# honglianghe/CDNet

Measured on AMD Instinct MI355X. Metric: tiles/sec (train fwd+bwd+Adam), 256x256, higher is better.
Workload: dtype fp32

## Files before the change

### cdnet_amd/csrc/conv.hip

```cpp
#include <type_traits>
#include <vector>
#include "common.h"
#include "conv_args.h"
#include "launch.h"
#include "xform.h"
#include "stage16.h"
#include <stdlib.h>

using namespace cdnet;

typedef __attribute__((ext_vector_type(16))) float f32x16;
typedef __attribute__((ext_vector_type(4))) float f32x4;

namespace {

__device__ int g_dbg_dummy;

struct PackDesc {
    const float *w;
    unsigned short *out;
    int Cout, Cin, KH, KW, CK, BN, nchunk, ntile, TAPS, mode, parity;
    unsigned block0, nblocks;
    int split;
    const float *scale;
};

__device__ __forceinline__ void pack_range(const PackDesc &d, size_t first, size_t stride) {
    const float *__restrict__ w = d.w;
    unsigned short *__restrict__ out = d.out;
    const int Cout = d.Cout, Cin = d.Cin, KH = d.KH, KW = d.KW, CK = d.CK, BN = d.BN, nchunk = d.nchunk, TAPS = d.TAPS, mode = d.mode,
              parity = d.parity;
    const size_t total = (size_t)d.ntile * nchunk * TAPS * (CK / 16) * 2 * BN * (d.split ? 2 : 1);
    for (size_t i = first; i < total; i += stride) {
        size_t r = i;
        int tap = r % TAPS; r /= TAPS;
        int col = r % BN; r /= BN;
        int half = r % 2; r /= 2;
        int kc = r % (CK / 16); r /= (CK / 16);
        int hl = 0;
        if (d.split) { hl = r % 2; r /= 2; }
        int chunk = r % nchunk; r /= nchunk;
        int tile = (int)r;
        int co = tile * BN + col;
        const size_t ovec = ((((((size_t)tile * nchunk + chunk) * (d.split ? 2 : 1) + hl) * TAPS + tap) * (CK / 16) + kc) * 2 + half) * BN + col;
        unsigned short o8[8];
#pragma unroll
        for (int j = 0; j < 8; ++j) {
        int ci = chunk * CK + kc * 16 + half * 8 + j;
        float v = 0.f;
        if (co < Cout && ci < Cin) {
            if (mode == 0) {
                v = w[(((size_t)co * Cin + ci) * KH + tap / KW) * KW + tap % KW];
            } else if (mode == 1) {
                int kh = KH - 1 - tap / KW, kw = KW - 1 - tap % KW;
                v = w[(((size_t)ci * Cout + co) * KH + kh) * KW + kw];
            } else if (mode == 2) {
                int a = parity >> 1, b = parity & 1, ty = tap >> 1, tx = tap & 1;
                int kh = a == 0 ? (ty == 0 ? 1 : 3) : (ty == 0 ? 0 : 2);
                int kw = b == 0 ? (tx == 0 ? 1 : 3) : (tx == 0 ? 0 : 2);
                v = w[(((size_t)ci * Cout + co) * 4 + kh) * 4 + kw];
            } else if (mode == 3) {
                int a = parity >> 1, b = parity & 1;
                v = w[(((size_t)ci * Cout + co) * 2 + a) * 2 + b];
            } else if (mode == 7) {
                const int Ct = Cout / 4;
                const int a = co / (2 * Ct), b = (co / Ct) & 1, c = co % Ct;
                const int tf = 8 - tap;
                const int kh = 2 * (tf / 3 - 1) + a + 1, kw = 2 * (tf % 3 - 1) + b + 1;
                if (kh >= 0 && kh < 3 && kw >= 0 && kw < 3) v = w[(((size_t)ci * Ct + c) * 3 + kh) * 3 + kw];
            } else {
                const int Ct = Cin / 4;
                const int a = ci / (2 * Ct), b = (ci / Ct) & 1, c = ci % Ct;
                if (mode == 4) {
                    const int kh = 2 * (tap / 3) + a - 1, kw = 2 * (tap % 3) + b - 1;
                    if (kh >= 0 && kh < 4 && kw >= 0 && kw < 4) v = w[(((size_t)co * Ct + c) * 4 + kh) * 4 + kw];
                } else if (mode == 5) {
                    v = w[(((size_t)co * Ct + c) * 2 + a) * 2 + b];
                } else {
                    const int kh = 2 * (tap / 3 - 1) + a + 1, kw = 2 * (tap % 3 - 1) + b + 1;
                    if (kh >= 0 && kh < 3 && kw >= 0 && kw < 3) v = w[(((size_t)co * Ct + c) * 3 + kh) * 3 + kw];
                }
            }
        }
        if (d.scale && co < Cout) v *= d.scale[co];
        const unsigned short hi = f2bf(v);
        o8[j] = hl ? f2bf(v - bf2f(hi)) : hi;
        }
        uint4 ov;
        ov.x = o8[0] | ((unsigned)o8[1] << 16); ov.y = o8[2] | ((unsigned)o8[3] << 16);
        ov.z = o8[4] | ((unsigned)o8[5] << 16); ov.w = o8[6] | ((unsigned)o8[7] << 16);
        reinterpret_cast<uint4 *>(out)[ovec] = ov;
    }
}

__global__ void pack_weights_kernel(PackDesc d) {
    pack_range(d, (size_t)blockIdx.x * blockDim.x + threadIdx.x, (size_t)gridDim.x * blockDim.x);
}

__global__ void pack_weights_batch_kernel(const PackDesc *__restrict__ table, int n) {
    int lo = 0, hi = n - 1;
    while (lo < hi) {
        const int mid = (lo + hi + 1) >> 1;
        if (table[mid].block0 <= blockIdx.x) lo = mid; else hi = mid - 1;
    }
    const PackDesc d = table[lo];
    pack_range(d, (size_t)(blockIdx.x - d.block0) * blockDim.x + threadIdx.x, (size_t)d.nblocks * blockDim.x);
}

__device__ __forceinline__ V16 max8(V16 a, V16 b, bool nonneg) {
    V16 o;
    if (nonneg) {
        o.u = __builtin_bit_cast(uint4, xf_max_nonneg_bf8(__builtin_bit_cast(xf_u32x4, a.u), __builtin_bit_cast(xf_u32x4, b.u)));
        return o;
    }
#pragma unroll
    for (int j = 0; j < 8; ++j) o.h[j] = bf2f(a.h[j]) >= bf2f(b.h[j]) ? a.h[j] : b.h[j];
    return o;
}

constexpr int XF_MAX = 2048;

__device__ __forceinline__ void load_chan_xf(ChanXf &t, const ConvSrc &s, const float *xf, int xfs, int c) {
    t.on = s.scale != nullptr;
    if (!t.on) return;
    const float4 *ps = reinterpret_cast<const float4 *>(xf ? xf + c : s.scale + c);
    const float4 *ph = reinterpret_cast<const float4 *>(xf ? xf + xfs + c : s.shift + c);
    float4 a = ps[0], b = ps[1], cc = ph[0], d = ph[1];
    t.sc[0] = a.x; t.sc[1] = a.y; t.sc[2] = a.z; t.sc[3] = a.w; t.sc[4] = b.x; t.sc[5] = b.y; t.sc[6] = b.z; t.sc[7] = b.w;
    t.sh[0] = cc.x; t.sh[1] = cc.y; t.sh[2] = cc.z; t.sh[3] = cc.w; t.sh[4] = d.x; t.sh[5] = d.y; t.sh[6] = d.z; t.sh[7] = d.w;
}

template <int TH, int CK>
struct HaloImg {
    static constexpr bool SWZ = (TH == 16 && CK == 16);
    static constexpr int PSTR = SWZ ? CK * 2 : CK * 2 + 16;
    __device__ __forceinline__ static int off(int pix, int hy, int slot) { return pix * PSTR + (SWZ ? ((slot ^ (hy & 1)) * 16) : slot * 16); }
};

template <int TH, int TW, int CK>
__device__ __forceinline__ void stage_input(const ConvSrc &s, int cc0, int n, int y0, int x0, int H, int W,
                                            unsigned char *lds_a, int tid, const float *xf = nullptr, int xfs = 0) {
    constexpr int VPP = CK / 8;
    constexpr int HW_ = TW + 2, NPIX = (TH + 2) * (TW + 2);
    const int slot = tid % VPP;
    ChanXf t;
    load_chan_xf(t, s, xf, xfs, cc0 + slot * 8);
    const bool relu = s.relu != 0;
    const bool f16 = s.f16 != 0;
    const bool plain = !t.on && !relu && s.res == nullptr && !f16;
    const int Hl = s.pool ? (s.Hs + (s.pool == 2)) / 2 : s.Hs, Wl = s.pool ? (s.Ws + (s.pool == 2)) / 2 : s.Ws;
    const size_t rs = s.row_stride ? (size_t)s.row_stride : (size_t)s.Ws * s.C;
    const size_t img = (size_t)n * s.Hs * rs;
    for (int v = tid; v < NPIX * VPP; v += 256) {
        const int pix = v / VPP;
        const int hy = pix / HW_, hx = pix - hy * HW_;
        const int y = y0 - 1 + hy, x = x0 - 1 + hx;
        V16 val;
        val.u = make_uint4(0, 0, 0, 0);
        const int ys = y - s.off_y, xs = x - s.off_x;
        if (y >= 0 && y < H && x >= 0 && x < W && ys >= 0 && ys < Hl && xs >= 0 && xs < Wl) {
            if (!s.pool) {
                const size_t e = img + (size_t)ys * rs + (size_t)xs * s.C + cc0 + slot * 8;
                V16 raw;
                raw.u = *reinterpret_cast<const uint4 *>(s.x + e);
                if (plain) val = raw;
                else if (s.res) { V16 r; r.u = *reinterpret_cast<const uint4 *>(s.res + e); val = xform8(raw, &r, t, relu, f16); }
                else val = xform8(raw, nullptr, t, relu, f16);
            } else {
#pragma unroll
                for (int q = 0; q < 4; ++q) {
                    const int yy = 2 * ys + (q >> 1), xx = 2 * xs + (q & 1);
                    if (q != 0 && (yy >= s.Hs || xx >= s.Ws)) continue;
                    const size_t e = img + (size_t)yy * rs + (size_t)xx * s.C + cc0 + slot * 8;
                    V16 raw;
                    raw.u = *reinterpret_cast<const uint4 *>(s.x + e);
                    V16 tv = plain ? raw : xform8(raw, nullptr, t, relu, f16);
                    val = q == 0 ? tv : max8(val, tv, relu);
                }
            }
        }
        *reinterpret_cast<uint4 *>(lds_a + HaloImg<TH, CK>::off(pix, hy, slot)) = val.u;
    }
}

#ifndef CDNET_CONV_XCD
#define CDNET_CONV_XCD 1
#endif
#ifndef CDNET_CONV_GLDS
#define CDNET_CONV_GLDS 1
#endif
#ifndef CDNET_CONV_ADEPTH
#define CDNET_CONV_ADEPTH 1
#endif
template <int TH, int TW, int CK, int BN, int TAPS>
struct ConvLds {
    static constexpr bool DEEP = (CK == 16 && TH == 16);
    static constexpr bool GLDS = CDNET_CONV_GLDS && DEEP;
    static constexpr int ADEPTH = DEEP ? CDNET_CONV_ADEPTH : 1;
    static constexpr int PSTR = HaloImg<TH, CK>::PSTR;
    static constexpr int A_BYTES = (TH + 2) * (TW + 2) * PSTR;
    static constexpr int B_BYTES = TAPS * CK * BN * 2;
    static constexpr int STAGE = A_BYTES + (GLDS ? 2 : 1) * B_BYTES;
    static constexpr int OUT_BYTES = TH * TW * (BN * 2 + 8);
    static constexpr int STATS_BYTES = 4 * 2 * BN * 4;
    static constexpr int MAIN = ((STAGE > OUT_BYTES + STATS_BYTES ? STAGE : OUT_BYTES + STATS_BYTES) + 15) / 16 * 16;
    static int bytes(int ctot) { return MAIN + 2 * ((ctot + 7) / 8 * 8) * 4; }
};

template <int TH, int TW, int CK, int BN, int TAPS>
struct Prefetch {
    static constexpr int VPP = CK / 8;
    static constexpr int NPIX = (TH + 2) * (TW + 2);
    static constexpr int NA = (NPIX * VPP + 255) / 256;
    static constexpr bool GLDS = ConvLds<TH, TW, CK, BN, TAPS>::GLDS;
    static constexpr int NB = (TAPS * CK * BN * 2 / 16 + 255) / 256;
    static constexpr int ADEPTH = ConvLds<TH, TW, CK, BN, TAPS>::ADEPTH;
    struct ASlot {
        uint4 a[NA];
        unsigned valid;
        bool pooled;
    };
    ASlot s[ADEPTH];
    uint4 b[GLDS ? 1 : NB];
    int eoff[2][NA];
    unsigned tvalid[2];
};

template <int SI, int TH, int TW, int CK, int BN, int TAPS>
__device__ __forceinline__ void prep_source(Prefetch<TH, TW, CK, BN, TAPS> &P, const ConvSrc &s, int y0, int x0, int H, int W, int tid) {
    using PF = Prefetch<TH, TW, CK, BN, TAPS>;
    constexpr int HW_ = TW + 2;
    const int slot = tid % PF::VPP;
    const int rs = s.row_stride ? s.row_stride : s.Ws * s.C;
    P.tvalid[SI] = 0;
#pragma unroll
    for (int i = 0; i < PF::NA; ++i) {
        const int v = tid + i * 256;
        const int pix = v / PF::VPP;
        const int hy = pix / HW_, hx = pix - hy * HW_;
        const int y = y0 - 1 + hy, x = x0 - 1 + hx;
        const int ys = y - s.off_y, xs = x - s.off_x;
        const bool inr = v < PF::NPIX * PF::VPP;
        const bool ok = inr && (unsigned)y < (unsigned)H && (unsigned)x < (unsigned)W && (unsigned)ys < (unsigned)s.Hs && (unsigned)xs < (unsigned)s.Ws;
        P.eoff[SI][i] = ok ? ys * rs + xs * s.C + slot * 8 : -1;
        P.tvalid[SI] |= (ok ? 1u : 0u) << i;
    }
}

template <int TH, int TW, int CK, int BN, int TAPS>
__device__ __forceinline__ void issue_b(Prefetch<TH, TW, CK, BN, TAPS> &P, const unsigned short *wchunk, int tid, unsigned char *lds_b_next) {
    using PF = Prefetch<TH, TW, CK, BN, TAPS>;
    if (PF::GLDS) {
        constexpr int NVEC = TAPS * CK * BN * 2 / 16;
        static_assert(NVEC % 64 == 0, "whole wave-instructions");
        const int wave = tid >> 6, lane = tid & 63;
#pragma unroll
        for (int i = 0; i < PF::NB; ++i) {
            const int v0 = (i * 4 + wave) * 64;
            if (v0 < NVEC)
                __builtin_amdgcn_global_load_lds((const __attribute__((address_space(1))) void *)(wchunk + (size_t)(v0 + lane) * 8),
                                                 (__attribute__((address_space(3))) void *)(lds_b_next + v0 * 16), 16, 0, 0);
        }
    } else {
        const uint4 *src = reinterpret_cast<const uint4 *>(wchunk);
#pragma unroll
        for (int i = 0; i < PF::NB; ++i) {
            const int v = tid + i * 256;
            if (v < TAPS * CK * BN * 2 / 16) P.b[i] = src[v];
        }
    }
}

template <typename PF>
__device__ __forceinline__ void issue_a(PF &P, typename PF::ASlot &S, const ConvSrc &s, int si, int cc0, int n) {
    S.pooled = s.pool != 0;
    S.valid = 0;
    if (S.pooled) return;
    const size_t rs = s.row_stride ? (size_t)s.row_stride : (size_t)s.Ws * s.C;
    const unsigned short *base = s.x + (size_t)n * s.Hs * rs + cc0;
    S.valid = si ? P.tvalid[1] : P.tvalid[0];
#pragma unroll
    for (int i = 0; i < PF::NA; ++i) {
        const int e = si ? P.eoff[1][i] : P.eoff[0][i];
        if (e >= 0) S.a[i] = *reinterpret_cast<const uint4 *>(base + e);
    }
}

template <int TH, int TW, int CK, int BN, int TAPS>
__device__ __forceinline__ void commit_chunk(const Prefetch<TH, TW, CK, BN, TAPS> &P, const typename Prefetch<TH, TW, CK, BN, TAPS>::ASlot &S,
                                             const ConvSrc &s, int si, int cc0, int n, int y0,
                                             int x0, int H, int W, unsigned char *lds_a, unsigned char *lds_b, int tid,
                                             const float *xf, int xfs) {
    using PF = Prefetch<TH, TW, CK, BN, TAPS>;
    if (!PF::GLDS) {
        uint4 *dst = reinterpret_cast<uint4 *>(lds_b);
#pragma unroll
        for (int i = 0; i < PF::NB; ++i) {
            const int v = tid + i * 256;
            if (v < TAPS * CK * BN * 2 / 16) dst[v] = P.b[i];
        }
    }
    if (S.pooled) { stage_input<TH, TW, CK>(s, cc0, n, y0, x0, H, W, lds_a, tid, xf, xfs); return; }
    const int slot = tid % PF::VPP;
    ChanXf t;
    load_chan_xf(t, s, xf, xfs, cc0 + slot * 8);
    const bool relu = s.relu != 0, f16 = s.f16 != 0;
    const bool plain = !t.on && !relu && s.res == nullptr && !f16;
    const size_t rs = s.row_stride ? (size_t)s.row_stride : (size_t)s.Ws * s.C;
    V16 rr[PF::NA];
    if (s.res) {
        const unsigned short *rbase = s.res + (size_t)n * s.Hs * rs + cc0;
#pragma unroll
        for (int i = 0; i < PF::NA; ++i) rr[i].u = *reinterpret_cast<const uint4 *>(rbase + ((S.valid & (1u << i)) ? (si ? P.eoff[1][i] : P.eoff[0][i]) : 0));
    }
#pragma unroll
    for (int i = 0; i < PF::NA; ++i) {
        if (tid + i * 256 >= PF::NPIX * PF::VPP) continue;
        V16 val;
        val.u = make_uint4(0, 0, 0, 0);
        if (S.valid & (1u << i)) {
            V16 raw;
            raw.u = S.a[i];
            if (plain) val = raw;
            else if (s.res) val = xform8(raw, &rr[i], t, relu, f16);
            else val = xform8(raw, nullptr, t, relu, f16);
        }
        const int pix = (tid + i * 256) / PF::VPP;
        *reinterpret_cast<uint4 *>(lds_a + HaloImg<TH, CK>::off(pix, pix / (TW + 2), slot)) = val.u;
    }
}

template <int TH, int TW, int CK, int BN, int WM, int WN, int TAPS>
__global__ __launch_bounds__(256, (BN <= 64 ? (CK == 16 && TH == 16 && CDNET_CONV_ADEPTH <= 2 ? 3 : 2) : 1)) void conv_fwd_kernel(ConvArgs A) {
    constexpr int PSTR = HaloImg<TH, CK>::PSTR;
    constexpr bool SWZ = HaloImg<TH, CK>::SWZ;
    constexpr int HW_ = TW + 2;
    constexpr int KC = CK / 16;
    constexpr int MT = TH * TW / 32, NT = BN / 32;
    constexpr int MPW = MT / WM, NPW = NT / WN;
    using LDS = ConvLds<TH, TW, CK, BN, TAPS>;
    constexpr bool GLDS = LDS::GLDS;
    constexpr int A_BYTES = LDS::A_BYTES;
    constexpr int B_BYTES = LDS::B_BYTES;
    constexpr int OSTR = BN * 2 + 8;
    static_assert(MT % WM == 0 && NT % WN == 0 && WM * WN == 4, "wave tiling");

    extern __shared__ __attribute__((aligned(16))) unsigned char smem[];
    unsigned char *lds_a = smem;
    unsigned char *lds_b0 = smem + A_BYTES;
    float (*s_stats)[2][BN] = reinterpret_cast<float (*)[2][BN]>(smem + LDS::OUT_BYTES);
    float *s_xf = reinterpret_cast<float *>(smem + LDS::MAIN);

    const int tid = threadIdx.x, lane = tid & 63, wave = tid >> 6;
    const int wm = wave / WN, wn = wave % WN;
    const int half = lane >> 5, l31 = lane & 31;
    const int xfs = ((A.src[0].C + (A.nsrc > 1 ? A.src[1].C : 0)) + 7) / 8 * 8;
    {
        const int c0n = A.src[0].C, ctot = c0n + (A.nsrc > 1 ? A.src[1].C : 0);
        for (int c = tid; c < ctot; c += 256) {
            const ConvSrc &S = c < c0n ? A.src[0] : A.src[1];
            const int cc = c < c0n ? c : c - c0n;
            s_xf[c] = S.scale ? S.scale[cc] : 1.f;
            s_xf[xfs + c] = S.shift ? S.shift[cc] : 0.f;
        }
    }

    const int tiles_x = (A.W + TW - 1) / TW, tiles_y = (A.H + TH - 1) / TH;
    const int tiles_img = tiles_x * tiles_y;
    const int total_tiles = A.N * A.npar * tiles_img;
    const int nchunk_total = A.nchunk;
#if CDNET_CONV_XCD
    int tile, cout_tile;
    {
        const int NC = (int)gridDim.y, lin = (int)blockIdx.y * (int)gridDim.x + (int)blockIdx.x;
        const int T = (int)gridDim.x * NC, q = T >> 3, rem = T & 7;
        const int xcd = lin & 7, idx = lin >> 3;
        const int seq = xcd < rem ? xcd * (q + 1) + idx : rem * (q + 1) + (xcd - rem) * q + idx;
        tile = seq / NC;
// ... 592 lines not shown
#endif
        return;
    }

    if (!STREAM) {
        const u32x4v *src = reinterpret_cast<const u32x4v *>(A.w + (size_t)cout_tile * 4 * (L::B_CHUNK / 2));
        u32x4v *dst = reinterpret_cast<u32x4v *>(lds_w);
        constexpr int nv = 4 * (L::B_CHUNK / 16), NW = (nv + 255) / 256;
        u32x4v wv[NW];
#pragma unroll
        for (int i = 0; i < NW; ++i) wv[i] = src[tid + i * 256 < nv ? tid + i * 256 : 0];
#pragma unroll
        for (int i = 0; i < NW; ++i)
            if (tid + i * 256 < nv) dst[tid + i * 256] = wv[i];
    }
    __syncthreads();
    const int wm = wave;
    const int half = lane >> 5, l31 = lane & 31;
    int abase[MPW][2];
#pragma unroll
    for (int mi = 0; mi < MPW; ++mi) {
        const int m = (wm * MPW + mi) * 32 + l31;
#pragma unroll
        for (int par = 0; par < 2; ++par) abase[mi][par] = ((m / TW) * HW_ + m % TW) * PSTR + ((half ^ ((m / TW + par) & 1)) * 16);
    }
    auto tpar = [](int t) { return (TAPS == 9 ? t / 3 : 1) & 1; };
    const int bbase = half * BN * 16 + l31 * 16;
    auto toff = [](int t) { return ((TAPS == 9 ? t / 3 : 1) * HW_ + (TAPS == 9 ? t % 3 : 1)) * PSTR; };
    f32x16 accA[MPW][NPW], accB[MPW][NPW];
    unsigned char *s_out = lds_o + wave * L::OUT_WAVE + l31 * L::IROW + half * 8;
    float e_osc[NPW], e_osh[NPW];
#pragma unroll
    for (int ni = 0; ni < NPW; ++ni) {
        const int co = cout0 + ni * 32 + l31;
        const bool cok = co < A.Cout;
        e_osc[ni] = (A.oscale && cok) ? A.oscale[co] : 1.f;
        e_osh[ni] = fmaf((A.bias && cok) ? A.bias[co] : 0.f, e_osc[ni], (A.oshift && cok) ? A.oshift[co] : 0.f);
    }
    const bool f16out = A.out_f16 != 0;
    const xf_s16x2 lo_clamp = A.orelu ? xf_s16x2{0, 0} : xf_s16x2{(short)-32768, (short)-32768};

    constexpr int NU = MPW * NPW * 4;
    float st_sum = 0.f, st_sq = 0.f;
    auto stat_unit = [&](const f32x16 (&P)[MPW][NPW], int u, int par) {
        const int ni = u / (MPW * 4), mi = (u / 4) % MPW, g = u % 4;
        if (mi == 0 && g == 0) { st_sum = 0.f; st_sq = 0.f; }
#pragma unroll
        for (int j = 0; j < 4; ++j) { const float v = P[mi][ni][4 * g + j]; st_sum += v; st_sq = fmaf(v, v, st_sq); }
        if (mi == MPW - 1 && g == 3) {
            float *sp = s_stats + par * (4 * 2 * BN);
            const float a = st_sum + __shfl_xor(st_sum, 32), b2 = st_sq + __shfl_xor(st_sq, 32);
            if (half == 0) {
                sp[(wave * 2 + 0) * BN + ni * 32 + l31] = a;
                sp[(wave * 2 + 1) * BN + ni * 32 + l31] = b2;
            }
        }
    };
    auto img_unit = [&](const f32x16 (&P)[MPW][NPW], int u) {
        const int mi = u / (NPW * 4), ni = (u / 4) % NPW, g = u % 4;
        const float osc = e_osc[ni], osh = e_osh[ni];
        const xf_f32x2 p0 = {fmaf(P[mi][ni][4 * g], osc, osh), fmaf(P[mi][ni][4 * g + 1], osc, osh)};
        const xf_f32x2 p1 = {fmaf(P[mi][ni][4 * g + 2], osc, osh), fmaf(P[mi][ni][4 * g + 3], osc, osh)};
        const xf_s16x2 h0 = __builtin_bit_cast(xf_s16x2, __builtin_convertvector(p0, xf_h16x2)), h1 = __builtin_bit_cast(xf_s16x2, __builtin_convertvector(p1, xf_h16x2));
        const xf_s16x2 b0 = __builtin_bit_cast(xf_s16x2, __builtin_convertvector(p0, xf_bf16x2)), b1 = __builtin_bit_cast(xf_s16x2, __builtin_convertvector(p1, xf_bf16x2));
        const xf_s16x2 k0 = __builtin_elementwise_max(f16out ? h0 : b0, lo_clamp), k1 = __builtin_elementwise_max(f16out ? h1 : b1, lo_clamp);
        *reinterpret_cast<uint2 *>(s_out + (mi * NPW + ni) * L::IBLK + g * 16) = make_uint2(__builtin_bit_cast(unsigned, k0), __builtin_bit_cast(unsigned, k1));
    };
    constexpr int SLOTS = TAPS * MPW * NPW;
    constexpr int IMG0 = STATS ? 2 * NU + 1 : 0;
    static_assert(IMG0 + 2 * NU <= 2 * SLOTS, "the deferred epilogue fits the MFMA slots of interval A");

    int stats_tile = -1, stats_par = 0;
    auto flush_stats = [&]() {
        if (STATS && stats_tile >= 0 && tid < 2 * BN) {
            const int which = tid / BN, col = tid % BN;
            const float *sp = s_stats + stats_par * (4 * 2 * BN);
            float v = 0.f;
#pragma unroll
            for (int w4 = 0; w4 < 4; ++w4) v += sp[(w4 * 2 + which) * BN + col];
            const int co = cout0 + col;
            if (co < A.Cout) A.stats[((size_t)stats_tile * 2 + which) * A.Cout + co] = v;
        }
        stats_tile = -1;
    };

    auto interval = [&](auto first_c, auto epi_c, f32x16 (&C)[MPW][NPW], const f32x16 (&P)[MPW][NPW], int par, int c0) {
        constexpr bool FIRST = decltype(first_c)::value;
        constexpr bool EPI = decltype(epi_c)::value;
        constexpr int NTAP = 2 * TAPS;
        bf16x8 af[3][MPW], bfr[3][NPW];
        const unsigned char *la = lds_a + c0 * L::A_BYTES, *lw = lds_w + c0 * L::B_CHUNK;
        auto request = [&](int tau) {
            const int ch = tau / TAPS, t = tau % TAPS;
#pragma unroll
            for (int mi = 0; mi < MPW; ++mi) af[tau % 3][mi] = *reinterpret_cast<const bf16x8 *>(la + ch * L::A_BYTES + abase[mi][tpar(t)] + toff(t));
#pragma unroll
            for (int ni = 0; ni < NPW; ++ni) bfr[tau % 3][ni] = *reinterpret_cast<const bf16x8 *>(lw + ch * L::B_CHUNK + bbase + (t * 2) * BN * 16 + ni * 512);
        };
        request(0);
        request(1);
#pragma unroll
        for (int tau = 0; tau < NTAP; ++tau) {
            if (tau + 2 < NTAP) request(tau + 2);
#pragma unroll
            for (int mi = 0; mi < MPW; ++mi)
#pragma unroll
                for (int ni = 0; ni < NPW; ++ni) {
                    if (FIRST && tau == 0) {
                        const f32x16 z = {0.f, 0.f, 0.f, 0.f, 0.f, 0.f, 0.f, 0.f, 0.f, 0.f, 0.f, 0.f, 0.f, 0.f, 0.f, 0.f};
                        C[mi][ni] = __builtin_amdgcn_mfma_f32_32x32x16_bf16(af[tau % 3][mi], bfr[tau % 3][ni], z, 0, 0, 0);
                    } else {
                        C[mi][ni] = __builtin_amdgcn_mfma_f32_32x32x16_bf16(af[tau % 3][mi], bfr[tau % 3][ni], C[mi][ni], 0, 0, 0);
                    }
                    if (EPI) {
                        const int sl = (tau * MPW + mi) * NPW + ni;
                        if (STATS && sl < 2 * NU && (sl & 1) == 0) { __builtin_amdgcn_sched_barrier(0); stat_unit(P, sl / 2, par); __builtin_amdgcn_sched_barrier(0); }
                        if (sl >= IMG0 && sl < IMG0 + 2 * NU && ((sl - IMG0) & 1) == 0) { __builtin_amdgcn_sched_barrier(0); img_unit(P, (sl - IMG0) / 2); __builtin_amdgcn_sched_barrier(0); }
                    }
                }
        }
    };
    using F_ = std::false_type;
    using T_ = std::true_type;
    auto tile_step = [&](auto has_prev, f32x16 (&C)[MPW][NPW], const f32x16 (&P)[MPW][NPW], int j) {
        constexpr bool HP = decltype(has_prev)::value;
        const int par = (j + 1) & 1;
        WS_STAMP(10);
#ifdef CDNET_WS_STAMPS
        if (A.debug & 512) interval(T_{}, F_{}, C, P, par, 0); else
#endif
        interval(T_{}, has_prev, C, P, par, 0);
        if (HP && STATS) { stats_tile = t_lo + j - 1; stats_par = par; }
        WS_STAMP(11);
        __syncthreads();
        WS_STAMP(14);
        flush_stats();
        interval(F_{}, F_{}, C, P, par, 2);
        WS_STAMP(12);
        __syncthreads();
        WS_STAMP(13);
        if (STREAM) {
            const int NI = NCH / 2;
            for (int i = 2; i < NI; ++i) {
                interval(F_{}, F_{}, C, P, par, (i & 1) * 2);
                __syncthreads();
            }
        }
    };
    auto serial_epilogue = [&](const f32x16 (&P)[MPW][NPW], int j) {
        const int par = j & 1;
        if (STATS) {
#pragma unroll
            for (int u = 0; u < NU; ++u) stat_unit(P, u, par);
            stats_tile = t_lo + j;
            stats_par = par;
        }
#pragma unroll
        for (int u = 0; u < NU; ++u) img_unit(P, u);
    };

    __syncthreads();
    tile_step(F_{}, accA, accB, 0);
    int j = 1;
    for (; j + 1 < ntl; j += 2) {
        tile_step(T_{}, accB, accA, j);
        tile_step(T_{}, accA, accB, j + 1);
    }
    if (j < ntl) {
        tile_step(T_{}, accB, accA, j);
        serial_epilogue(accB, j);
    } else {
        serial_epilogue(accA, ntl - 1);
    }
    __syncthreads();
    flush_stats();
#ifdef CDNET_WS_STAMPS
    if (stamp_on) { for (int i = 0; i < sn; ++i) g_ws_stamps[i] = s_stamp[i]; g_ws_stamps[sn] = 0; }
#endif
}

template <int BN, int TAPS>
int try_launch_conv_ws(const ConvArgs &A, hipStream_t st, bool dry_run = false) {
    using L = WsLds<BN, TAPS>;
    int ctot = 0;
    if (A.ws == 2) return -1;
    if (A.eres) return -1;
    if (A.nchunk < 4 || A.nchunk % 4 != 0) return -1;
    if ((A.src[0].C / 16) & 1) return -1;
    const bool stream = A.nchunk != 4;
    if (A.H % 16 != 0 || A.W % 16 != 0) return -1;
    for (int i = 0; i < A.nsrc; ++i) {
        if (A.src[i].pool || A.src[i].relu == 3) return -1;
        ctot += A.src[i].C;
        if (!in_mover_reach(A.src[i], (long long)A.N * A.npar, 2)) return -1;
    }
#ifdef CDNET_WS_STAMPS
    const int smem = L::bytes(4, ctot, 2) + 2 * 384 * 8;
#else
    const int smem = L::bytes(4, ctot, 2);
#endif
    if (smem > 160 * 1024) return -1;
    const int T = (A.W / 16) * (A.H / 16) * A.N;
    int n_cu = 0;
    if (const int rc = cu_count(&n_cu)) return rc;
    const int ctiles = cdiv(A.Cout, BN);
    const int Gmax = n_cu / ctiles > 0 ? n_cu / ctiles : 1;
    if (!(A.debug & CONV_DBG_PERSIST_SMALL) && ((long long)T * A.nchunk < 12LL * Gmax || (T < Gmax && A.nchunk < 16))) return -1;
    bool all_plain = true, all_fast = true;
    for (int i = 0; i < A.nsrc; ++i) {
        const ConvSrc &s = A.src[i];
        all_plain = all_plain && !s.scale && !s.relu && !s.res && !s.f16;
        all_fast = all_fast && s.scale && s.relu && !s.res && s.f16 == 1;
    }
    dim3 grid(persistent_grid(n_cu, ctiles, T, 0, 0), ctiles, 1);
    const int xf = all_plain ? 0 : (all_fast ? 1 : 2);
    if (dry_run) return CDNET_OK;
    return with_bool(A.stats != nullptr, [&](auto st_c) {
        return with_int<0, 1, 2>(xf, [&](auto xf_c) {
            return with_bool(stream, [&](auto sm_c) {
                return launch_lds<conv_ws_kernel<BN, TAPS, decltype(xf_c)::value, decltype(st_c)::value, decltype(sm_c)::value>>(
                    grid, 512, 160 * 1024, smem, st, "hipFuncSetAttribute(conv_ws)", "conv_ws_kernel", A);
            });
        });
    });
}

template <int TAPS>
int dispatch_conv(const ConvArgs &A, hipStream_t st) {
    const int key = A.tile * 10000 + A.CK * 100 + (A.BN == 128 ? 99 : A.BN);
    switch (key) {
        case 16 * 10000 + 16 * 100 + 32: return launch_conv<16, 16, 16, 32, 4, 1, TAPS>(A, st);
        case 16 * 10000 + 16 * 100 + 64: return launch_conv<16, 16, 16, 64, 4, 1, TAPS>(A, st);
        case 16 * 10000 + 32 * 100 + 32: return launch_conv<16, 16, 32, 32, 4, 1, TAPS>(A, st);
        case 16 * 10000 + 32 * 100 + 64: return launch_conv<16, 16, 32, 64, 4, 1, TAPS>(A, st);
        case 16 * 10000 + 32 * 100 + 99: return launch_conv<16, 16, 32, 128, 2, 2, TAPS>(A, st);
        case 16 * 10000 + 64 * 100 + 64: return launch_conv<16, 16, 64, 64, 4, 1, TAPS>(A, st);
        case 8 * 10000 + 32 * 100 + 64: return launch_conv<8, 8, 32, 64, 2, 2, TAPS>(A, st);
        case 8 * 10000 + 32 * 100 + 99: return launch_conv<8, 8, 32, 128, 2, 2, TAPS>(A, st);
        case 8 * 10000 + 64 * 100 + 64: return launch_conv<8, 8, 64, 64, 2, 2, TAPS>(A, st);
        default:
            set_error("cdnet_conv: unsupported configuration tile=%d CK=%d BN=%d", A.tile, A.CK, A.BN);
            return CDNET_E_ARG;
    }
}

__global__ __launch_bounds__(256) void materialize_kernel(const ConvSrc s, int N, int H, int W, unsigned short *__restrict__ out) {
    const int VPP = s.C / 8;
    const size_t total = (size_t)N * H * W * VPP;
    const bool relu = s.relu != 0, f16 = s.f16 != 0;
    const int Hl = s.pool ? (s.Hs + (s.pool == 2)) / 2 : s.Hs, Wl = s.pool ? (s.Ws + (s.pool == 2)) / 2 : s.Ws;
    const size_t rs = s.row_stride ? (size_t)s.row_stride : (size_t)s.Ws * s.C;
    for (size_t i = (size_t)blockIdx.x * 256 + threadIdx.x; i < total; i += (size_t)gridDim.x * 256) {
        const int slot = (int)(i % VPP);
        const size_t pix = i / VPP;
        const int x = (int)(pix % W), y = (int)((pix / W) % H), n = (int)(pix / ((size_t)W * H));
        ChanXf t;
        load_chan_xf(t, s, nullptr, 0, slot * 8);
        const bool plain = !t.on && !relu && s.res == nullptr && !f16;
        const size_t img = (size_t)n * s.Hs * rs;
        V16 val;
        val.u = make_uint4(0, 0, 0, 0);
        const int ys = y - s.off_y, xs = x - s.off_x;
        if (ys >= 0 && ys < Hl && xs >= 0 && xs < Wl) {
            if (!s.pool) {
                const size_t e = img + (size_t)ys * rs + (size_t)xs * s.C + slot * 8;
                V16 raw;
                raw.u = *reinterpret_cast<const uint4 *>(s.x + e);
                if (plain) val = raw;
                else if (s.res) { V16 r; r.u = *reinterpret_cast<const uint4 *>(s.res + e); val = xform8(raw, &r, t, relu, f16); }
                else val = xform8(raw, nullptr, t, relu, f16);
            } else {
                V16 raw[4];
                bool ok[4];
#pragma unroll
                for (int q = 0; q < 4; ++q) {
                    int yy = 2 * ys + (q >> 1), xx = 2 * xs + (q & 1);
                    ok[q] = q == 0 || (yy < s.Hs && xx < s.Ws);
                    yy = yy < s.Hs ? yy : s.Hs - 1;
                    xx = xx < s.Ws ? xx : s.Ws - 1;
                    raw[q].u = *reinterpret_cast<const uint4 *>(s.x + img + (size_t)yy * rs + (size_t)xx * s.C + slot * 8);
                }
#pragma unroll
                for (int q = 0; q < 4; ++q) {
                    const V16 tv = plain ? raw[q] : xform8(raw[q], nullptr, t, relu, f16);
                    val = q == 0 ? tv : (ok[q] ? max8(val, tv, relu) : val);
                }
            }
        }
        *reinterpret_cast<uint4 *>(out + pix * s.C + slot * 8) = val.u;
    }
}

}

extern "C" size_t cdnet_conv_packed_weight_elems(int Cout, int Cin_padded_chunks, int taps, int CK, int BN, int npar) {
    return (size_t)npar * cdiv(Cout, BN) * Cin_padded_chunks * taps * CK * BN;
}

static int fill_pack_desc(PackDesc &d, const float *w, void *packed, int Cout, int Cin, int KH, int KW, int CK, int BN, int mode, int p,
                          const char *who) {
    const int split = (mode & 16) ? 1 : 0;
    mode &= 15;
    CDNET_REQUIRE(w && packed, "%s: null pointer", who);
    CDNET_REQUIRE(CK % 16 == 0 && BN % 32 == 0 && Cin % CK == 0 && mode >= 0 && mode <= 7, "%s: Cin=%d CK=%d BN=%d mode=%d", who, Cin, CK, BN, mode);
    const int taps = mode == 2 ? 4 : (mode == 3 ? 1 : ((mode == 4 || mode == 6 || mode == 7) ? 9 : (mode == 5 ? 1 : KH * KW)));
    const int nchunk = Cin / CK, ntile = cdiv(Cout, BN);
    const size_t per = (size_t)ntile * nchunk * taps * CK * BN * (split ? 2 : 1);
    d.split = split;
    d.scale = nullptr;
    d.w = w; d.out = (unsigned short *)packed + (size_t)p * per;
    d.Cout = Cout; d.Cin = Cin; d.KH = KH; d.KW = KW; d.CK = CK; d.BN = BN; d.nchunk = nchunk; d.ntile = ntile; d.TAPS = taps; d.mode = mode;
    d.parity = p;
    d.block0 = 0;
    d.nblocks = (unsigned)((per + 2047) / 2048);
    if (d.nblocks > 4096) d.nblocks = 4096;
    return CDNET_OK;
}

extern "C" int cdnet_pack_conv_weights(const float *w, void *packed, int Cout, int Cin, int KH, int KW, int CK, int BN,
                                       int mode, void *stream) {
    const int npar = ((mode & 15) == 2 || (mode & 15) == 3) ? 4 : 1;
    for (int p = 0; p < npar; ++p) {
        PackDesc d;
        int rc = fill_pack_desc(d, w, packed, Cout, Cin, KH, KW, CK, BN, mode, p, "cdnet_pack_conv_weights");
        if (rc) return rc;
        pack_weights_kernel<<<d.nblocks, 256, 0, (hipStream_t)stream>>>(d);
    }
    return check_launch("cdnet_pack_conv_weights");
}

extern "C" int cdnet_pack_conv_weights_scaled(const float *w, const float *cout_scale, void *packed, int Cout, int Cin, int KH, int KW, int CK,
                                              int BN, int mode, void *stream) {
    CDNET_REQUIRE(cout_scale && (mode & 15) == 0, "cdnet_pack_conv_weights_scaled: forward Conv2d packs (mode 0) with a scale vector");
    PackDesc d;
    int rc = fill_pack_desc(d, w, packed, Cout, Cin, KH, KW, CK, BN, mode, 0, "cdnet_pack_conv_weights_scaled");
    if (rc) return rc;
    d.scale = cout_scale;
    pack_weights_kernel<<<d.nblocks, 256, 0, (hipStream_t)stream>>>(d);
    return check_launch("cdnet_pack_conv_weights_scaled");
}

extern "C" size_t cdnet_pack_batch_table_bytes(int n_jobs) { return (size_t)n_jobs * 4 * sizeof(PackDesc); }

extern "C" int cdnet_pack_conv_weights_batch(const cdnet_pack_job *jobs, int n_jobs, void *table, size_t table_bytes, int upload,
                                             void *stream) {
    CDNET_REQUIRE(jobs && n_jobs > 0 && table, "cdnet_pack_conv_weights_batch: null pointer / no jobs");
    CDNET_REQUIRE(table_bytes >= cdnet_pack_batch_table_bytes(n_jobs), "cdnet_pack_conv_weights_batch: table too small");
    static thread_local std::vector<PackDesc> host;
    host.clear();
    unsigned blocks = 0;
    for (int j = 0; j < n_jobs; ++j) {
        const cdnet_pack_job &J = jobs[j];
        const int npar = ((J.mode & 15) == 2 || (J.mode & 15) == 3) ? 4 : 1;
        for (int p = 0; p < npar; ++p) {
            PackDesc d;
            int rc = fill_pack_desc(d, J.w, J.packed, J.Cout, J.Cin, J.KH, J.KW, J.CK, J.BN, J.mode, p, "cdnet_pack_conv_weights_batch");
            if (rc) return rc;
            d.block0 = blocks;
            blocks += d.nblocks;
            host.push_back(d);
        }
    }
    hipStream_t st = (hipStream_t)stream;
    if (upload) {
        if (hipMemcpyAsync(table, host.data(), host.size() * sizeof(PackDesc), hipMemcpyHostToDevice, st) != hipSuccess ||
            hipStreamSynchronize(st) != hipSuccess)
            return check_launch("cdnet_pack_conv_weights_batch(upload)");
    }
    pack_weights_batch_kernel<<<blocks, 256, 0, st>>>((const PackDesc *)table, (int)host.size());
    return check_launch("cdnet_pack_conv_weights_batch");
}

extern "C" int cdnet_conv_forward(const cdnet_conv_args *args, void *stream) {
    CDNET_REQUIRE(args, "cdnet_conv_forward: null args");
    const ConvArgs &A = *reinterpret_cast<const ConvArgs *>(args);
    CDNET_REQUIRE(A.nsrc >= 1 && A.nsrc <= 2 && A.w && (A.out || A.dot_out), "cdnet_conv_forward: bad pointers / nsrc=%d", A.nsrc);
    CDNET_REQUIRE(!A.dot_out || (A.dot_w && !A.f32 && !A.pool_out), "cdnet_conv_forward: dot_out needs dot_w, the 16-bit path and no pool_out");
    CDNET_REQUIRE(A.N > 0 && A.H > 0 && A.W > 0 && A.Cout > 0 && A.Cout % 8 == 0, "cdnet_conv_forward: bad size (Cout must be a multiple of 8)");
    {
        int ctot_xf = 0;
        for (int i = 0; i < A.nsrc; ++i) ctot_xf += A.src[i].C;
        CDNET_REQUIRE(ctot_xf <= XF_MAX, "cdnet_conv_forward: %d source channels exceed the %d-entry scale/shift table", ctot_xf, XF_MAX);
    }
    CDNET_REQUIRE(A.ws == 0 || A.ws == 2, "cdnet_conv_forward: ws must be 0 or 2 (BatchNorm-backward statistics epilogue)");
    if (A.f32) {
        CDNET_REQUIRE(A.f32 == 1, "cdnet_conv_forward: f32 must be 0 or 1");
        for (int i = 0; i < A.nsrc; ++i)
            CDNET_REQUIRE(A.src[i].f16 == 2, "cdnet_conv_forward(f32): every source must be fp32 (f16 = 2)");
    } else {
        for (int i = 0; i < A.nsrc; ++i)
            CDNET_REQUIRE(A.src[i].f16 == 0 || A.src[i].f16 == 1, "cdnet_conv_forward: fp32 sources need args.f32 = 1");
    }
    if (A.eres && A.ws != 2) {
        CDNET_REQUIRE(A.ostride == 1 && A.npar == 1 && A.out_coff == 0 && A.out_cstride == A.Cout && !A.stats && !A.orelu &&
                      !A.out_f16 && ((A.eres_scale == nullptr) == (A.eres_shift == nullptr)),
                      "cdnet_conv_forward: fused residual epilogue needs a dense bf16 output, no statistics and no ReLU before the add");
    }
    int nchunk = 0;
    for (int i = 0; i < A.nsrc; ++i) {
        CDNET_REQUIRE(A.src[i].x && A.src[i].C % A.CK == 0, "cdnet_conv_forward: source %d channels %d not a multiple of CK=%d",
                      i, A.src[i].C, A.CK);
        CDNET_REQUIRE(!(A.src[i].pool && A.src[i].res), "cdnet_conv_forward: pool+residual source unsupported");
        nchunk += A.src[i].C / A.CK;
    }
    const bool padded = A.nchunk == nchunk + 1 && A.taps == 9 && A.nsrc == 2 && !A.f32;
    CDNET_REQUIRE(nchunk == A.nchunk || padded, "cdnet_conv_forward: nchunk %d != %d", A.nchunk, nchunk);
    CDNET_REQUIRE((A.taps == 9 && A.npar == 1 && A.ostride == 1) || (A.taps == 1 && A.npar == 1 && A.ostride == 1) ||
                  (A.taps == 4 && A.npar == 4 && A.ostride == 2) || (A.taps == 1 && A.npar == 4 && A.ostride == 2),
                  "cdnet_conv_forward: taps=%d npar=%d ostride=%d", A.taps, A.npar, A.ostride);
    CDNET_REQUIRE(A.out_cstride % 8 == 0 && A.out_coff % 8 == 0, "cdnet_conv_forward: output channel slice must be 16-byte aligned");
    hipStream_t st = (hipStream_t)stream;
    CDNET_REQUIRE(A.taps1 == 0 || A.taps1 == A.taps || (A.taps1 == 1 && A.taps == 9 && A.nsrc == 2), "cdnet_conv_forward: taps1 = %d (0, taps, or 1 beside a nine-tap first source)", A.taps1);
    if (A.f32) return conv_forward_f32(A, st);
    {
        const int rc = conv_forward_ws16(A, st);
        if (rc >= 0) return rc;
        CDNET_REQUIRE(A.taps1 == 0 || A.taps1 == A.taps, "cdnet_conv_forward: a one-tap second source runs on conv_ws16_kernel only (ask cdnet_conv_ws_eligible)");
        CDNET_REQUIRE(!A.pool_out, "cdnet_conv_forward: the fused max-pool output needs conv_ws16_kernel's out-image form (ask cdnet_conv_ws_eligible)");
        CDNET_REQUIRE(!A.dot_out, "cdnet_conv_forward: the fused 1x1 classifier (dot_out) needs conv_ws16_kernel's out-image form with resident weights (ask cdnet_conv_ws_eligible)");
        CDNET_REQUIRE(!padded, "cdnet_conv_forward: a padding chunk (nchunk = real + 1) runs on conv_ws16_kernel only (ask cdnet_conv_ws_eligible)");
    }
    static const int dbg = getenv("CDNET_CONV_DEBUG") ? atoi(getenv("CDNET_CONV_DEBUG")) : 0;
    if (!(A.debug & CONV_DBG_ONE_TILE) && A.taps == 9 && A.npar == 1 && A.ostride == 1 && A.tile == 16 && A.CK == 16 && (A.BN == 64 || A.BN == 32)) {
        const int rc = A.BN == 64 ? try_launch_conv_ws<64, 9>(A, st) : try_launch_conv_ws<32, 9>(A, st);
        if (rc >= 0) return rc;
    }
    for (int i = 0; i < A.nsrc; ++i)
        CDNET_REQUIRE(A.src[i].relu >= 0 && A.src[i].relu <= 2, "cdnet_conv_forward: source %d: relu = %d (the BatchNorm-backward source of round 2, relu = 3, was removed)", i, A.src[i].relu);
    CDNET_REQUIRE(A.ws != 2, "cdnet_conv_forward: the BatchNorm-backward statistics epilogue (ws = 2) exists in fp32 mode on conv_ws32_kernel only "
                             "(ask cdnet_conv_ws_eligible first)");
    if (dbg) { ConvArgs B = A; B.debug = dbg; if (B.taps == 9) return dispatch_conv<9>(B, st); }
    if (A.debug & CONV_DBG_ONE_TILE) { ConvArgs B = A; B.debug = 0; if (B.taps == 9) return dispatch_conv<9>(B, st); if (B.taps == 4) return dispatch_conv<4>(B, st); return dispatch_conv<1>(B, st); }
    if (A.taps == 9) return dispatch_conv<9>(A, st);
    if (A.taps == 4) return dispatch_conv<4>(A, st);
    return dispatch_conv<1>(A, st);
}

extern "C" int cdnet_conv_ws_eligible(const cdnet_conv_args *args) {
    if (!args) return 0;
    const ConvArgs &A = *reinterpret_cast<const ConvArgs *>(args);
    if (A.f32) return (!A.dot_out && conv_forward_f32_ws(A, nullptr, true) == CDNET_OK) ? 1 : 0;
    if (conv_forward_ws16(A, nullptr, true) == CDNET_OK) return 2;
    if ((A.taps1 != 0 && A.taps1 != A.taps) || A.pool_out || A.dot_out) return 0;
    if (A.debug & CONV_DBG_ONE_TILE) return 0;
    if (!(A.taps == 9 && A.npar == 1 && A.ostride == 1 && A.tile == 16 && A.CK == 16 && (A.BN == 64 || A.BN == 32))) return 0;
    const int rc = A.BN == 64 ? try_launch_conv_ws<64, 9>(A, nullptr, true) : try_launch_conv_ws<32, 9>(A, nullptr, true);
    return rc == CDNET_OK ? 1 : 0;
}

extern "C" int cdnet_src_materialize(const cdnet_conv_src *src, int N, int H, int W, uint16_t *out, void *stream) {
    CDNET_REQUIRE(src && out && src->x && N > 0 && H > 0 && W > 0, "cdnet_src_materialize: bad args");
    const ConvSrc &s = *reinterpret_cast<const ConvSrc *>(src);
    CDNET_REQUIRE(s.C >= 8 && s.C % 8 == 0 && s.Hs > 0 && s.Ws > 0, "cdnet_src_materialize: C=%d must be a multiple of 8", s.C);
    CDNET_REQUIRE(!(s.pool && s.res), "cdnet_src_materialize: pooled sources carry no residual");
    CDNET_REQUIRE((s.scale == nullptr) == (s.shift == nullptr), "cdnet_src_materialize: scale and shift come together");
    if (s.f16 == 2) return materialize_f32(s, N, H, W, out, (hipStream_t)stream);
    const size_t total = (size_t)N * H * W * (s.C / 8);
    size_t g = (total + 255) / 256;
    g = g > 8192 ? 8192 : g;
    materialize_kernel<<<(int)g, 256, 0, (hipStream_t)stream>>>(s, N, H, W, out);
    return check_launch("cdnet_src_materialize");
}
```

### cdnet_amd/csrc/conv32.hip

```cpp
#include <type_traits>
#include "common.h"
#include "conv_args.h"
#include "launch.h"
#include <stdlib.h>

using namespace cdnet;

typedef __attribute__((ext_vector_type(8))) __bf16 bf16x8;
typedef __attribute__((ext_vector_type(2))) __bf16 bf16x2;
typedef __attribute__((ext_vector_type(16))) float f32x16;
typedef __attribute__((ext_vector_type(2))) float f32x2;
typedef unsigned u32x4 __attribute__((ext_vector_type(4)));
typedef float f32x4 __attribute__((ext_vector_type(4)));

namespace {

__device__ __forceinline__ void split8(const float *v, u32x4 &hi, u32x4 &lo) {
#pragma unroll
    for (int k = 0; k < 4; ++k) {
        const f32x2 x = {v[2 * k], v[2 * k + 1]};
        const bf16x2 h = __builtin_convertvector(x, bf16x2);
        const unsigned hb = __builtin_bit_cast(unsigned, h);
        const f32x2 hf = {__builtin_bit_cast(float, hb << 16), __builtin_bit_cast(float, hb & 0xffff0000u)};
        const bf16x2 l = __builtin_convertvector(x - hf, bf16x2);
        hi[k] = hb;
        lo[k] = __builtin_bit_cast(unsigned, l);
    }
}

constexpr int CK = 16;
constexpr int PSTR = CK * 2 + 16;
constexpr int XF_MAX = 2048;

template <int TH, int TW, int BN, int TAPS>
struct Lds32 {
    static constexpr int NPIX = (TH + 2) * (TW + 2);
    static constexpr int A_PLANE = NPIX * PSTR;
    static constexpr int B_PLANE = TAPS * CK * BN * 2;
    static constexpr int STAGE = 2 * A_PLANE + 2 * B_PLANE;
    static constexpr int STATS_BYTES = 4 * 2 * BN * 4;
    static constexpr int MAIN = ((STAGE > STATS_BYTES ? STAGE : STATS_BYTES) + 15) / 16 * 16;
    static int bytes(int ctot) { return MAIN + 2 * ((ctot + 7) / 8 * 8) * 4; }
};


template <int MPW, int NPW, int TW>
__device__ __forceinline__ void store_tile_f32(const ConvArgs &A, const f32x16 (&acc)[MPW][NPW], int n, int y0, int x0, int mblock0, int nblock0,
                                               int half, int l31, int cout0, int pa_, int pb_) {
    const int Ho = A.H * A.ostride, Wo = A.W * A.ostride;
    float *out = reinterpret_cast<float *>(A.out);
    const float *eres = reinterpret_cast<const float *>(A.eres);
    const bool full = y0 + 16 <= A.H && x0 + TW <= A.W && cout0 + (nblock0 + NPW) * 32 <= A.Cout && A.ostride == 1 && TW == 16 &&
                      !(A.debug & 16);
    if (full) {
        const int cs = A.out_cstride, ce = A.Cout;
        float *tb = out + (((size_t)n * A.H + y0) * A.W + x0) * cs + A.out_coff;
        const float *te = eres ? eres + (((size_t)n * A.H + y0) * A.W + x0) * ce : nullptr;
#pragma unroll
        for (int ni = 0; ni < NPW; ++ni) {
            const int co = cout0 + (nblock0 + ni) * 32 + l31;
            const float osc = A.oscale ? A.oscale[co] : 1.f;
            const float osh = fmaf(A.bias ? A.bias[co] : 0.f, osc, A.oshift ? A.oshift[co] : 0.f);
            const float esc = (eres && A.eres_scale) ? A.eres_scale[co] : 1.f;
            const float esh = (eres && A.eres_shift) ? A.eres_shift[co] : 0.f;
            float *ob = tb + co;
#pragma unroll
            for (int mi = 0; mi < MPW; ++mi) {
                const int rowb = ((mblock0 + mi) * 2) * A.W + 4 * half;
                float ev[16];
                if (eres) {
#pragma unroll
                    for (int r = 0; r < 16; ++r) {
                        const int p = (r & 3) + 8 * (r >> 2);
                        ev[r] = te[(rowb + (p / 16) * A.W + (p % 16)) * ce + co];
                    }
                }
#pragma unroll
                for (int r = 0; r < 16; ++r) {
                    const int p = (r & 3) + 8 * (r >> 2);
                    const int off = (rowb + (p / 16) * A.W + (p % 16)) * cs;
                    float v = fmaf(acc[mi][ni][r], osc, osh);
                    if (A.orelu) v = fmaxf(v, 0.f);
                    if (eres) {
                        v = fmaf(ev[r], esc, esh) + v;
                        if (A.eres_relu) v = fmaxf(v, 0.f);
                    }
                    ob[off] = v;
                }
            }
        }
        return;
    }
#pragma unroll
    for (int ni = 0; ni < NPW; ++ni) {
        const int co = cout0 + (nblock0 + ni) * 32 + l31;
        const bool cok = co < A.Cout;
        const float osc = (A.oscale && cok) ? A.oscale[co] : 1.f;
        const float osh = fmaf((A.bias && cok) ? A.bias[co] : 0.f, osc, (A.oshift && cok) ? A.oshift[co] : 0.f);
        const float esc = (A.eres && A.eres_scale && cok) ? A.eres_scale[co] : 1.f;
        const float esh = (A.eres && A.eres_shift && cok) ? A.eres_shift[co] : 0.f;
#pragma unroll
        for (int mi = 0; mi < MPW; ++mi) {
            float ev[16];
            if (A.eres) {
#pragma unroll
                for (int r = 0; r < 16; ++r) {
                    const int m = (mblock0 + mi) * 32 + (r & 3) + 8 * (r >> 2) + 4 * half;
                    int y = y0 + m / TW, x = x0 + m % TW;
                    y = y < A.H ? y : A.H - 1; x = x < A.W ? x : A.W - 1;
                    ev[r] = eres[(((size_t)n * A.H + y) * A.W + x) * A.Cout + (cok ? co : 0)];
                }
            }
#pragma unroll
            for (int r = 0; r < 16; ++r) {
                const int m = (mblock0 + mi) * 32 + (r & 3) + 8 * (r >> 2) + 4 * half;
                const int y = y0 + m / TW, x = x0 + m % TW;
                float v = fmaf(acc[mi][ni][r], osc, osh);
                if (A.orelu) v = fmaxf(v, 0.f);
                if (A.eres) {
                    v = fmaf(ev[r], esc, esh) + v;
                    if (A.eres_relu) v = fmaxf(v, 0.f);
                }
                if (cok && y < A.H && x < A.W) {
                    const size_t opix = ((size_t)n * Ho + (y * A.ostride + pa_)) * Wo + (x * A.ostride + pb_);
                    out[opix * A.out_cstride + A.out_coff + co] = v;
                }
            }
        }
    }
}

template <int TH, int TW, int BN, int WM, int WN, int TAPS>
__global__ __launch_bounds__(256, 2) void conv_f32_kernel(ConvArgs A) {
    using L = Lds32<TH, TW, BN, TAPS>;
    constexpr int HW_ = TW + 2, NPIX = L::NPIX;
    constexpr int MT = TH * TW / 32, NT = BN / 32;
    constexpr int MPW = MT / WM, NPW = NT / WN;
    constexpr int VPP = CK / 8;
    constexpr int NA = (NPIX * VPP + 255) / 256;
    constexpr int NBV = 2 * L::B_PLANE / 16;
    constexpr int NB = (NBV + 255) / 256;
    static_assert(MT % WM == 0 && NT % WN == 0 && WM * WN == 4, "wave tiling");

    extern __shared__ __attribute__((aligned(16))) unsigned char smem[];
    unsigned char *lds_a = smem;
    unsigned char *lds_b = smem + 2 * L::A_PLANE;
    float (*s_stats)[2][BN] = reinterpret_cast<float (*)[2][BN]>(smem);
    float *s_xf = reinterpret_cast<float *>(smem + L::MAIN);

    const int tid = threadIdx.x, lane = tid & 63, wave = tid >> 6;
    const int wm = wave / WN, wn = wave % WN;
    const int half = lane >> 5, l31 = lane & 31;
    const int c0n = A.src[0].C, ctot = c0n + (A.nsrc > 1 ? A.src[1].C : 0);
    const int xfs = (ctot + 7) / 8 * 8;
    for (int c = tid; c < ctot; c += 256) {
        const ConvSrc &S = c < c0n ? A.src[0] : A.src[1];
        const int cc = c < c0n ? c : c - c0n;
        s_xf[c] = S.scale ? S.scale[cc] : 1.f;
        s_xf[xfs + c] = S.shift ? S.shift[cc] : 0.f;
    }

    const int tiles_x = (A.W + TW - 1) / TW, tiles_y = (A.H + TH - 1) / TH;
    const int tiles_img = tiles_x * tiles_y;
    int tile, cout_tile;
    {
        const int NC = (int)gridDim.y, lin = (int)blockIdx.y * (int)gridDim.x + (int)blockIdx.x;
        const int T = (int)gridDim.x * NC, q = T >> 3, rem = T & 7;
        const int xcd = lin & 7, idx = lin >> 3;
        const int seq = xcd < rem ? xcd * (q + 1) + idx : rem * (q + 1) + (xcd - rem) * q + idx;
        tile = seq / NC;
        cout_tile = seq - tile * NC;
    }
    const int z = tile / tiles_img, rt = tile - z * tiles_img;
    const int n = z / A.npar, par = z - n * A.npar;
    const int ty_ = rt / tiles_x;
    const int y0 = ty_ * TH, x0 = (rt - ty_ * tiles_x) * TW;

    int eoff[2][NA];
    const int slot = tid % VPP;
#pragma unroll
    for (int si = 0; si < 2; ++si) {
        if (si >= A.nsrc) break;
        const ConvSrc &s = A.src[si];
        const int rs = s.row_stride ? s.row_stride : s.Ws * s.C;
#pragma unroll
        for (int i = 0; i < NA; ++i) {
            const int v = tid + i * 256;
            const int pix = v / VPP;
            const int hy = pix / HW_, hx = pix - hy * HW_;
            const int y = y0 - 1 + hy, x = x0 - 1 + hx;
            const int ys = y - s.off_y, xs = x - s.off_x;
            const bool ok = v < NPIX * VPP && (unsigned)y < (unsigned)A.H && (unsigned)x < (unsigned)A.W && (unsigned)ys < (unsigned)s.Hs &&
                            (unsigned)xs < (unsigned)s.Ws;
            eoff[si][i] = ok ? ys * rs + xs * s.C + slot * 8 : -1;
        }
    }
    auto chunk_src = [&](int c, int &si, int &cc0) {
        const int n0 = A.src[0].C / CK;
        if (c < n0) { si = 0; cc0 = c * CK; } else { si = 1; cc0 = (c - n0) * CK; }
    };
    const unsigned short *wbase = A.w + ((size_t)(par * gridDim.y + cout_tile) * A.nchunk) * (size_t)(L::B_PLANE);

    f32x4 pa[NA][2];
    u32x4 pb[NB];
    auto issue = [&](int chunk) {
        int si, cc0;
        chunk_src(chunk, si, cc0);
        const ConvSrc &s = A.src[si];
        const size_t rs = s.row_stride ? (size_t)s.row_stride : (size_t)s.Ws * s.C;
        const float *base = reinterpret_cast<const float *>(s.x) + (size_t)n * s.Hs * rs + cc0;
#pragma unroll
        for (int i = 0; i < NA; ++i) {
            const int e = si ? eoff[1][i] : eoff[0][i];
            const f32x4 *p = reinterpret_cast<const f32x4 *>(base + (e >= 0 ? e : 0));
            pa[i][0] = p[0];
            pa[i][1] = p[1];
        }
        const u32x4 *wsrc = reinterpret_cast<const u32x4 *>(wbase + (size_t)chunk * L::B_PLANE);
#pragma unroll
        for (int i = 0; i < NB; ++i) {
            const int v = tid + i * 256;
            if (v < NBV) pb[i] = wsrc[v];
        }
    };
    auto commit = [&](int chunk) {
        int si, cc0;
        chunk_src(chunk, si, cc0);
        const ConvSrc &s = A.src[si];
        const bool on = s.scale != nullptr, relu = s.relu != 0;
        const float *xf = s_xf + (si ? c0n : 0) + cc0 + slot * 8;
        float sc[8], sh[8];
        if (on) {
#pragma unroll
            for (int j = 0; j < 8; ++j) { sc[j] = xf[j]; sh[j] = xf[xfs + j]; }
        }
        f32x4 rr[NA][2];
        if (s.res) {
            const size_t rs = s.row_stride ? (size_t)s.row_stride : (size_t)s.Ws * s.C;
            const float *rbase = reinterpret_cast<const float *>(s.res) + (size_t)n * s.Hs * rs + cc0;
#pragma unroll
            for (int i = 0; i < NA; ++i) {
                const int e = si ? eoff[1][i] : eoff[0][i];
                const f32x4 *p = reinterpret_cast<const f32x4 *>(rbase + (e >= 0 ? e : 0));
                rr[i][0] = p[0];
                rr[i][1] = p[1];
            }
        }
        unsigned char *dst0 = lds_a + (tid / VPP) * PSTR + slot * 16;
#pragma unroll
        for (int i = 0; i < NA; ++i) {
            if (tid + i * 256 >= NPIX * VPP) continue;
            const int e = si ? eoff[1][i] : eoff[0][i];
            u32x4 hi = {0u, 0u, 0u, 0u}, lo = {0u, 0u, 0u, 0u};
            if (e >= 0) {
                float v[8] = {pa[i][0][0], pa[i][0][1], pa[i][0][2], pa[i][0][3], pa[i][1][0], pa[i][1][1], pa[i][1][2], pa[i][1][3]};
                if (on) {
#pragma unroll
                    for (int j = 0; j < 8; ++j) v[j] = fmaf(v[j], sc[j], sh[j]);
                }
                if (s.res) {
                    const float r[8] = {rr[i][0][0], rr[i][0][1], rr[i][0][2], rr[i][0][3], rr[i][1][0], rr[i][1][1], rr[i][1][2], rr[i][1][3]};
#pragma unroll
                    for (int j = 0; j < 8; ++j) v[j] += r[j];
                }
                if (relu) {
#pragma unroll
                    for (int j = 0; j < 8; ++j) v[j] = fmaxf(v[j], 0.f);
                }
                split8(v, hi, lo);
            }
            unsigned char *d = dst0 + i * (256 / VPP) * PSTR;
            *reinterpret_cast<u32x4 *>(d) = hi;
            *reinterpret_cast<u32x4 *>(d + L::A_PLANE) = lo;
        }
        u32x4 *bdst = reinterpret_cast<u32x4 *>(lds_b);
#pragma unroll
        for (int i = 0; i < NB; ++i) {
            const int v = tid + i * 256;
            if (v < NBV) bdst[v] = pb[i];
        }
    };

    int abase[MPW];
#pragma unroll
    for (int mi = 0; mi < MPW; ++mi) {
        const int m = (wm * MPW + mi) * 32 + l31;
        abase[mi] = ((m / TW) * HW_ + m % TW) * PSTR + half * 16;
    }
    const int bbase = half * BN * 16 + (wn * NPW * 32 + l31) * 16;
    int toff[TAPS];
#pragma unroll
    for (int t = 0; t < TAPS; ++t) {
        int r, c;
        if (TAPS == 9) { r = t / 3; c = t % 3; }
        else if (TAPS == 4) {
            const int a = par >> 1, b = par & 1, ty = t >> 1, tx = t & 1;
            r = a == 0 ? (ty == 0 ? 1 : 0) : (ty == 0 ? 2 : 1);
            c = b == 0 ? (tx == 0 ? 1 : 0) : (tx == 0 ? 2 : 1);
        } else { r = 1; c = 1; }
        toff[t] = (r * HW_ + c) * PSTR;
    }
    f32x16 acc[MPW][NPW];
#pragma unroll
    for (int mi = 0; mi < MPW; ++mi)
#pragma unroll
        for (int ni = 0; ni < NPW; ++ni)
#pragma unroll
            for (int r = 0; r < 16; ++r) acc[mi][ni][r] = 0.f;

    issue(0);
    for (int chunk = 0; chunk < A.nchunk; ++chunk) {
        __syncthreads();
        commit(chunk);
        __syncthreads();
        if (chunk + 1 < A.nchunk) issue(chunk + 1);
#pragma unroll
        for (int t = 0; t < TAPS; ++t) {
            bf16x8 ah[MPW], al[MPW], bh[NPW], bl[NPW];
#pragma unroll
            for (int mi = 0; mi < MPW; ++mi) {
                ah[mi] = *reinterpret_cast<const bf16x8 *>(lds_a + abase[mi] + toff[t]);
                al[mi] = *reinterpret_cast<const bf16x8 *>(lds_a + L::A_PLANE + abase[mi] + toff[t]);
            }
#pragma unroll
            for (int ni = 0; ni < NPW; ++ni) {
                bh[ni] = *reinterpret_cast<const bf16x8 *>(lds_b + bbase + t * 2 * BN * 16 + ni * 512);
                bl[ni] = *reinterpret_cast<const bf16x8 *>(lds_b + L::B_PLANE + bbase + t * 2 * BN * 16 + ni * 512);
            }
#pragma unroll
            for (int mi = 0; mi < MPW; ++mi)
#pragma unroll
                for (int ni = 0; ni < NPW; ++ni) {
                    acc[mi][ni] = __builtin_amdgcn_mfma_f32_32x32x16_bf16(al[mi], bh[ni], acc[mi][ni], 0, 0, 0);
                    acc[mi][ni] = __builtin_amdgcn_mfma_f32_32x32x16_bf16(ah[mi], bl[ni], acc[mi][ni], 0, 0, 0);
                    acc[mi][ni] = __builtin_amdgcn_mfma_f32_32x32x16_bf16(ah[mi], bh[ni], acc[mi][ni], 0, 0, 0);
                }
        }
    }
    __syncthreads();

    const int cout0 = cout_tile * BN;
    if (A.stats) {
        float ssum[NPW], ssq[NPW];
        const bool full_tile = y0 + TH <= A.H && x0 + TW <= A.W && !(A.debug & 16);
#pragma unroll
        for (int ni = 0; ni < NPW; ++ni) {
            ssum[ni] = 0.f; ssq[ni] = 0.f;
            if (full_tile) {
#pragma unroll
                for (int mi = 0; mi < MPW; ++mi)
#pragma unroll
                    for (int r = 0; r < 16; ++r) {
                        const float v = acc[mi][ni][r];
                        ssum[ni] += v;
                        ssq[ni] = fmaf(v, v, ssq[ni]);
                    }
            } else {
#pragma unroll
            for (int mi = 0; mi < MPW; ++mi)
#pragma unroll
                for (int r = 0; r < 16; ++r) {
                    const int m = (wm * MPW + mi) * 32 + (r & 3) + 8 * (r >> 2) + 4 * half;
                    const float v = ((y0 + m / TW) < A.H && (x0 + m % TW) < A.W) ? acc[mi][ni][r] : 0.f;
                    ssum[ni] += v;
                    ssq[ni] = fmaf(v, v, ssq[ni]);
                }
            }
            ssum[ni] += __shfl_xor(ssum[ni], 32);
            ssq[ni] += __shfl_xor(ssq[ni], 32);
            if (half == 0) {
                s_stats[wave][0][(wn * NPW + ni) * 32 + l31] = ssum[ni];
                s_stats[wave][1][(wn * NPW + ni) * 32 + l31] = ssq[ni];
            }
        }
        __syncthreads();
        if (tid < 2 * BN) {
            const int which = tid / BN, col = tid % BN;
            const int wn_of = col / (NPW * 32);
            float v = 0.f;
#pragma unroll
            for (int k = 0; k < WM; ++k) v += s_stats[k * WN + wn_of][which][col];
            const int co = cout0 + col;
            if (co < A.Cout) A.stats[((size_t)tile * 2 + which) * A.Cout + co] = v;
        }
    }
    store_tile_f32<MPW, NPW, TW>(A, acc, n, y0, x0, wm * MPW, wn * NPW, half, l31, cout0, par >> 1, par & 1);
}

template <int TH, int TW, int BN, int WM, int WN, int TAPS>
int launch_conv32(const ConvArgs &A, hipStream_t st) {
    using L = Lds32<TH, TW, BN, TAPS>;
    int ctot = 0;
    for (int i = 0; i < A.nsrc; ++i) ctot += A.src[i].C;
    const int smem = L::bytes(ctot);
    dim3 grid(cdiv(A.W, TW) * cdiv(A.H, TH) * A.N * A.npar, cdiv(A.Cout, BN), 1);
    return launch_lds<conv_f32_kernel<TH, TW, BN, WM, WN, TAPS>>(grid, 256, L::bytes(XF_MAX), smem, st, "hipFuncSetAttribute(conv32)", "conv_f32_kernel", A);
}

template <int TAPS>
int dispatch_conv32(const ConvArgs &A, hipStream_t st) {
    if (A.tile == 16 && A.BN == 64) return launch_conv32<16, 16, 64, 4, 1, TAPS>(A, st);
    if (A.tile == 16 && A.BN == 32) return launch_conv32<16, 16, 32, 4, 1, TAPS>(A, st);
    if (A.tile == 8 && A.BN == 64) return launch_conv32<8, 8, 64, 2, 2, TAPS>(A, st);
    set_error("cdnet_conv_forward(f32): unsupported configuration tile=%d CK=%d BN=%d", A.tile, A.CK, A.BN);
    return CDNET_E_ARG;
}

template <int BN, int NCH, bool XF, bool ERES>
__global__ __launch_bounds__(256, 4) void conv1x1_f32_stream_kernel(ConvArgs A) {
    constexpr int NPW = BN / 32;
    constexpr int B_PLANE = CK * BN * 2;
    constexpr int CIN = NCH * CK;
    __shared__ __attribute__((aligned(16))) unsigned char smem[NCH * 2 * B_PLANE + 2 * CIN * 4];
    unsigned char *lds_b = smem;
    float *s_xf = reinterpret_cast<float *>(smem + NCH * 2 * B_PLANE);

    const int tid = threadIdx.x, lane = tid & 63, wave = __builtin_amdgcn_readfirstlane(tid >> 6);
    const int half = lane >> 5, l31 = lane & 31;
    const int cout_tile = blockIdx.y, cout0 = cout_tile * BN;
    const ConvSrc &S = A.src[0];
    {
        const u32x4 *wsrc = reinterpret_cast<const u32x4 *>(A.w + (size_t)cout_tile * NCH * B_PLANE);
        u32x4 *bdst = reinterpret_cast<u32x4 *>(lds_b);
        for (int v = tid; v < NCH * 2 * B_PLANE / 16; v += 256) bdst[v] = wsrc[v];
        for (int c = tid; c < CIN; c += 256) {
            s_xf[c] = S.scale ? S.scale[c] : 1.f;
            s_xf[CIN + c] = S.shift ? S.shift[c] : 0.f;
        }
    }
    __syncthreads();

    const size_t P = (size_t)A.N * A.H * A.W;
    const int nblk = (int)((P + 31) / 32), bstride = (int)gridDim.x * 4;
    int blk = (int)blockIdx.x * 4 + wave;
    if (blk >= nblk) return;
    const bool relu = S.relu != 0, orelu = A.orelu != 0, eres_relu = A.eres_relu != 0;
    const int cout = A.Cout;
    const int bbase = half * BN * 16 + l31 * 16;

    float osc[NPW], osh[NPW], esc[NPW], esh[NPW];
#pragma unroll
    for (int ni = 0; ni < NPW; ++ni) {
        const int co = cout0 + ni * 32 + l31, c = co < A.Cout ? co : 0;
        osc[ni] = A.oscale ? A.oscale[c] : 1.f;
        osh[ni] = fmaf(A.bias ? A.bias[c] : 0.f, osc[ni], A.oshift ? A.oshift[c] : 0.f);
        esc[ni] = (ERES && A.eres_scale) ? A.eres_scale[c] : 1.f;
        esh[ni] = (ERES && A.eres_shift) ? A.eres_shift[c] : 0.f;
    }

    const char *xbase = reinterpret_cast<const char *>(S.x);
    char *obase = reinterpret_cast<char *>(A.out) + (size_t)A.out_coff * 4;
    const char *ebase = ERES ? reinterpret_cast<const char *>(A.eres) : xbase;
    const unsigned cs4 = (unsigned)A.out_cstride * 4, ce4 = (unsigned)cout * 4;
    const unsigned vo_in = l31 * (CIN * 4) + half * 32;
    unsigned vo_out[NPW], vo_eres[NPW];
#pragma unroll
    for (int ni = 0; ni < NPW; ++ni) {
        const unsigned co = cout0 + ni * 32 + l31;
        vo_out[ni] = co < (unsigned)cout ? 4 * half * cs4 + co * 4 : 0x7fff0000u;
        vo_eres[ni] = co < (unsigned)cout ? 4 * half * ce4 + co * 4 : 0x7fff0000u;
    }
    auto rsrc = [&](const char *base, size_t bytes) {
        return __builtin_amdgcn_make_buffer_rsrc(const_cast<char *>(base), 0, (int)bytes, 0x00020000);
    };

    auto request = [&](f32x4 (&v)[NCH][2], int b) {
        const size_t left = P - (size_t)b * 32;
        const __amdgpu_buffer_rsrc_t rx = rsrc(xbase + (size_t)b * (32 * CIN * 4), (left < 32 ? left : 32) * (CIN * 4));
#pragma unroll
        for (int c = 0; c < NCH; ++c) {
            v[c][0] = __builtin_bit_cast(f32x4, __builtin_amdgcn_raw_buffer_load_b128(rx, (int)(vo_in + c * 64), 0, 0));
            v[c][1] = __builtin_bit_cast(f32x4, __builtin_amdgcn_raw_buffer_load_b128(rx, (int)(vo_in + c * 64 + 16), 0, 0));
        }
    };
    auto block = [&](auto tail_c, const f32x4 (&cur)[NCH][2], f32x4 (&nxt)[NCH][2]) {
        constexpr bool TAIL = decltype(tail_c)::value;
        asm volatile("" ::: "memory");
        if (!TAIL) {
            request(nxt, blk + bstride < nblk ? blk + bstride : blk);
            __builtin_amdgcn_sched_barrier(0);
        }
        f32x16 acc[NPW];
#pragma unroll
        for (int ni = 0; ni < NPW; ++ni)
#pragma unroll
            for (int r = 0; r < 16; ++r) acc[ni][r] = 0.f;
#pragma unroll
        for (int c = 0; c < NCH; ++c) {
            float v[8] = {cur[c][0][0], cur[c][0][1], cur[c][0][2], cur[c][0][3], cur[c][1][0], cur[c][1][1], cur[c][1][2], cur[c][1][3]};
            if (XF) {
                const float *xf = s_xf + c * CK + half * 8;
#pragma unroll
                for (int j = 0; j < 8; ++j) {
                    v[j] = fmaf(v[j], xf[j], xf[CIN + j]);
                    v[j] = relu ? fmaxf(v[j], 0.f) : v[j];
                }
            }
            u32x4 hi, lo;
            split8(v, hi, lo);
            const bf16x8 ah = __builtin_bit_cast(bf16x8, hi), al = __builtin_bit_cast(bf16x8, lo);
#pragma unroll
            for (int ni = 0; ni < NPW; ++ni) {
                const bf16x8 bh = *reinterpret_cast<const bf16x8 *>(lds_b + c * 2 * B_PLANE + bbase + ni * 512);
                const bf16x8 bl = *reinterpret_cast<const bf16x8 *>(lds_b + c * 2 * B_PLANE + B_PLANE + bbase + ni * 512);
                acc[ni] = __builtin_amdgcn_mfma_f32_32x32x16_bf16(al, bh, acc[ni], 0, 0, 0);
                acc[ni] = __builtin_amdgcn_mfma_f32_32x32x16_bf16(ah, bl, acc[ni], 0, 0, 0);
                acc[ni] = __builtin_amdgcn_mfma_f32_32x32x16_bf16(ah, bh, acc[ni], 0, 0, 0);
            }
        }
        const size_t left = P - (size_t)blk * 32, rows = left < 32 ? left : 32;
        const __amdgpu_buffer_rsrc_t ro = rsrc(obase + (size_t)blk * 32 * cs4, rows * cs4);
        float ev[NPW][16];
        if (ERES) {
            const __amdgpu_buffer_rsrc_t re = rsrc(ebase + (size_t)blk * 32 * ce4, rows * ce4);
#pragma unroll
            for (int ni = 0; ni < NPW; ++ni)
#pragma unroll
                for (int r = 0; r < 16; ++r) {
                    const unsigned pr = (r & 3) + 8 * (r >> 2);
                    ev[ni][r] = __builtin_bit_cast(float, TAIL ? __builtin_amdgcn_raw_buffer_load_b32(re, (int)(vo_eres[ni] + pr * ce4), 0, 0)
                                                               : __builtin_amdgcn_raw_buffer_load_b32(re, (int)vo_eres[ni], (int)(pr * ce4), 0));
                }
        }
#pragma unroll
        for (int ni = 0; ni < NPW; ++ni)
#pragma unroll
            for (int r = 0; r < 16; ++r) {
                const unsigned pr = (r & 3) + 8 * (r >> 2);
                float v = fmaf(acc[ni][r], osc[ni], osh[ni]);
                v = orelu ? fmaxf(v, 0.f) : v;
                if (ERES) {
                    v = fmaf(ev[ni][r], esc[ni], esh[ni]) + v;
                    v = eres_relu ? fmaxf(v, 0.f) : v;
                }
                if (TAIL) __builtin_amdgcn_raw_buffer_store_b32(__builtin_bit_cast(unsigned, v), ro, (int)(vo_out[ni] + pr * cs4), 0, 0);
                else __builtin_amdgcn_raw_buffer_store_b32(__builtin_bit_cast(unsigned, v), ro, (int)vo_out[ni], (int)(pr * cs4), 0);
            }
    };
    f32x4 xa[NCH][2], xb[NCH][2];
    const int nfull = (int)(P / 32);
    if (blk < nfull) {
        request(xa, blk);
#pragma unroll
        for (int c = 0; c < NCH; ++c) asm volatile("" ::"v"(xa[c][0]), "v"(xa[c][1]));
        for (;;) {
            block(std::false_type{}, xa, xb);
            blk += bstride;
            if (blk >= nfull) break;
            block(std::false_type{}, xb, xa);
            blk += bstride;
            if (blk >= nfull) break;
        }
    }
    if (blk < nblk) {
        request(xa, blk);
        block(std::true_type{}, xa, xb);
    }
}

template <int BN, int NCH>
int launch_conv1x1_stream(const ConvArgs &A, hipStream_t st) {
    int n_cu = 0;
    if (const int rc = cu_count(&n_cu)) return rc;
    const long long nblk = ((long long)A.N * A.H * A.W + 31) / 32;
    const int ctiles = cdiv(A.Cout, BN);
    const long long waves = (long long)n_cu * 16 / ctiles > 4 ? (long long)n_cu * 16 / ctiles : 4;
    const long long rounds = (nblk + waves - 1) / waves;
    const long long G = ((nblk + rounds - 1) / rounds + 3) / 4;
    dim3 grid((unsigned)G, ctiles, 1);
    return with_bool(A.src[0].scale != nullptr, [&](auto xf_c) {
        return with_bool(A.eres != nullptr, [&](auto er_c) {
            conv1x1_f32_stream_kernel<BN, NCH, decltype(xf_c)::value, decltype(er_c)::value><<<grid, 256, 0, st>>>(A);
            return check_launch("conv1x1_f32_stream_kernel");
        });
    });
}

int try_conv1x1_stream(const ConvArgs &A, hipStream_t st) {
    if (A.debug & CONV_DBG_NO_STREAM_1X1) return -1;
    if (A.taps != 1 || A.taps1 != 0 || A.npar != 1 || A.ostride != 1 || A.ws || A.stats || A.pool_out || A.nsrc != 1) return -1;
    const ConvSrc &s = A.src[0];
    if (s.off_y || s.off_x || s.Hs != A.H || s.Ws != A.W || (s.row_stride && s.row_stride != s.Ws * s.C) || s.pool || s.res) return -1;
    if (s.relu && !s.scale) return -1;
    if (s.C != A.nchunk * CK || (long long)A.N * A.H * A.W > (1LL << 31) - 64 || (long long)A.out_cstride * 4 * 36 >= (1LL << 31)) return -1;
    auto go = [&](auto bn_c) -> int {
        constexpr int BN = decltype(bn_c)::value;
        if (A.nchunk == 1) return launch_conv1x1_stream<BN, 1>(A, st);
        if (A.nchunk == 2) return launch_conv1x1_stream<BN, 2>(A, st);
        if (A.nchunk == 4) return launch_conv1x1_stream<BN, 4>(A, st);
        return -1;
    };
    if (A.BN == 64) return go(std::integral_constant<int, 64>{});
    if (A.BN == 32) return go(std::integral_constant<int, 32>{});
    return -1;
}

__global__ __launch_bounds__(256) void materialize_f32_kernel(const ConvSrc s, int N, int H, int W, float *__restrict__ out) {
    const int VPP = s.C / 4;
    const size_t total = (size_t)N * H * W * VPP;
    const bool relu = s.relu != 0, on = s.scale != nullptr;
    const int Hl = s.pool ? (s.Hs + (s.pool == 2)) / 2 : s.Hs, Wl = s.pool ? (s.Ws + (s.pool == 2)) / 2 : s.Ws;
    const size_t rs = s.row_stride ? (size_t)s.row_stride : (size_t)s.Ws * s.C;
    const float *sx = reinterpret_cast<const float *>(s.x), *sr = reinterpret_cast<const float *>(s.res);
    for (size_t i = (size_t)blockIdx.x * 256 + threadIdx.x; i < total; i += (size_t)gridDim.x * 256) {
        const int c = (int)(i % VPP) * 4;
        const size_t pix = i / VPP;
        const int x = (int)(pix % W), y = (int)((pix / W) % H), n = (int)(pix / ((size_t)W * H));
        float4 sc = make_float4(1.f, 1.f, 1.f, 1.f), sh = make_float4(0.f, 0.f, 0.f, 0.f);
        if (on) { sc = *reinterpret_cast<const float4 *>(s.scale + c); sh = *reinterpret_cast<const float4 *>(s.shift + c); }
        const size_t img = (size_t)n * s.Hs * rs;
        float4 val = make_float4(0.f, 0.f, 0.f, 0.f);
        const int ys = y - s.off_y, xs = x - s.off_x;
        auto xf = [&](float4 v, const float4 *r) {
            v.x = fmaf(v.x, sc.x, sh.x); v.y = fmaf(v.y, sc.y, sh.y); v.z = fmaf(v.z, sc.z, sh.z); v.w = fmaf(v.w, sc.w, sh.w);
            if (r) { v.x += r->x; v.y += r->y; v.z += r->z; v.w += r->w; }
            if (relu) { v.x = fmaxf(v.x, 0.f); v.y = fmaxf(v.y, 0.f); v.z = fmaxf(v.z, 0.f); v.w = fmaxf(v.w, 0.f); }
            return v;
        };
        if (ys >= 0 && ys < Hl && xs >= 0 && xs < Wl) {
            if (!s.pool) {
                const size_t e = img + (size_t)ys * rs + (size_t)xs * s.C + c;
                const float4 raw = *reinterpret_cast<const float4 *>(sx + e);
                if (sr) { const float4 r = *reinterpret_cast<const float4 *>(sr + e); val = xf(raw, &r); }
                else val = xf(raw, nullptr);
            } else {
                float4 raw[4];
                bool ok[4];
#pragma unroll
                for (int q = 0; q < 4; ++q) {
                    int yy = 2 * ys + (q >> 1), xx = 2 * xs + (q & 1);
                    ok[q] = q == 0 || (yy < s.Hs && xx < s.Ws);
                    yy = yy < s.Hs ? yy : s.Hs - 1;
                    xx = xx < s.Ws ? xx : s.Ws - 1;
                    raw[q] = *reinterpret_cast<const float4 *>(sx + img + (size_t)yy * rs + (size_t)xx * s.C + c);
                }
#pragma unroll
                for (int q = 0; q < 4; ++q) {
                    const float4 t = xf(raw[q], nullptr);
                    if (q == 0) val = t;
                    else if (ok[q]) { val.x = fmaxf(val.x, t.x); val.y = fmaxf(val.y, t.y); val.z = fmaxf(val.z, t.z); val.w = fmaxf(val.w, t.w); }
                }
            }
        }
        *reinterpret_cast<float4 *>(out + pix * s.C + c) = val;
    }
}

}

namespace cdnet {

int conv_forward_f32(const ConvArgs &A, hipStream_t st) {
    CDNET_REQUIRE(A.CK == 16, "cdnet_conv_forward(f32): CK must be 16 (got %d)", A.CK);
    for (int i = 0; i < A.nsrc; ++i)
        CDNET_REQUIRE(!A.src[i].pool, "cdnet_conv_forward(f32): pooled sources must be materialised (cdnet_src_materialize)");
    CDNET_REQUIRE(!A.out_f16, "cdnet_conv_forward(f32): out_f16 must be 0");
    {
        const int rc = conv_forward_f32_ws(A, st);
        if (rc >= 0) return rc;
    }
    CDNET_REQUIRE(A.ws != 2, "cdnet_conv_forward(f32): the BatchNorm-backward statistics epilogue (ws = 2) needs the producer / consumer kernel "
                             "(ask cdnet_conv_ws_eligible first)");
    CDNET_REQUIRE(A.taps1 == 0 || A.taps1 == A.taps, "cdnet_conv_forward(f32): a one-tap second source runs on conv_ws32_kernel only (ask cdnet_conv_ws_eligible)");
    CDNET_REQUIRE(!A.pool_out, "cdnet_conv_forward(f32): the fused max-pool output rides in conv_ws32_kernel's epilogue only (ask cdnet_conv_ws_eligible)");
    if (A.taps == 9) return dispatch_conv32<9>(A, st);
    if (A.taps == 4) return dispatch_conv32<4>(A, st);
    {
        const int rc = try_conv1x1_stream(A, st);
        if (rc >= 0) return rc;
    }
    return dispatch_conv32<1>(A, st);
}

int materialize_f32(const ConvSrc &s, int N, int H, int W, void *out, hipStream_t st) {
    const size_t total = (size_t)N * H * W * (s.C / 4);
    size_t g = (total + 255) / 256;
    g = g > 8192 ? 8192 : g;
    materialize_f32_kernel<<<(int)g, 256, 0, st>>>(s, N, H, W, reinterpret_cast<float *>(out));
    return check_launch("cdnet_src_materialize(f32)");
}

}
```

### cdnet_amd/csrc/conv_args.h

```cpp
#pragma once
#include "../../include/cdnet_hip.h"

struct ConvSrc {
    const unsigned short *x;
    const unsigned short *res;
    const float *scale;
    const float *shift;
    int C, Hs, Ws, pool, relu, off_y, off_x;
    int f16, row_stride;
};

struct ConvArgs {
    ConvSrc src[2];
    int nsrc;
    const unsigned short *w;
    const float *bias;
    const float *oscale;
    const float *oshift;
    int orelu;
    unsigned short *out;
    int Cout, out_cstride, out_coff;
    float *stats;
    int N, H, W;
    int taps, npar, ostride, nchunk;
    int tile, CK, BN;
    int out_f16;
    int debug;
    int ws;
    int f32;
    const unsigned short *eres;
    const float *eres_scale, *eres_shift;
    int eres_f16, eres_relu;
    int taps1, pad_;
    unsigned short *pool_out;
    const float *dot_w, *dot_b;
    float *dot_out;
};

enum : int {
    CONV_DBG_WS16_QUAD = 16,
    CONV_DBG_ONE_TILE = 32,
    CONV_DBG_PERSIST_SMALL = 64,
    CONV_DBG_OLD_WS16 = 128,
    CONV_DBG_NO_STREAM_1X1 = 256,
    CONV_DBG_GRID_SHIFT = 8,
};
enum : int {
    WGRAD_DBG_NO_WS = 8,
    WGRAD_DBG_ALL_QUADS = 16,
};

static_assert(sizeof(ConvSrc) == sizeof(cdnet_conv_src), "ConvSrc layout");
static_assert(sizeof(ConvArgs) == sizeof(cdnet_conv_args), "ConvArgs layout");

namespace cdnet {
int conv_forward_f32(const ConvArgs &A, hipStream_t st);
int conv_forward_f32_ws(const ConvArgs &A, hipStream_t st, bool dry_run = false);
int conv_forward_ws16(const ConvArgs &A, hipStream_t st, bool dry_run = false);
int materialize_f32(const ConvSrc &s, int N, int H, int W, void *out, hipStream_t st);
}
```

### cdnet_amd/engine.py

```python
import ctypes as C
import os
import torch

from . import _lib


class ConvSrc(C.Structure):
    _fields_ = [('x', C.c_void_p), ('res', C.c_void_p), ('scale', C.c_void_p), ('shift', C.c_void_p),
                ('C', C.c_int), ('Hs', C.c_int), ('Ws', C.c_int), ('pool', C.c_int), ('relu', C.c_int),
                ('off_y', C.c_int), ('off_x', C.c_int), ('f16', C.c_int), ('row_stride', C.c_int)]


class ConvArgs(C.Structure):
    _fields_ = [('src', ConvSrc * 2), ('nsrc', C.c_int), ('w', C.c_void_p), ('bias', C.c_void_p),
                ('oscale', C.c_void_p), ('oshift', C.c_void_p), ('orelu', C.c_int), ('out', C.c_void_p),
                ('Cout', C.c_int), ('out_cstride', C.c_int), ('out_coff', C.c_int), ('stats', C.c_void_p),
                ('N', C.c_int), ('H', C.c_int), ('W', C.c_int), ('taps', C.c_int), ('npar', C.c_int),
                ('ostride', C.c_int), ('nchunk', C.c_int), ('tile', C.c_int), ('CK', C.c_int), ('BN', C.c_int),
                ('out_f16', C.c_int), ('debug', C.c_int), ('ws', C.c_int), ('f32', C.c_int),
                ('eres', C.c_void_p), ('eres_scale', C.c_void_p), ('eres_shift', C.c_void_p), ('eres_f16', C.c_int), ('eres_relu', C.c_int),
                ('taps1', C.c_int), ('pad_', C.c_int), ('pool_out', C.c_void_p),
                ('dot_w', C.c_void_p), ('dot_b', C.c_void_p), ('dot_out', C.c_void_p)]


def _dp(t):
    return None if t is None else t.data_ptr()


class Src:

    def __init__(self, x, scale=None, shift=None, relu=False, pool=False, res=None, off=(0, 0), view=None):
        assert x.dtype in (torch.bfloat16, torch.float16, torch.float32) and x.is_contiguous()
        assert res is None or res.dtype == x.dtype
        self.x, self.scale, self.shift, self.relu, self.pool, self.res, self.off = x, scale, shift, relu, pool, res, off
        if view is None:
            assert x.dim() == 4
            self.N, self.Hs, self.Ws, self.Cc = x.shape
            self.ptr_off, self.row_stride = 0, 0
        else:
            self.ptr_off, self.Hs, self.Ws, self.Cc, self.row_stride = view
            self.N = x.shape[0]

    @property
    def f16(self):
        return {torch.bfloat16: 0, torch.float16: 1, torch.float32: 2}[self.x.dtype]

    @property
    def f32(self):
        return self.x.dtype == torch.float32

    @property
    def C(self):
        return self.Cc

    def ptr(self):
        return self.x.data_ptr() + self.x.element_size() * self.ptr_off

    def logical_hw(self):
        h, w = self.Hs, self.Ws
        if self.pool:
            c = 1 if int(self.pool) == 2 else 0
            return ((h + c) // 2, (w + c) // 2)
        return (h, w)

    def fill(self, cs):
        cs.x = self.ptr()
        cs.res = _dp(self.res)
        cs.scale, cs.shift = _dp(self.scale), _dp(self.shift)
        cs.C, cs.Hs, cs.Ws = self.C, self.Hs, self.Ws
        cs.pool, cs.relu = int(self.pool), int(self.relu)
        cs.off_y, cs.off_x = self.off
        cs.f16 = int(self.f16)
        cs.row_stride = int(self.row_stride)


_SUPPORTED = {(16, 16, 32), (16, 16, 64), (16, 32, 32), (16, 32, 64), (16, 32, 128), (16, 64, 64),
              (8, 32, 64), (8, 32, 128), (8, 64, 64)}


def choose_cfg(src_channels, Cout, H, W, override=None, taps=9, transposed=False, N=16, f32=False):
    if f32:
        assert all(c % 16 == 0 for c in src_channels), src_channels
        assert override is None or (tuple(override)[1] == 16 and tuple(override) in ((16, 16, 64), (16, 16, 32), (8, 16, 64))), \
            'fp32 precision: configuration override %s is not one of the fp32 kernels' % (override,)
        if override is not None:
            return tuple(override)
        small = min(H, W) <= 8 or (min(H, W) <= 16 and N <= 32)
        if small and Cout > 32:
            if os.environ.get('CDNET_F32_WS16', '1') == '1' and taps == 9 and not transposed and H == 16 and W == 16 and \
                    sum(src_channels) >= 256 and Cout >= 256 and 8 <= N <= 32:
                return (16, 16, 32)
            return (8, 16, 64)
        return (16, 16, 64 if Cout > 32 else 32)
    if override is not None:
        assert tuple(override) in _SUPPORTED, override
        return tuple(override)
    ctot = sum(src_channels)
    small = min(H, W) <= 8 or (min(H, W) <= 16 and N <= 32)
    ck = 64
    while any(c % ck for c in src_channels):
        ck //= 2
    assert ck >= 16, 'source channels must be multiples of 16: %s' % (src_channels,)
    if small:
        ws16 = taps == 9 and not transposed and H % 16 == 0 and W % 16 == 0 and min(H, W) == 16 and ctot % 64 == 0 and 256 <= ctot <= 768
        if ck >= 32 and not ws16:
            return (8, 32, 64)
    if ck == 64:
        ck = 32
    bn = 64 if Cout > 32 else 32
    if ck >= 16:
        ck = 16
    if ck == 16 and bn > 64:
        bn = 64
    return (16, ck, bn)


def dominant_kernel_name(precision, tiles=16):
    if precision == 'fp32':
        return 'conv_ws32_kernel<64,0,false>'
    quad = tiles * 256 * 256 * (64 + 64) * 2 >= (512 << 20)
    return 'conv_ws16_kernel<64,0,false,false,0,4,4,true,false,true,%s>' % ('true' if quad else 'false')


def packed_elems(Cout, nchunk, taps, CK, BN, npar):
    return _lib.load().cdnet_conv_packed_weight_elems(Cout, nchunk, taps, CK, BN, npar)


def _pack_dims(w, cfg, mode):
    _, CK, BN = cfg[:3]
    if mode == 0:
        Cout, Cin, KH, KW = w.shape
    elif mode == 1:
        Cin, Cout, KH, KW = w.shape
    elif mode in (4, 5, 6):
        Cout, ct, KH, KW = w.shape
        Cin = 4 * ct
    elif mode == 7:
        Cin, ct, KH, KW = w.shape
        Cout = 4 * ct
    else:
        Cin, Cout, KH, KW = w.shape
    taps = {2: 4, 3: 1, 4: 9, 5: 1, 6: 9, 7: 9}.get(mode, KH * KW)
    npar = 4 if mode in (2, 3) else 1
    return Cout, Cin, KH, KW, CK, BN, taps, npar


class PackJob(C.Structure):
    _fields_ = [('w', C.c_void_p), ('packed', C.c_void_p), ('Cout', C.c_int), ('Cin', C.c_int), ('KH', C.c_int), ('KW', C.c_int),
                ('CK', C.c_int), ('BN', C.c_int), ('mode', C.c_int), ('pad_', C.c_int)]


def pack_job(w, cfg, mode, out, split=False):
    Cout, Cin, KH, KW, CK, BN, taps, npar = _pack_dims(w, cfg, mode)
    assert out.numel() == packed_elems(Cout, Cin // CK, taps, CK, BN, npar) * (2 if split else 1)
    j = PackJob()
    j.w, j.packed, j.Cout, j.Cin, j.KH, j.KW, j.CK, j.BN = w.data_ptr(), out.data_ptr(), Cout, Cin, KH, KW, CK, BN
    j.mode = mode | (PACK_SPLIT if split else 0)
    return j


PACK_SPLIT = 16


def pack_weights(w, cfg, mode, Cin_pad=None, out=None, split=False, cout_scale=None):
    assert w.dtype == torch.float32 and w.is_cuda and w.is_contiguous()
    Cout, Cin, KH, KW, CK, BN, taps, npar = _pack_dims(w, cfg, mode)
    Cin_p = Cin if Cin_pad is None else Cin_pad
    if Cin_p != Cin:
        if mode == 0:
            wp = torch.zeros((Cout, Cin_p, KH, KW), dtype=torch.float32, device=w.device)
            wp[:, :Cin] = w
        else:
            raise NotImplementedError
        w, Cin = wp.contiguous(), Cin_p
    n = packed_elems(Cout, Cin // CK, taps, CK, BN, npar) * (2 if split else 1)
    if out is None or out.numel() != n:
        out = torch.empty((n,), dtype=torch.int16, device=w.device)
    if cout_scale is not None:
        assert mode == 0 and cout_scale.dtype == torch.float32 and cout_scale.numel() == Cout
        _lib.call('cdnet_pack_conv_weights_scaled', _lib.ptr(w), _lib.ptr(cout_scale), _lib.ptr(out), Cout, Cin, KH, KW, CK, BN,
                  mode | (PACK_SPLIT if split else 0), _lib.stream_ptr())
        return out
    _lib.call('cdnet_pack_conv_weights', _lib.ptr(w), _lib.ptr(out), Cout, Cin, KH, KW, CK, BN, mode | (PACK_SPLIT if split else 0),
              _lib.stream_ptr())
    return out


CONV_DEBUG = 0


def conv_forward(srcs, wpacked, Cout, cfg, taps=9, transposed=False, bias=None, oscale=None, oshift=None,
                 orelu=False, out=None, stats=None, H=None, W=None, out_dtype=torch.bfloat16, eres=None, query_ws=False, bns=None, taps1=0, pool_out=None, dot=None,
                 pad_chunks=0, debug_or=0):
    tile, CK, BN = cfg[:3]
    s0 = srcs[0]
    f32 = s0.f32
    assert all(s.f32 == f32 for s in srcs)
    if f32:
        out_dtype = torch.float32
    N = s0.N
    if H is None:
        H, W = s0.logical_hw()
        H, W = H + 0, W + 0
    ostride = 2 if transposed else 1
    npar = 4 if transposed else 1
    a = ConvArgs()
    nchunk = 0
    for i, s in enumerate(srcs):
        assert s.C % CK == 0, (s.C, CK)
        s.fill(a.src[i])
        nchunk += s.C // CK
    a.nsrc = len(srcs)
    if dot is not None:
        assert out is None and stats is None and eres is None and bns is None and pool_out is None and not f32 and not transposed
        a.dot_w, a.dot_b, a.dot_out = dot[0].data_ptr(), dot[1].data_ptr(), dot[2].data_ptr()
        assert dot[0].numel() == Cout and dot[0].dtype == torch.float32 and dot[2].dtype == torch.float32 and dot[2].numel() == N * H * W
    elif out is None:
        out = torch.empty((N, H * ostride, W * ostride, Cout), dtype=out_dtype, device=s0.x.device)
    ntiles = ((H + tile - 1) // tile) * ((W + tile - 1) // tile)
    if stats is True:
        stats = torch.empty((N * npar * ntiles, 2, Cout), dtype=torch.float32, device=s0.x.device)
    a.w, a.bias, a.oscale, a.oshift = _dp(wpacked), _dp(bias), _dp(oscale), _dp(oshift)
    a.orelu = int(orelu)
    a.out, a.Cout, a.out_cstride, a.out_coff = (None if out is None else out.data_ptr()), Cout, (Cout if out is None else out.shape[3]), 0
    a.stats = _dp(stats)
    a.N, a.H, a.W = N, H, W
    assert pad_chunks == 0 or (len(srcs) == 2 and taps == 9 and not f32 and all(s.scale is None and not s.relu and s.res is None and not s.f16 for s in srcs))
    a.taps, a.npar, a.ostride, a.nchunk = taps, npar, ostride, nchunk + pad_chunks
    a.tile, a.CK, a.BN = tile, CK, BN
    a.out_f16 = int(out is not None and out.dtype == torch.float16)
    a.ws = 0
    a.taps1 = taps1
    a.pool_out = _dp(pool_out)
    a.debug = CONV_DEBUG | debug_or
    a.f32 = int(f32)
    assert out is None or (out.dtype == torch.float32) == f32
    if eres is not None:
        assert not transposed and stats is None and not orelu and out.dtype == (torch.float32 if f32 else torch.bfloat16) and tuple(eres.x.shape) == tuple(out.shape)
        assert eres.f32 == f32
        a.eres, a.eres_scale, a.eres_shift = eres.x.data_ptr(), _dp(eres.scale), _dp(eres.shift)
        a.eres_f16, a.eres_relu = int(eres.f16), int(eres.relu)
    if bns is not None:
        raw, sc, sh, mu, inv, partial = bns
        assert eres is None and stats is None and bias is None and oscale is None and oshift is None and tuple(raw.shape) == tuple(out.shape)
        a.ws = 2
        a.eres, a.oscale, a.oshift, a.eres_scale, a.eres_shift, a.stats = raw.data_ptr(), sc.data_ptr(), sh.data_ptr(), mu.data_ptr(), inv.data_ptr(), partial.data_ptr()
    if query_ws:
        return int(_lib.load().cdnet_conv_ws_eligible(C.byref(a)))
    _lib.call('cdnet_conv_forward', C.byref(a), _lib.stream_ptr())
    return out, stats
```

### cdnet_amd/runtime.py

```python
import ctypes as C
import weakref
import torch

from . import _lib, engine
from .engine import Src

BN_EPS = 1e-5
BN_MOMENTUM = 0.1

import os as _os

PRECISION = _os.environ.get('CDNET_PRECISION', 'bf16')
assert PRECISION in ('bf16', 'fp32'), PRECISION


def set_precision(p):
    global PRECISION
    assert p in ('bf16', 'fp32'), p
    if p != PRECISION:
        PRECISION = p
        WEIGHTS_EPOCH[0] += 1


def act_dtype():
    return torch.float32 if PRECISION == 'fp32' else torch.bfloat16


def raw_dtype():
    return torch.float32 if PRECISION == 'fp32' else torch.float16


DEBUG_NORELU = False
TAPE = None
WEIGHTS_EPOCH = [0]
LAYERS = weakref.WeakSet()


class HeadFeat(C.Structure):
    _fields_ = [('raw', C.c_void_p), ('res', C.c_void_p), ('scale', C.c_void_p), ('shift', C.c_void_p),
                ('relu', C.c_int), ('f16', C.c_int)]


def head_feat(s):
    assert not s.pool and s.off == (0, 0) and s.C == 64
    f = HeadFeat()
    f.raw, f.res = s.x.data_ptr(), (None if s.res is None else s.res.data_ptr())
    f.scale = None if s.scale is None else s.scale.data_ptr()
    f.shift = None if s.shift is None else s.shift.data_ptr()
    f.relu = int(s.relu)
    f.f16 = int(s.f16)
    return f


class ConvLayer:

    def __init__(self, name, kind, weight, bias=None, bn=None, cfg_override=None):
        assert kind in ('conv3', 'conv1', 'convT4', 'convT2', 'conv3s2')
        self.name, self.kind, self.weight, self.bias, self.bn = name, kind, weight, bias, bn
        self.cfg_override = cfg_override
        if kind == 'conv3s2':
            self.Cout, self.Cin = weight.shape[0], 4 * weight.shape[1]
        elif kind in ('conv3', 'conv1'):
            self.Cout, self.Cin = weight.shape[0], weight.shape[1]
        else:
            self.Cin, self.Cout = weight.shape[0], weight.shape[1]
        self.taps = {'conv3': 9, 'conv1': 1, 'convT4': 4, 'convT2': 1, 'conv3s2': 9}[kind]
        self.transposed = kind in ('convT4', 'convT2')
        self.pack_mode = {'conv3': 0, 'conv1': 0, 'convT4': 2, 'convT2': 3, 'conv3s2': 6}[kind]
        self.cfg = None
        self.cfg_f32 = False
        self.wp = None
        self.wp_version = None
        self.fold = None
        self.fold_version = None
        dev = weight.device
        if bn is not None:
            self.scale = torch.empty((self.Cout,), dtype=torch.float32, device=dev)
            self.shift = torch.empty((self.Cout,), dtype=torch.float32, device=dev)
            self.save_mean = torch.empty((self.Cout,), dtype=torch.float32, device=dev)
            self.save_invstd = torch.empty((self.Cout,), dtype=torch.float32, device=dev)
        self.stats = None
        self.saved = None
        self.node_relu, self.node_res = True, None
        self.needs_input_grad = True
        self.bias_grad_from = None
        self.wpb, self.wpb_version, self.cfg_bwd = None, None, None
        self.wp_padded = False
        LAYERS.add(self)

    def _version(self):
        v = self.weight._version
        if self.bias is not None:
            v = (v, self.bias._version)
        return v

    def prepare(self, src_channels, H, W, N=16):
        cin_total = sum(src_channels)
        f32 = PRECISION == 'fp32'
        if self.cfg is None or self.cfg_f32 != f32:
            self.cfg = engine.choose_cfg(src_channels, self.Cout, H, W, self.cfg_override, taps=self.taps, transposed=self.transposed, N=N,
                                         f32=f32)
            self.cfg_f32, self.wp, self.cfg_bwd, self.wpb = f32, None, None, None
        ver = (self.weight._version, WEIGHTS_EPOCH[0])
        if self.wp is None or self.wp_version != ver:
            pad = cin_total if cin_total != self.Cin else None
            self.wp_padded = pad is not None
            self.wp = engine.pack_weights(self.weight.detach(), self.cfg, self.pack_mode, Cin_pad=pad, out=self.wp, split=f32)
            self.wp_version = ver

    def backward_pack(self, cin_total, H, W):
        ver = (self.weight._version, WEIGHTS_EPOCH[0])
        f32 = self.cfg_f32
        if self.cfg_bwd is None:
            if self.transposed:
                self.cfg_bwd = engine.choose_cfg([2 * self.Cout, 2 * self.Cout], self.Cin, H, W, taps=(9 if self.kind == 'convT4' else 1), f32=f32)
            else:
                self.cfg_bwd = engine.choose_cfg([self.Cout], cin_total, H, W, taps=self.taps, f32=f32)
        if self.wpb is None or self.wpb_version != ver:
            if self.transposed:
                mode = 4 if self.kind == 'convT4' else 5
                self.wpb = engine.pack_weights(self.weight.detach(), self.cfg_bwd, mode, out=self.wpb, split=f32)
            else:
                assert cin_total == self.Cin, 'the RGB stem never needs an input gradient'
                self.wpb = engine.pack_weights(self.weight.detach(), self.cfg_bwd, 7 if self.kind == 'conv3s2' else 1, out=self.wpb, split=f32)
            self.wpb_version = ver
        return self.wpb, self.cfg_bwd

    def eval_fold(self):
        bn = self.bn
        ver = (bn.weight._version, bn.bias._version, bn.running_mean._version, bn.running_var._version,
               None if self.bias is None else self.bias._version, WEIGHTS_EPOCH[0])
        if self.fold is None or self.fold_version != ver:
            if self.fold is None:
                self.fold = (torch.empty_like(self.scale), torch.empty_like(self.shift))
            _lib.call('cdnet_bn_fold_eval', _lib.ptr(bn.weight.detach()), _lib.ptr(bn.bias.detach()),
                      _lib.ptr(bn.running_mean), _lib.ptr(bn.running_var),
                      None if self.bias is None else _lib.ptr(self.bias.detach()), BN_EPS, self.Cout,
                      _lib.ptr(self.fold[0]), _lib.ptr(self.fold[1]), _lib.stream_ptr())
            self.fold_version = ver
        return self.fold

    def eval_pack(self, src_channels, allow_f32=False):
        if not EVAL_FOLD_WEIGHTS or not getattr(self, 'fold_eval', True) or self.kind not in ('conv3', 'conv1') or self.bn is None:
            return None
        f32 = PRECISION == 'fp32'
        if f32 and not allow_f32:
            return None
        cin_total = sum(src_channels)
        pad = cin_total if cin_total != self.Cin else None
        sc, sh = self.eval_fold()
        ver = (self.weight._version, self.fold_version, WEIGHTS_EPOCH[0], tuple(self.cfg), f32)
        if getattr(self, 'wpe', None) is None or self.wpe_version != ver:
            self.wpe = engine.pack_weights(self.weight.detach(), self.cfg, 0, Cin_pad=pad, out=getattr(self, 'wpe', None), cout_scale=sc, split=f32)
            self.wpe_version = ver
        return self.wpe, sh

    def forward_eval_swapped(self, srcs, relu=True, H=None, W=None):
        if PRECISION != 'bf16' or self.kind != 'conv3' or self.bn is None or len(srcs) != 2 or not EVAL_FOLD_WEIGHTS or not getattr(self, 'fold_eval', True):
            return None
        a, b = srcs
        if (a.C // 16) % 2 == 0 or (b.C // 16) % 2 or a.C % 16 or b.C % 16 or a.C + b.C != self.Cin:
            return None
        if any(s.scale is not None or s.relu or s.res is not None or s.f16 or s.pool for s in srcs):
            return None
        if H is None:
            H, W = b.logical_hw()
        if H % 16 or W % 16:
            return None
        self.prepare([s.C for s in srcs], H, W, a.N)
        if tuple(self.cfg[:2]) != (16, 16):
            return None
        sc, sh = self.eval_fold()
        ver = (self.weight._version, self.fold_version, WEIGHTS_EPOCH[0], tuple(self.cfg), a.C)
        if getattr(self, 'wps', None) is None or self.wps_version != ver:
            w = self.weight.detach()
            wz = torch.zeros((w.shape[0], 16, w.shape[2], w.shape[3]), dtype=w.dtype, device=w.device)
            wperm = torch.cat([w[:, a.C:], w[:, :a.C], wz], 1).contiguous()
            self.wps = engine.pack_weights(wperm, self.cfg, 0, cout_scale=sc)
            self.wps_version = ver
        kw = dict(oshift=sh, orelu=relu and not DEBUG_NORELU, H=H, W=W, pad_chunks=1)
        key = (a.N, H, W, a.C, b.C, a.off, b.off, engine.CONV_DEBUG, PRECISION)
        elig = self.__dict__.setdefault('_swapped_eligible', {})
        if key not in elig:
            elig[key] = engine.conv_forward([b, a], self.wps, self.Cout, self.cfg, 9, query_ws=True, **kw) == 2
        if not elig[key]:
            return None
        out, _ = engine.conv_forward([b, a], self.wps, self.Cout, self.cfg, 9, **kw)
        return Src(out)

    def forward_eval_pool(self, srcs):
        H, W = srcs[0].logical_hw()
        if PRECISION == 'bf16' and H % 2 == 0 and W % 2 == 0:
            self.prepare([s.C for s in srcs], H, W, srcs[0].N)
            ep = self.eval_pack([s.C for s in srcs])
            if ep is not None:
                N = srcs[0].N
                out = torch.empty((N, H, W, self.Cout), dtype=torch.bfloat16, device=srcs[0].x.device)
                pout = torch.empty((N, H // 2, W // 2, self.Cout), dtype=torch.bfloat16, device=srcs[0].x.device)
                kw = dict(oshift=ep[1], orelu=True, H=H, W=W, out=out, pool_out=pout)
                if engine.conv_forward(srcs, ep[0], self.Cout, self.cfg, self.taps, self.transposed, query_ws=True, **kw) == 2:
                    engine.conv_forward(srcs, ep[0], self.Cout, self.cfg, self.taps, self.transposed, **kw)
                    return Src(out), Src(pout)
        if PRECISION == 'fp32' and H % 2 == 0 and W % 2 == 0 and self.bn is not None and not DEBUG_NORELU:
            self.prepare([s.C for s in srcs], H, W, srcs[0].N)
            sc, sh = self.eval_fold()
            N = srcs[0].N
            out = torch.empty((N, H, W, self.Cout), dtype=torch.float32, device=srcs[0].x.device)
            pout = torch.empty((N, H // 2, W // 2, self.Cout), dtype=torch.float32, device=srcs[0].x.device)
            kw = dict(oscale=sc, oshift=sh, orelu=True, H=H, W=W, out=out, pool_out=pout)
            if engine.conv_forward(srcs, self.wp, self.Cout, self.cfg, self.taps, self.transposed, query_ws=True, **kw) == 1:
                engine.conv_forward(srcs, self.wp, self.Cout, self.cfg, self.taps, self.transposed, **kw)
                return Src(out), Src(pout)
        return self.forward(srcs, False), None

    def forward(self, srcs, training, relu=True, H=None, W=None, out_dtype=None, eres=None, debug_or=0):
        if PRECISION == 'fp32':
            out_dtype = torch.float32
        elif out_dtype is None:
            out_dtype = torch.bfloat16
        if H is None:
            H, W = srcs[0].logical_hw()
        if DEBUG_NORELU:
            relu = False
        self.prepare([s.C for s in srcs], H, W, srcs[0].N)
        bias = None if self.bias is None else self.bias.detach()
        if self.bn is None:
            out, _ = engine.conv_forward(srcs, self.wp, self.Cout, self.cfg, self.taps, self.transposed, bias=bias, H=H, W=W,
                                         out_dtype=out_dtype, eres=eres)
            if training:
                self.saved = (srcs, out, H, W)
                self.node_relu, self.node_res = False, None
                if TAPE is not None:
                    TAPE.append(self)
            return Src(out)
        if not training:
            ep = self.eval_pack([s.C for s in srcs])
            if ep is not None:
                out, _ = engine.conv_forward(srcs, ep[0], self.Cout, self.cfg, self.taps, self.transposed, oshift=ep[1],
                                             orelu=relu and eres is None, H=H, W=W, out_dtype=out_dtype, eres=eres, debug_or=debug_or)
                return Src(out)
            sc, sh = self.eval_fold()
            out, _ = engine.conv_forward(srcs, self.wp, self.Cout, self.cfg, self.taps, self.transposed, oscale=sc,
                                         oshift=sh, orelu=relu and eres is None, H=H, W=W, out_dtype=out_dtype, eres=eres, debug_or=debug_or)
            return Src(out)
        tile = self.cfg[0]
        N = srcs[0].N
        npar = 4 if self.transposed else 1
        T = N * npar * ((H + tile - 1) // tile) * ((W + tile - 1) // tile)
        if self.stats is None or self.stats.shape[0] != T:
            self.stats = torch.empty((T, 2, self.Cout), dtype=torch.float32, device=self.weight.device)
        raw, _ = engine.conv_forward(srcs, self.wp, self.Cout, self.cfg, self.taps, self.transposed, stats=self.stats,
                                     H=H, W=W, out_dtype=raw_dtype())
        count = float(N * H * W * npar)
        bn = self.bn
        _lib.call('cdnet_bn_finalize_train', _lib.ptr(self.stats), T, self.Cout, count, _lib.ptr(bn.weight.detach()),
                  _lib.ptr(bn.bias.detach()), None if bias is None else _lib.ptr(bias), BN_EPS,
                  BN_MOMENTUM if getattr(bn, 'momentum', None) is None else float(bn.momentum),
                  _lib.ptr(bn.running_mean), _lib.ptr(bn.running_var), _lib.ptr(self.scale), _lib.ptr(self.shift),
                  _lib.ptr(self.save_mean), _lib.ptr(self.save_invstd), _lib.stream_ptr())
        self.saved = (srcs, raw, H, W)
        self.node_relu, self.node_res = relu, None
        self.fold_version = None
        if TAPE is not None:
            TAPE.append(self)
        return Src(raw, self.scale, self.shift, relu=relu)


class FuseTerm(C.Structure):
    _fields_ = [('x', C.c_void_p), ('Hs', C.c_int), ('Ws', C.c_int), ('scale', C.c_void_p), ('shift', C.c_void_p),
                ('f16', C.c_int), ('pad_', C.c_int)]


class GradTerm(C.Structure):
    _fields_ = [('g', C.c_void_p), ('cstride', C.c_int), ('coff', C.c_int)]


class FuseNode:

    def __init__(self, name):
        self.name = name
        self.saved = None

    def forward(self, terms, relu, out=None, out_coff=0, training=False):
        for t in terms:
            assert t.res is None and not t.pool and not t.relu and t.row_stride == 0 and t.x.is_contiguous()
        N, Cc = terms[0].N, terms[0].C
        H, W = (max(t.Hs for t in terms), max(t.Ws for t in terms)) if out is None else (out.shape[1], out.shape[2])
        arr = (FuseTerm * len(terms))()
        for k, t in enumerate(terms):
            assert t.C == Cc
            arr[k].x, arr[k].Hs, arr[k].Ws = t.x.data_ptr(), t.Hs, t.Ws
            arr[k].scale, arr[k].shift = (None if t.scale is None else t.scale.data_ptr()), (None if t.shift is None else t.shift.data_ptr())
            arr[k].f16 = int(t.f16)
        f32 = terms[0].f32
        assert all(t.f32 == f32 for t in terms)
        if out is None:
            o, cs = torch.empty((N, H, W, Cc), dtype=torch.float32 if f32 else torch.bfloat16, device=terms[0].x.device), Cc
        else:
            o, cs = out, out.shape[3]
        assert (o.dtype == torch.float32) == f32
        if DEBUG_NORELU:
            relu = False
        _lib.call(_lib.entry('cdnet_fuse_sum', f32), C.byref(arr), len(terms), N, H, W, Cc, int(relu), _lib.ptr(o), cs, out_coff,
                  _lib.stream_ptr())
        if training:
            self.saved = (list(terms), o, relu, H, W, Cc, out_coff)
            if TAPE is not None:
                TAPE.append(self)
        return Src(o) if out is None else None

    def backward(self, tr, grads, add):
        terms, o, relu, H, W, Cc, coff = self.saved
        sliced = o.shape[3] != Cc
        if sliced:
            d, dcs, dco = tr.cat_grad(o, grads), o.shape[3], coff
            if d is None:
                return
        else:
            gl = tr.take(grads, id(o))
            if gl is None:
                return
            if relu and self._residual_tail(tr, grads, gl, terms, o, H, W, Cc):
                return
            if relu or len(gl) > 1 or gl[0].coff or gl[0].cstride not in (0, Cc):
                d = tr.buf(('dfuse', self.name), o.shape, o.dtype)
                tr.grad_sum(gl, o if relu else None, o.shape[0] * H * W, Cc, d)
            else:
                d = gl[0].t
            dcs, dco = 0, 0
        N = o.shape[0]
        for k, t in enumerate(terms):
            if t.Hs == H and t.Ws == W:
                add(t.x, tr.G(d, H, W, coff=dco, cstride=dcs))
            else:
                din = tr.buf(('dup', self.name, k), (N, t.Hs, t.Ws, Cc), d.dtype)
                _lib.call(_lib.entry('cdnet_upsample_bilinear_backward', d.dtype == torch.float32), _lib.ptr(d),
                          N, H, W, Cc, dcs, dco, t.Hs, t.Ws, _lib.ptr(din), _lib.stream_ptr())
                add(t.x, tr.G(din, t.Hs, t.Ws))


def _residual_tail(self, tr, grads, gl, terms, o, H, W, Cc):
    if DEBUG_NORELU:
        return False
    if len(terms) == 1:
        y = terms[0]
        P = tr._producer.get(id(y.x)) if y.scale is not None else None
        if P is None or P.bn is None or getattr(P, 'node_res', None) is not None or tr._readers.get(id(y.x), 0) != 1 or id(y.x) in grads \
                or tuple(y.x.shape) != tuple(o.shape) or getattr(P, 'fused_res_of', None) is not None or (y.Hs, y.Ws) != (H, W):
            return False
        P.node_relu, P.node_res = True, None
        grads[id(y.x)] = gl
        return True
    if len(terms) != 2 or len(gl) > 3:
        return False
    bn_t = [t for t in terms if t.scale is not None]
    if not bn_t or any((t.Hs, t.Ws) != (H, W) for t in terms):
        return False
    y = max(bn_t, key=lambda t: tr._tape_pos.get(id(tr._producer.get(id(t.x))), -1))
    x = terms[1] if terms[0] is y else terms[0]
    P = tr._producer.get(id(y.x))
    if P is None or P.bn is None or getattr(P, 'node_res', None) is not None or tr._readers.get(id(y.x), 0) != 1 or id(y.x) in grads \
            or tuple(y.x.shape) != tuple(o.shape) or getattr(P, 'fused_res_of', None) is not None:
        return False
    if any(g.pooled or g.oy or g.ox or (g.Hg, g.Wg) != (H, W) for g in gl):
        return False
    P.node_relu, P.node_res, P.node_res_grad_to = 2, o, x.x
    grads[id(y.x)] = gl
    return True


FuseNode._residual_tail = _residual_tail


def input_pack(x):
    assert x.dtype == torch.float32 and x.is_cuda and x.dim() == 4
    x = x.contiguous()
    N, Cc, H, W = x.shape
    out = torch.empty((N, H, W, 16), dtype=act_dtype(), device=x.device)
    _lib.call(_lib.entry('cdnet_input_pack', PRECISION == 'fp32'), _lib.ptr(x), N, Cc, H, W, _lib.ptr(out),
              _lib.stream_ptr())
    return out


POOL_MATERIALIZE = True
RU_MATERIALIZE = True
RU_FUSE = True
EVAL_FOLD_WEIGHTS = True
RU_EVAL_ONE_LAUNCH = True
RU_EVAL_POINT_DOT = True


class PointLogit:

    def __init__(self, point):
        self.point = point


def residual_unit_eval(c1, c2, cr, x, relu2=True, dot=None):
    if not (RU_EVAL_ONE_LAUNCH and EVAL_FOLD_WEIGHTS) or not getattr(c2, 'fold_eval', True) or x.pool or x.C % 16 or c2.Cout % 16:
        return None
    H, W = x.logical_hw()
    if H % 16 or W % 16 or x.C != cr.Cin:
        return None
    c2.prepare([c2.Cin], H, W, x.N)
    if tuple(c2.cfg[:2]) != (16, 16):
        return None
    ep = c2.eval_pack([c1.Cout], allow_f32=True)
    if ep is None:
        return None
    f32 = PRECISION == 'fp32'
    rver = (cr.weight._version, WEIGHTS_EPOCH[0], tuple(c2.cfg), f32)
    if getattr(c2, 'ru_wr', None) is None or c2.ru_wr_version != rver:
        c2.ru_wr = engine.pack_weights(cr.weight.detach(), c2.cfg, 0, out=getattr(c2, 'ru_wr', None), split=f32)
        c2.ru_wr_version = rver
    pad = 1 if (not f32 and (x.C // 16) % 2 == 1 and c2.cfg[1] == 16) else 0
    ver = (c2.wpe_version, rver, None if cr.bias is None else cr.bias._version, PRECISION, pad)
    if getattr(c2, 'ru_pack', None) is None or c2.ru_pack_version != ver:
        BN = c2.cfg[2]
        ntile = -(-c2.Cout // BN)
        a, b = ep[0].view(ntile, -1), c2.ru_wr.view(ntile, -1)
        parts = [a, b]
        if pad:
            parts.append(torch.zeros((ntile, 16 * BN), dtype=a.dtype, device=a.device))
        c2.ru_pack = torch.cat(parts, 1).contiguous().view(-1)
        c2.ru_shift = ep[1] if cr.bias is None else ep[1] + cr.bias.detach()
        c2.ru_pack_version = ver
    hC = c1.Cout
    keep = engine.CONV_DEBUG
    elig = c2.__dict__.setdefault('_ru_eligible', {})
# ... 46 lines not shown
```

### cdnet_amd/trainer.py

```python
import ctypes as C
import os

import torch

from . import _lib, engine, optim, runtime, streams
from .allreduce import BucketReducer, bucketed_allreduce
from .engine import Src
from .optim import HEAD_PARAMS, FlatState
from .synth import synthetic_batch


class GradIn(C.Structure):
    _fields_ = [('g', C.c_void_p), ('Hg', C.c_int), ('Wg', C.c_int), ('oy', C.c_int), ('ox', C.c_int),
                ('pooled', C.c_int), ('coff', C.c_int), ('cstride', C.c_int), ('pad_', C.c_int)]


class BnBwdArgs(C.Structure):
    _fields_ = [('raw', C.c_void_p), ('res', C.c_void_p), ('scale', C.c_void_p), ('shift', C.c_void_p),
                ('mean', C.c_void_p), ('invstd', C.c_void_p), ('gin', GradIn * 3), ('ngin', C.c_int),
                ('f16', C.c_int), ('relu', C.c_int), ('N', C.c_int), ('H', C.c_int), ('W', C.c_int), ('C', C.c_int)]


_WGRAD_WGS_DEEP, _WGRAD_WGS_SHALLOW = 128, 160
_WGRAD_WGS_KQ = 128
# ... 259 lines not shown
                    or hasattr(f, 'grad_to') or tuple(f.off) != (0, 0) or f.C != 64:
                return None
        owner = None
        for Lt in self.tape:
            if isinstance(Lt, runtime.FuseNode):
                if any(t.x is f3.x for t in Lt.saved[0]):
                    return None
                continue
            if any(sx.x is f3.x or sx.res is f3.x for sx in Lt.saved[0]):
                return None
            if Lt.saved[1] is f3.x:
                owner = getattr(Lt, 'fused_res_of', None) if Lt.kind == 'conv1' else None
        if owner is None or owner.bn is None or getattr(owner, 'node_relu', True) != 2 or getattr(owner, 'node_res', None) is not f3.x \
                or owner.saved[1].dtype != torch.float32 or tuple(owner.saved[1].shape) != tuple(f3.x.shape):
            return None
        return owner

    def _classifier_backward(self, key, f, conv, dl):
        N, H, W, _ = f.x.shape
        K = conv.out_channels
        df = self.buf(key, (N, H, W, 64), runtime.act_dtype())
        ws = self._ws('slab', _lib.load().cdnet_final_conv1x1_backward_workspace_floats(), side=True)
        hf = runtime.head_feat(f)
        w = conv.weight.detach().reshape(K, 64)
        _lib.call('cdnet_final_conv1x1_backward', C.byref(hf), _lib.ptr(w), _lib.ptr(dl), K, N, H, W, _lib.ptr(df), _lib.ptr(ws),
                  ws.numel(), _lib.ptr(conv.weight.grad), _lib.ptr(conv.bias.grad), _lib.stream_ptr())
        return _G(df, H, W)

    def _run_tape(self, heads, params):
        grads = {}

        def add(t, g):
            grads.setdefault(id(t), []).append(g)
        for t, g in heads:
            add(t, g)
        self._overlap_begin()
        self._overlap_done(params)
        self._backward_tape(grads, add)

    def _backward_tape(self, grads, add):
        self._cat_cache = {}
        self._rd_pending, self._rd_params, self._rd_bytes = [], [], 0
        if len(self._rd_tables) > 16:
            self._rd_tables.clear()
        self._readers, self._producer, self._bn_partials = {}, {}, {}
        self._tape_pos = {id(Lt): k for k, Lt in enumerate(self.tape)}
        for Lt in self.tape:
            if isinstance(Lt, runtime.FuseNode):
                for t in Lt.saved[0]:
                    self._readers[id(t.x)] = self._readers.get(id(t.x), 0) + 1
                continue
            for sx in Lt.saved[0]:
                self._readers[id(sx.x)] = self._readers.get(id(sx.x), 0) + 1
                if sx.res is not None:
                    self._readers[id(sx.res)] = self._readers.get(id(sx.res), 0) + 1
            self._producer[id(Lt.saved[1])] = Lt
        side = self._side_stream()
        self._side_active = side is not None
        if self._packb_pending:
            torch.cuda.current_stream().wait_event(self._event('packb'))
            self._packb_pending = False
        for k, L in enumerate(reversed(self.tape)):
            if isinstance(L, runtime.FuseNode):
                L.backward(self, grads, add)
                continue
            gl = self.take(grads, id(L.saved[1]))
            if gl is None:
                continue
            owner = getattr(L, 'fused_res_of', None)
            if owner is not None:
                grads.setdefault(id(owner.saved[1]), []).extend(gl)
                owner.deferred_layer = L
                continue
            self._layer_backward(k, L, gl, grads, add, side)
            d = getattr(L, 'deferred_layer', None)
            if d is not None:
                L.deferred_layer = None
                self._layer_backward(('deferred', k), d, self.take(grads, id(d.saved[1])), grads, add, side)
        if side is not None:
            with _on_stream(side):
                self._flush_reduces()
            ev = self._event(-1)
            ev.record(side)
            torch.cuda.current_stream().wait_event(ev)
        else:
            self._flush_reduces()

    def _weights_done(self, params):
        if not self._rd_pending:
            self._overlap_done(params)
            return
        self._rd_params.append(params)
        if self._rd_bytes >= self._rd_mb * (1 << 20):
            self._flush_reduces()

    def _flush_reduces(self):
        if self._rd_pending:
            key = tuple(self._rd_pending)
            tab = self._rd_tables.get(key)
            if tab is None:
                lib = _lib.load()
                descs = (_lib.WgradReduceDesc * len(key))()
                b0 = 0
                for i, a in enumerate(key):
                    _lib.call('cdnet_wgrad_reduce_desc_fill', *a, b0, C.byref(descs[i]))
                    b0 += descs[i].blocks
                dev_tab = torch.frombuffer(bytearray(bytes(descs)), dtype=torch.uint8).to(self.dev)
                tab = self._rd_tables[key] = (dev_tab, len(key), b0)
            _lib.call('cdnet_wgrad_reduce_batch', _lib.ptr(tab[0]), tab[1], tab[2], _lib.stream_ptr())
        for params in self._rd_params:
            self._overlap_done(params)
        self._rd_pending, self._rd_params, self._rd_bytes = [], [], 0

    def _layer_backward(self, k, L, gl, grads, add, side):
        srcs, out, Hl, Wl = L.saved
        No, Ho, Wo, Co = out.shape
        params = (L.weight, L.bias, None if L.bn is None else L.bn.weight, None if L.bn is None else L.bn.bias)
        part = self._bn_partials.pop(id(out), None)
        if len(gl) == 1 and gl[0].masked:
            g = self._bn_backward_masked(L, out, gl[0], add)
        elif part is not None:
            assert len(gl) == 1, (L.name, len(gl))
            a, ktab = self._bn_backward_stats(L, out, gl[0], partial=part)
            g = self.buf(('draw', L.name), (No, Ho, Wo, Co), runtime.act_dtype())
            _lib.call('cdnet_bn_backward_apply', C.byref(a), _lib.ptr(ktab), _lib.ptr(g), _lib.stream_ptr())
        elif L.bn is not None or len(gl) > 1 or gl[0].pooled or gl[0].coff or (gl[0].cstride not in (0, Co)):
            g = self._bn_backward(L, out, gl, add)
        else:
            g = gl[0].t
        if side is None:
            self._weight_backward(L, srcs, g, Hl, Wl)
            self._weights_done(params)
            self._input_backward(L, srcs, g, Hl, Wl, add)
        else:
            ev = self._event(k)
            ev.record()
            beside = _RU_1X1_SIDE and L.kind == 'conv1' and isinstance(k, tuple) and getattr(L, 'needs_input_grad', True)
            if not beside:
                self._input_backward(L, srcs, g, Hl, Wl, add)
            side.wait_event(ev)
            with _on_stream(side):
                if beside:
                    ev2 = self._event(('beside', k))

                    def add_beside(tgt, g_):
                        g_.event = ev2
                        add(tgt, g_)
                    self._input_backward(L, srcs, g, Hl, Wl, add_beside)
                    ev2.record()
                self._weight_backward(L, srcs, g, Hl, Wl)
                self._weights_done(params)

    def _bn_backward_stats(self, L, out, g, partial):
        a = self._bn_args(L, out, [_G(g.t, g.Hg, g.Wg)], res=None, relu=1)
        ktab = self.buf(('ktab', L.name), (7, out.shape[3]), torch.float32)
        bn = L.bn
        _lib.call('cdnet_bn_backward_finalize', C.byref(a), _lib.ptr(bn.weight.detach()), _lib.ptr(bn.weight.grad), _lib.ptr(bn.bias.grad),
                  _lib.ptr(partial), partial.shape[0], _lib.ptr(ktab), _lib.stream_ptr())
        return a, ktab

    def _bn_backward_masked(self, L, out, g, add):
        No, Ho, Wo, Co = out.shape
        a = self._bn_args(L, out, [_G(g.t, g.Hg, g.Wg)], res=None, relu=0)
        draw = self.buf(('draw', L.name), (No, Ho, Wo, Co), runtime.act_dtype())
        ws = self._ws('bn', _lib.load().cdnet_bn_backward_workspace_floats(Co))
        bn = L.bn
        _lib.call('cdnet_bn_backward', C.byref(a), _lib.ptr(bn.weight.detach()), _lib.ptr(bn.weight.grad), _lib.ptr(bn.bias.grad),
                  _lib.ptr(ws), ws.numel(), _lib.ptr(draw), None, _lib.stream_ptr())
        add(L.node_res, _G(g.t, Ho, Wo))
        return draw

    def _stats_fusable(self, L, srcs, H, W, N, wpb, cfgb, cin_total):
        f32 = runtime.PRECISION == 'fp32'
        if not f32 or os.environ.get('CDNET_BN_STATS_FUSE', '1') != '1' or getattr(runtime, 'DEBUG_NORELU', False):
            return None
        if L.kind != 'conv3' or L.transposed or len(srcs) != 1:
            return None
        sx = srcs[0]
        if getattr(sx, 'is_input', False) or sx.scale is None or sx.shift is None or sx.relu is not True or sx.res is not None or sx.pool \
                or tuple(sx.off) != (0, 0) or sx.x.dtype != runtime.raw_dtype() or hasattr(sx, 'grad_to') or sx.row_stride:
            return None
        if f32 and cin_total % 64:
            return None
        P = self._producer.get(id(sx.x))
        if P is None or P.bn is None or getattr(P, 'node_res', None) is not None or getattr(P, 'node_relu', True) is not True \
                or self._readers.get(id(sx.x), 0) != 1 or tuple(sx.x.shape) != (N, H, W, cin_total):
            return None
        key = ('statsfusable', L.name, N, H, W, runtime.PRECISION)
        hit = self._bufs.get(key)
        if hit is None:
            part = torch.zeros((1024, 2, cin_total), dtype=torch.float32, device=self.dev)
            gin = self.buf(('din', L.name), (N, H, W, cin_total), runtime.act_dtype())
            gdummy = self.buf(('draw', L.name), (N, H, W, L.Cout), runtime.act_dtype())
            ok = engine.conv_forward([Src(gdummy)], wpb, cin_total, cfgb, taps=L.taps, out=gin, H=H, W=W, query_ws=True,
                                     bns=(sx.x, P.scale, P.shift, P.save_mean, P.save_invstd, part))
            hit = self._bufs[key] = (part if ok else False)
        if hit is False:
            return None
        return P, hit

    def _bn_args(self, L, out, gl, res, relu):
        a = BnBwdArgs()
        a.raw = out.data_ptr()
        a.res = None if res is None else res.data_ptr()
        if L.bn is not None:
            a.scale, a.shift = L.scale.data_ptr(), L.shift.data_ptr()
            a.mean, a.invstd = L.save_mean.data_ptr(), L.save_invstd.data_ptr()
        a.ngin = len(gl)
        assert 1 <= len(gl) <= 3, (L.name, len(gl))
        for k, g in enumerate(gl):
            a.gin[k].g = g.t.data_ptr()
            a.gin[k].Hg, a.gin[k].Wg, a.gin[k].oy, a.gin[k].ox = g.Hg, g.Wg, g.oy, g.ox
            a.gin[k].pooled, a.gin[k].coff, a.gin[k].cstride = int(g.pooled), g.coff, g.cstride or out.shape[3]
        a.f16 = {torch.bfloat16: 0, torch.float16: 1, torch.float32: 2}[out.dtype]
        a.relu = relu
        a.N, a.H, a.W, a.C = out.shape
        return a

    def _bn_backward(self, L, out, gl, add):
        No, Ho, Wo, Co = out.shape
        res = getattr(L, 'node_res', None)
        has_bn = L.bn is not None
        if len(gl) > 3:
            plain = [g for g in gl if not g.pooled and g.oy == 0 and g.ox == 0 and (g.Hg, g.Wg) == (Ho, Wo)]
            rest = [g for g in gl if g not in plain]
            assert len(rest) <= 2 and len(plain) >= 2, (L.name, len(gl))
            d = self.buf(('gsum', L.name), (No, Ho, Wo, Co), runtime.act_dtype())
            self.grad_sum(plain, None, No * Ho * Wo, Co, d)
            gl = rest + [_G(d, Ho, Wo)]
        a = self._bn_args(L, out, gl, res, int(getattr(L, 'node_relu', True)))
        draw = self.buf(('draw', L.name), (No, Ho, Wo, Co), runtime.act_dtype())
        dz = None
        if res is not None:
            dz = self.buf(('dz', L.name), (No, Ho, Wo, Co), runtime.act_dtype())
        ws = self._ws('bn', _lib.load().cdnet_bn_backward_workspace_floats(Co))
        bn = L.bn
        _lib.call('cdnet_bn_backward', C.byref(a), _lib.ptr(bn.weight.detach()) if has_bn else None,
                  _lib.ptr(bn.weight.grad) if has_bn else None, _lib.ptr(bn.bias.grad) if has_bn else None,
                  _lib.ptr(ws), ws.numel(), _lib.ptr(draw), _lib.ptr(dz), _lib.stream_ptr())
        if res is not None:
            add(getattr(L, 'node_res_grad_to', None) if getattr(L, 'node_res_grad_to', None) is not None else res, _G(dz, Ho, Wo))
            L.node_res_grad_to = None
        return draw

    def _side_stream(self):
        if not WGRAD_STREAM or self.dev.type != 'cuda':
            return None
        if self._wstream is None:
            self._wstream = streams.side_stream(self.dev)
            self._events = {}
        return self._wstream

    def _event(self, k):
        e = self._events.get(k)
        if e is None:
            e = self._events[k] = torch.cuda.Event()
        return e

    def _weight_backward(self, L, srcs, g, H, W):
        lib = _lib.load()
        N = g.shape[0]
        Cout = L.Cout
        cin_total = sum(s.C for s in srcs)
        cin_real = L.Cin
        mode = {'conv3': 0, 'conv1': 0, 'convT4': 2, 'convT2': 3, 'conv3s2': 6}[L.kind]
        taps, npar, ostride = L.taps, (4 if L.transposed else 1), (2 if L.transposed else 1)
        cap = _wgrad_wgs(self._side_active and getattr(L, 'needs_input_grad', True), H * W, Cout)
        coff = 0
        for s in srcs:
            ci_t = _choose_ci_tiles(s.C, Cout)
            CI, CO = ci_t * 32, (4 // ci_t) * 32
            other = -(-s.C // CI) * -(-Cout // CO) * npar
            ntiles = N * (-(-H // 8)) * (-(-W // 16))
            ksplit = max(1, min(ntiles, cap // other if other < cap else 1))
            nslab = lib.cdnet_conv_wgrad_slab_floats(s.C, Cout, taps, npar, ci_t, ksplit)
            defer = self._rd_mb > 0
            slab = self.buf(('wslab', L.name, coff), (nslab,), torch.float32) if defer else self._ws('slab', nslab, side=True)
            cs = engine.ConvSrc()
            s.fill(cs)
            csrc_real = min(s.C, cin_real - coff) if cin_total != cin_real else s.C
            _lib.call('cdnet_conv_backward_weight', C.byref(cs), coff, csrc_real, cin_real, _lib.ptr(g), Cout, N, H, W, taps,
                      npar, ostride, ci_t, ksplit, _lib.ptr(slab), _lib.ptr(L.weight.grad), mode | (_WGRAD_DEFER if defer else 0),
                      _lib.stream_ptr())
            if defer:
                self._rd_pending.append((s.C, coff, csrc_real, cin_real, Cout, taps, npar, ci_t, ksplit, slab.data_ptr(),
                                         L.weight.grad.data_ptr(), mode))
                self._rd_bytes += nslab * 4
            coff += s.C
        if L.bias is not None and L.bn is None:
            owner = getattr(L, 'bias_grad_from', None)
            if owner is not None:
                L.bias.grad.copy_(owner.bn.bias.grad)
            else:
                ws = self._ws('slab', lib.cdnet_bias_grad_workspace_floats(Cout), side=True)
                _lib.call(_lib.entry('cdnet_bias_grad', g.dtype == torch.float32), _lib.ptr(g), g.numel() // Cout, Cout,
                          _lib.ptr(ws), ws.numel(), _lib.ptr(L.bias.grad), _lib.stream_ptr())

    def _input_backward(self, L, srcs, g, H, W, add):
        if not getattr(L, 'needs_input_grad', True):
            return
        N = g.N if isinstance(g, Src) else g.shape[0]
        Cout = L.Cout
        cin_total = sum(s.C for s in srcs)
        wpb, cfgb = L.backward_pack(cin_total, H, W)
        if L.kind == 'conv3s2':
            Cp = cin_total // 4
            gs2d = self.buf(('ds2d', L.name), (N, H, W, cin_total), runtime.act_dtype())
            engine.conv_forward([Src(g)], wpb, cin_total, cfgb, taps=9, out=gs2d, H=H, W=W)
            gin = self.buf(('din', L.name), (N, 2 * H, 2 * W, Cp), runtime.act_dtype())
            _lib.call(_lib.entry('cdnet_s2d_to_nhwc', gin.dtype == torch.float32), _lib.ptr(gs2d), N, H, W, Cp, _lib.ptr(gin),
                      _lib.stream_ptr())
            add(srcs[0].x, _G(gin, 2 * H, 2 * W))
            return
        if not L.transposed:
            gin = self.buf(('din', L.name), (N, H, W, cin_total), runtime.act_dtype())
            fuse = None if isinstance(g, Src) else self._stats_fusable(L, srcs, H, W, N, wpb, cfgb, cin_total)
            if fuse is not None:
                P, part = fuse
                engine.conv_forward([Src(g)], wpb, cin_total, cfgb, taps=L.taps, out=gin, H=H, W=W,
                                    bns=(srcs[0].x, P.scale, P.shift, P.save_mean, P.save_invstd, part))
                self._bn_partials[id(srcs[0].x)] = part
            else:
                engine.conv_forward([g if isinstance(g, Src) else Src(g)], wpb, cin_total, cfgb, taps=L.taps, out=gin, H=H, W=W)
        else:
            gin = self.buf(('din', L.name), (N, H, W, cin_total), runtime.act_dtype())
            views = [Src(g, view=(a * 2 * W * Cout, H, W, 2 * Cout, 4 * W * Cout)) for a in (0, 1)]
            engine.conv_forward(views, wpb, cin_total, cfgb, taps=(9 if L.kind == 'convT4' else 1), out=gin, H=H, W=W)
        coff = 0
        for s in srcs:
            if getattr(s, 'is_input', False):
                coff += s.C
                continue
            tgt, pool = getattr(s, 'grad_to', (s.x, int(s.pool)))
            add(tgt, _G(gin, H, W, oy=s.off[0], ox=s.off[1], pooled=pool, coff=coff, cstride=cin_total))
            coff += s.C

    def _overlap_begin(self):
        self._ar = None
        if not self._reduce_active() or os.environ.get('CDNET_ALLREDUCE_OVERLAP', '1') == '0':
            return
        f = self.flat
        base = f.G.data_ptr()
        pend = {}
        owners = [p for L in self.tape if not isinstance(L, runtime.FuseNode) for p in (L.weight, L.bias, None if L.bn is None else L.bn.weight,
                                                 None if L.bn is None else L.bn.bias) if p is not None]
        for p in owners:
            off = (p.grad.data_ptr() - base) // 4
            if 0 <= off < f.n_used:
                pend[off] = off + p.numel()
        if f.n_head:
            pend[0] = f.n_head
        self._ar = BucketReducer(f.G, f.n_used, self.bucket, pend)

    def _overlap_done(self, params):
        if self._ar is None:
            return
        if params is None:
            self._ar.done([0])
        else:
            base = self.flat.G.data_ptr()
            self._ar.done([(p.grad.data_ptr() - base) // 4 for p in params if p is not None])

    def _reduce_active(self):
        return self.world > 1 or os.environ.get('CDNET_FORCE_ALLREDUCE', '0') == '1'

    def allreduce_and_step(self):
        f = self.flat
        gscale = 1.0
        works = None
        if self._reduce_active():
            if self._ar is not None:
                ranges = self._ar.finish(wait=False)
                works = self._ar.works
                self.ar_stats = dict(buckets=len(works), released_during_backward=self._ar.early)
                self._ar = None
            else:
                bucketed_allreduce(f.G, f.n_used, self.bucket)
            gscale = 1.0 / self.world
        f.step_count += 1
        step = self._rule_stepper(gscale)
        if works is None:
            step(0, f.n_used)
        else:
            for w, (a, b) in zip(works, ranges):
                w.wait()
                step(a, b)
        runtime.WEIGHTS_EPOCH[0] += 1
        self._repack_all()

    def _rule_stepper(self, gscale):
        return optim.stepper(self, gscale)

    def _repack_all(self):
        f = self.flat
        lo, hi = f.P.data_ptr(), f.P.data_ptr() + f.P.numel() * 4
        if self._pack_jobs is not None and self._pack_prec != runtime.PRECISION:
            self._pack_jobs = None
        if self._pack_jobs is None:
            groups = ([], []), ([], [])
            for L in runtime.LAYERS:
                if not (lo <= L.weight.data_ptr() < hi):
                    continue
                w = L.weight.detach()
                if L.wp is not None and not L.wp_padded:
                    groups[0][0].append(engine.pack_job(w, L.cfg, L.pack_mode, L.wp, split=L.cfg_f32)); groups[0][1].append((L, 'wp_version'))
                if L.wpb is not None:
                    mode = (4 if L.kind == 'convT4' else 5) if L.transposed else (7 if L.kind == 'conv3s2' else 1)
                    groups[1][0].append(engine.pack_job(w, L.cfg_bwd, mode, L.wpb, split=L.cfg_f32)); groups[1][1].append((L, 'wpb_version'))
            if not groups[0][0] or not groups[1][0] or self.flat.step_count < 1:
                return
            self._pack_jobs = []
            self._pack_prec = runtime.PRECISION
            for jobs, owners in groups:
                arr = (engine.PackJob * len(jobs))(*jobs)
                nbytes = _lib.load().cdnet_pack_batch_table_bytes(len(jobs))
                table = torch.empty((nbytes,), dtype=torch.uint8, device=f.P.device)
                self._pack_jobs.append((arr, len(jobs), table, owners, [True]))
        side = self._side_stream()
        for k, (arr, n, table, owners, first) in enumerate(self._pack_jobs):
            if k == 1 and side is not None and self._packb_stream:
                ev = self._event('adam')
                ev.record()
                side.wait_event(ev)
                with _on_stream(side):
                    _lib.call('cdnet_pack_conv_weights_batch', C.byref(arr), n, _lib.ptr(table), table.numel(), int(first[0]), _lib.stream_ptr())
                    self._event('packb').record()
                self._packb_pending = True
            else:
                _lib.call('cdnet_pack_conv_weights_batch', C.byref(arr), n, _lib.ptr(table), table.numel(), int(first[0]), _lib.stream_ptr())
            first[0] = False
            for L, attr in owners:
                setattr(L, attr, (L.weight._version, runtime.WEIGHTS_EPOCH[0]))

    def write_bn_counters(self):
        with torch.no_grad():
            unused = tuple(getattr(self.model, 'UNUSED_PREFIXES', ()))
            for name, mod in self.model.named_modules():
                if isinstance(mod, torch.nn.BatchNorm2d) and mod.num_batches_tracked is not None and not (name + '.').startswith(unused or ('\0',)):
                    mod.num_batches_tracked.fill_(self._bn_base + self._forwards)

    def refresh_parameters(self):
        if hasattr(self.model, 'sync_real_parameters') and getattr(self.model, '_rt', None) is not None:
            self.model._ensure_runtime()
        runtime.WEIGHTS_EPOCH[0] += 1

    def state_dict(self):
        return optim.state_dict(self)

    def load_state_dict(self, sd):
        optim.load_state_dict(self, sd)

    def train_step(self, x, label, dirlab, point_t, weight):
        mask, point, direction = self.forward(x)
        dmask, dpoint, ddir = self.loss_and_grads(mask, point, direction, label, dirlab, point_t, weight)
        self.backward(dmask, dpoint, ddir)
        self.allreduce_and_step()
        return self.losses


class UNetTrainer(Trainer):

    def __init__(self, model, **kw):
        super().__init__(model, **kw)
        self.unet_losses = torch.zeros((3,), dtype=torch.float32, device=self.dev)

    def loss_and_grads(self, logits, label, weight):
        B, K, H, W = logits.shape
        assert K == 3, 'the fused loss serves the 3-class configuration (options.py: out_c = 3)'
        z = lambda shape, dt: self.buf(('zero',) + tuple(shape) + (dt,), shape, dt)
        point, dirn = z((B, 1, H, W), torch.float32), z((B, 9, H, W), torch.float32)
        dirlab, point_t = z((B, H, W), torch.uint8), z((B, H, W), torch.float16)
        for t in (point, dirn, dirlab, point_t):
            t.zero_()
        dmask, _, _ = super().loss_and_grads(logits, point, dirn, label, dirlab, point_t, weight)
        self.unet_losses[1:3] = self.losses[4:6]
        self.unet_losses[0] = self.losses[4] + self.losses[5]
        if self.alpha:
            self.unet_losses[0] += self.loss_var[0]
        if self.boundary:
            self.unet_losses[0] += self.loss_boundary[0]
        return dmask

    def backward(self, dlogits):
        conv, feat = self.model.final_conv, self.model._last_feat
        self._run_tape([(feat.x, self._classifier_backward('dF', feat, conv, dlogits))], [conv.weight, conv.bias])

    def train_step(self, x, label, weight):
        logits = self.forward(x)
        dlogits = self.loss_and_grads(logits, label, weight)
        self.backward(dlogits)
        self.allreduce_and_step()
        return self.unet_losses


class AblationTrainer(Trainer):

    def __init__(self, model, **kw):
        assert getattr(model, 'VARIANT', 'rev1') in ('MandD', 'MandDandP') and model.DIRECTION_OUT in (5, 9, 17), \
            'AblationTrainer serves model_unet_MandD / MandD4 / MandD16 / MandDandP'
        super().__init__(model, **kw)

    def loss_and_grads(self, outputs, label, dirlab, point_t, weight):
        if len(outputs) == 3:
            return super().loss_and_grads(outputs[0], outputs[1], outputs[2], label, dirlab, point_t, weight)
        mask, direction = outputs
        B, _, H, W = mask.shape
        point = self.buf('zero_point', (B, 1, H, W), torch.float32)
        pt = self.buf('zero_point_t', (B, H, W), torch.float16)
        point.zero_()
        pt.zero_()
        dmask, _, ddir = super().loss_and_grads(mask, point, direction, label, dirlab, pt, weight)
        return dmask, None, ddir

    def backward(self, dmask, dpoint, ddir):
        m = self.model
        f1m, f2, f3 = m._last_feats
        heads, params = [], []
        for name, f, conv, dl in (('m', f1m, m.mask_conv, dmask), ('d', f2, m.direction_conv, ddir), ('p', f3, m.point_conv, dpoint)):
            if f is None or dl is None:
                continue
            heads.append((getattr(f, 'grad_to', (f.x,))[0], self._classifier_backward('dF' + name, f, conv, dl)))
            params += [conv.weight, conv.bias]
        self._run_tape(heads, params)

    def train_step(self, x, label, dirlab, point_t, weight):
        out = self.forward(x)
        g = self.loss_and_grads(out, label, dirlab, point_t, weight)
        self.backward(*g)
        self.allreduce_and_step()
        return self.losses


def make_bench_step(model, B, dev, rank, world):
    tr = Trainer(model, world_size=world)
    batch = synthetic_batch(B, dev, seed=2022 + rank)

    def step():
        return tr.train_step(*batch)
    metric = 'tiles/sec (train fwd+bwd+Adam), 256x256'
    workload = ('CDNet UNet2RevA1_vgg16 (UNet+DAM) training step: forward, 5-term loss, backward%s, %s fused Adam; '
                '256x256x3 synthetic tiles, batch %d per GPU' % ('', 'RCCL gradient all-reduce,' if world > 1 else '', B))
    return step, metric, workload
```

### include/cdnet_hip.h

```cpp
#ifndef CDNET_HIP_H
#define CDNET_HIP_H

#include <stddef.h>
#include <stdint.h>

#ifdef __cplusplus
extern "C" {
#endif

#define CDNET_OK            0
#define CDNET_E_ARG         1
#define CDNET_E_WORKSPACE   2
#define CDNET_E_LAUNCH      3

#define CDNET_ABI_VERSION   5

int         cdnet_abi_version(void);
size_t      cdnet_abi_sizeof(const char *struct_name);
const char *cdnet_last_error(void);
const char *cdnet_build_info(void);
int         cdnet_spin(int microseconds, void *stream);
int         cdnet_box_copy(const void *src, void *dst, size_t bytes, void *stream);
int         cdnet_box_mfma(const uint32_t *seed, float *sink, unsigned long long *stamps, int workgroups, int waves_per_wg, int iters, void *stream);

size_t cdnet_tile_postproc_workspace_bytes(int B, int C, int H, int W);
int cdnet_tile_postproc(const float *mask_logits, const float *dir_logits, const float *point, int B, int C, int H, int W,
                        const int8_t *lut_host, int nbr, int extra_zero, int min_area, int radius, void *workspace, size_t workspace_bytes,
                        float *prob, uint8_t *dcm, int32_t *minmax, uint8_t *pred, uint8_t *fill, uint8_t *small, int32_t *label,
                        int32_t *final_, int32_t *counts, void *stream);

int cdnet_ddm_codes(const uint8_t *dcm, int N, int H, int W, int classes, const int8_t *lut_host, int nbr,
                    int extra_zero, uint8_t *code, int32_t *minmax, void *stream);
int cdnet_ddm_normalize(const uint8_t *code, const int32_t *minmax, int N, int H, int W, float *out,
                        void *stream);

int cdnet_probmaps(const float *mask_logits, const float *dir_logits, int N, int C, int H, int W,
                   float *prob, uint8_t *dcm, void *stream);

int cdnet_tta_boost_argmax(const float *probs, const float *points, const uint8_t *codes, const int32_t *minmax,
                           int I, int V, const int *view_xform_host, int H, int W,
                           float *prob_mean, float *point_mean, uint8_t *ddm16, uint8_t *pred,
                           float *pmax_ws, void *stream);

size_t cdnet_watershed_workspace_bytes(int N, int H, int W);
int cdnet_watershed_process(const uint8_t *pred, int N, int H, int W, int min_size, void *workspace, size_t workspace_bytes,
                            uint8_t *dist, int32_t *marker, int32_t *labels, void *stream);
int cdnet_fill_label_process(const uint8_t *pred, int N, int H, int W, int min_size, void *workspace, size_t workspace_bytes,
                             int32_t *labels, void *stream);

size_t cdnet_cc_workspace_bytes(int N, int H, int W);
int cdnet_cc_chain(const uint8_t *pred, int fg_value, int N, int H, int W, int min_area, int radius,
                   void *workspace, size_t workspace_bytes,
                   uint8_t *fill, uint8_t *small, int32_t *label, int32_t *final_, int32_t *counts,
                   void *stream);

int cdnet_mask_views_argmax(const float *logits, int I, int V, int K, const int *view_xform_host, int H, int W, float *prob_mean,
                            uint8_t *pred, void *stream);
size_t cdnet_tile_mask_postproc_workspace_bytes(int B, int K, int H, int W);
int cdnet_tile_mask_postproc(const float *logits, int B, int K, int H, int W, int min_area, int radius, void *workspace, size_t workspace_bytes,
                             float *prob, uint8_t *pred, uint8_t *fill, uint8_t *small, int32_t *label, int32_t *final_, int32_t *counts,
                             void *stream);
int cdnet_dilate_labels(const int32_t *label, int N, int H, int W, int radius, int32_t *out, void *stream);


typedef struct cdnet_conv_src {
    const uint16_t *x;
    const uint16_t *res;
    const float *scale;
    const float *shift;
    int C;
    int Hs, Ws;
    int pool;
    int relu;
    int off_y, off_x;
    int f16;
    int row_stride;
} cdnet_conv_src;

typedef struct cdnet_conv_args {
    cdnet_conv_src src[2];
    int nsrc;
    const uint16_t *w;
    const float *bias;
    const float *oscale;
    const float *oshift;
    int orelu;
    uint16_t *out;
    int Cout, out_cstride, out_coff;
    float *stats;
    int N, H, W;
    int taps;
    int npar;
    int ostride;
    int nchunk;
    int tile, CK, BN;
    int out_f16;
    int debug;
    int ws;
    int f32;
    const uint16_t *eres;
    const float *eres_scale, *eres_shift;
    int eres_f16, eres_relu;
    int taps1;
    int pad_;
    uint16_t *pool_out;
    const float *dot_w;
    const float *dot_b;
    float *dot_out;
} cdnet_conv_args;

size_t cdnet_conv_packed_weight_elems(int Cout, int nchunk, int taps, int CK, int BN, int npar);
#define CDNET_PACK_SPLIT 16
int cdnet_pack_conv_weights(const float *w, void *packed, int Cout, int Cin, int KH, int KW, int CK, int BN, int mode,
                            void *stream);
int cdnet_pack_conv_weights_scaled(const float *w, const float *cout_scale, void *packed, int Cout, int Cin, int KH, int KW, int CK,
                                   int BN, int mode, void *stream);
typedef struct cdnet_pack_job {
    const float *w;
    void *packed;
    int Cout, Cin, KH, KW, CK, BN, mode, pad_;
} cdnet_pack_job;
size_t cdnet_pack_batch_table_bytes(int n_jobs);
int cdnet_pack_conv_weights_batch(const cdnet_pack_job *jobs, int n_jobs, void *table, size_t table_bytes, int upload,
                                  void *stream);
int cdnet_conv_forward(const cdnet_conv_args *args, void *stream);

int cdnet_input_pack(const float *x, int N, int C, int H, int W, void *out_bf16_nhwc16, void *stream);
int cdnet_input_pack_f32(const float *x, int N, int C, int H, int W, float *out_f32_nhwc16, void *stream);
int cdnet_bn_fold_eval(const float *gamma, const float *beta, const float *running_mean, const float *running_var,
                       const float *conv_bias, float eps, int C, float *scale, float *shift, void *stream);
int cdnet_bn_finalize_train(const float *stats, int T, int C, float count, const float *gamma, const float *beta,
                            const float *conv_bias, float eps, float momentum, float *running_mean,
                            float *running_var, float *scale, float *shift, float *save_mean, float *save_invstd,
                            void *stream);

typedef struct cdnet_head_feat {
    const uint16_t *raw;
    const uint16_t *res;
    const float *scale;
    const float *shift;
    int relu;
    int f16;
} cdnet_head_feat;

#define CDNET_HEAD_WEIGHT_FLOATS 855
int cdnet_dam_head_forward(const cdnet_head_feat *f1, const cdnet_head_feat *f2, const cdnet_head_feat *f3,
                           const float *head_weights, int N, int H, int W, float *mask, float *point,
                           float *direction, void *stream);
int cdnet_final_conv1x1(const cdnet_head_feat *f, const float *w, const float *b, int K, int N, int H, int W,
                        float *out, void *stream);
size_t cdnet_bias_grad_workspace_floats(int C);
int cdnet_bias_grad(const uint16_t *grad_out, size_t npix, int C, float *workspace, size_t workspace_floats, float *db, void *stream);
int cdnet_bias_grad_f32(const float *grad_out, size_t npix, int C, float *workspace, size_t workspace_floats, float *db, void *stream);
size_t cdnet_final_conv1x1_backward_workspace_floats(void);
int cdnet_final_conv1x1_backward(const cdnet_head_feat *f, const float *w, const float *dlogits, int K, int N, int H, int W,
                                 uint16_t *df, float *workspace, size_t workspace_floats, float *dw, float *db, void *stream);

int cdnet_conv_ws_eligible(const cdnet_conv_args *args);

int cdnet_src_materialize(const cdnet_conv_src *src, int N, int H, int W, uint16_t *out, void *stream);

size_t cdnet_conv_wgrad_slab_floats(int C_src, int Cout, int taps, int npar, int ci_tiles, int ksplit);
int cdnet_conv_backward_weight(const cdnet_conv_src *src, int src_coff, int Csrc_real, int Cin_real,
                               const uint16_t *grad_out, int Cout, int N, int H, int W, int taps, int npar,
                               int ostride, int ci_tiles, int ksplit, float *slab, float *dw, int mode, void *stream);

#define CDNET_WGRAD_DEFER_REDUCE 0x100
typedef struct cdnet_wgrad_reduce_desc {
    const float *slab;
    float *dw;
    int ksplit, npar, ci_blocks, co_blocks, taps, CI, CO, Csrc_real, Cin_real, src_coff, Cout, mode;
    int block0, blocks;
} cdnet_wgrad_reduce_desc;
int cdnet_wgrad_reduce_desc_fill(int C_src, int src_coff, int Csrc_real, int Cin_real, int Cout, int taps, int npar, int ci_tiles,
                                 int ksplit, const float *slab, float *dw, int mode, int block0, cdnet_wgrad_reduce_desc *out);
int cdnet_wgrad_reduce_batch(const cdnet_wgrad_reduce_desc *table_dev, int n, int total_blocks, void *stream);

typedef struct cdnet_grad_in {
    const uint16_t *g;
    int Hg, Wg;
    int oy, ox;
    int pooled;
    int coff, cstride;
    int pad_;
} cdnet_grad_in;

typedef struct cdnet_bn_bwd_args {
    const uint16_t *raw;
    const uint16_t *res;
    const float *scale, *shift;
    const float *mean, *invstd;
    cdnet_grad_in gin[3];
    int ngin;
    int f16, relu;
    int N, H, W, C;
} cdnet_bn_bwd_args;

size_t cdnet_bn_backward_workspace_floats(int C);
int cdnet_bn_backward_stats(const cdnet_bn_bwd_args *args, const float *gamma, float *dgamma, float *dbeta, float *workspace,
                            size_t workspace_floats, float *ktab, void *stream);
int cdnet_bn_backward_apply(const cdnet_bn_bwd_args *args, const float *ktab, uint16_t *draw, void *stream);
int cdnet_bn_backward_finalize(const cdnet_bn_bwd_args *args, const float *gamma, float *dgamma, float *dbeta, const float *partial,
                               int nb, float *ktab, void *stream);
int cdnet_bn_backward(const cdnet_bn_bwd_args *args, const float *gamma, float *dgamma, float *dbeta, float *workspace,
                      size_t workspace_floats, uint16_t *draw, uint16_t *dz_out, void *stream);

size_t cdnet_dam_head_backward_workspace_floats(int N, int H, int W);
int cdnet_dam_head_backward(const cdnet_head_feat *f1, const cdnet_head_feat *f2, const cdnet_head_feat *f3,
                            const float *head_weights, const float *dmask, const float *dpoint, const float *ddir,
                            int N, int H, int W, uint16_t *df1, uint16_t *df2, uint16_t *df3, float *workspace,
                            size_t workspace_floats, float *dhead_weights, void *stream);
int cdnet_dam_head_backward_fused_blocks(void);
int cdnet_dam_head_backward_fused_scratch_bytes(void);
size_t cdnet_dam_head_backward_fused_workspace_floats(void);
int cdnet_dam_head_backward_fused(const cdnet_head_feat *f1, const cdnet_head_feat *f2, const cdnet_head_feat *f3,
                                  const float *head_weights, const float *dmask, const float *dpoint, const float *ddir, int N, int H,
                                  int W, float *df1, float *df2, float *dz3, float *workspace, size_t workspace_floats,
                                  float *dhead_weights, void *stream);

size_t cdnet_dam_loss_workspace_floats(int B, int P);
int cdnet_dam_loss(const float *mask, const float *point, const float *direction, const uint8_t *label,
                   const uint8_t *dirlab, const uint16_t *point_target_f16, const uint8_t *weight_u8, int B, int H, int W,
                   int quirk_sample0, float *workspace, size_t workspace_floats, float *losses, float *dmask,
                   float *dpoint, float *ddir, void *stream);
size_t cdnet_dam_loss_classes_workspace_floats(int B, int P, int direction_classes);
int cdnet_dam_loss_classes(const float *mask, const float *point, const float *direction, const uint8_t *label,
                           const uint8_t *dirlab, const uint16_t *point_target_f16, const uint8_t *weight_u8, int B, int H, int W,
                           int direction_classes, int quirk_sample0, float *workspace, size_t workspace_floats, float *losses,
                           float *dmask, float *dpoint, float *ddir, void *stream);

size_t cdnet_variance_loss_workspace_bytes(int B, int K, int H, int W);
int cdnet_variance_loss(const float *mask_logits, const uint8_t *label, int fg_value, int B, int K, int H, int W, float alpha,
                        void *workspace, size_t workspace_bytes, float *loss_var, float *total, float *dmask, int32_t *root_out,
                        int32_t *counts, void *stream);

size_t cdnet_boundary_loss_workspace_bytes(int kind, int B, int K, int H, int W);
int cdnet_boundary_loss(const float *mask_logits, const uint8_t *label, int kind, int B, int K, int H, int W, float beta,
                        void *workspace, size_t workspace_bytes, float *loss_out, float *total, float *dmask, void *stream);
int cdnet_boundary_loss_scratch_bytes(void);

#define CDNET_VAL_SUMS 42
size_t cdnet_dam_val_sums_workspace_floats(int B, int P);
int cdnet_dam_val_sums(const float *mask, const float *point, const float *dirn, const uint8_t *label, const uint8_t *dirlab,
                       const uint16_t *point_target_f16, const uint8_t *weight_u8, const int *dir_rank_host, int B, int H, int W,
                       float *workspace, size_t workspace_floats, float *sums, void *stream);
size_t cdnet_dam_val_sums_classes_workspace_floats(int B, int P, int direction_classes);
int cdnet_dam_val_sums_classes(const float *mask, const float *point, const float *dirn, const uint8_t *label, const uint8_t *dirlab,
                               const uint16_t *point_target_f16, const uint8_t *weight_u8, const int *dir_rank_host,
                               int direction_classes, int B, int H, int W, float *workspace, size_t workspace_floats, float *sums,
                               void *stream);

int cdnet_adam_step(float *param, const float *grad, float *exp_avg, float *exp_avg_sq, size_t n, float lr, float beta1,
                    float beta2, float eps, float weight_decay, int step, float grad_scale, void *stream);

int cdnet_moment_step(float *param, const float *grad, float *exp_avg, float *exp_avg_sq, float *slow, size_t n, double beta1,
                      double beta2, float grad_scale, int move, int rect, float decay, float step_size, float v_div, float eps,
                      int sync, float alpha, void *stream);
int cdnet_sgd_step(float *param, const float *grad, float *momentum_buffer, size_t n, float lr, float momentum, float weight_decay,
                   int step, float grad_scale, void *stream);

int cdnet_window_pack(const float *img, int C, int H, int W, int view_xform, int tile_h, int tile_w, int stride, int ny,
                      int nx, void *out_bf16_nhwc16, void *stream);
int cdnet_window_pack_f32(const float *img, int C, int H, int W, int view_xform, int tile_h, int tile_w, int stride, int ny,
                          int nx, float *out_f32_nhwc16, void *stream);
int cdnet_window_stitch(const float *tiles, int K, int tile_h, int tile_w, int stride, int overlap, int ny, int nx, int Hv,
                        int Wv, float *out, void *stream);

typedef struct cdnet_aug_sample {
    double minv[6];
    const uint8_t *img;
    const uint8_t *weight;
    const void *label;
    int32_t H, W, img_stride, weight_stride, label_stride, label_i32;
    float color[4];
    int32_t hflip, vflip, filter, y0, x0;
    float alpha, sigma;
    uint32_t seed;
} cdnet_aug_sample;
size_t cdnet_augment_workspace_bytes(int B, int size, int max_radius);
int cdnet_augment_batch(const cdnet_aug_sample *samples, const cdnet_aug_sample *samples_host, int B, int size, const float *norm_host,
                        void *workspace, size_t workspace_bytes, float *image, uint8_t *weight, void *label, int label_i32, int32_t *varied,
                        float *field, void *stream);

size_t cdnet_label_encoding_workspace_bytes(int N, int H, int W, int max_instances);
int cdnet_label_encoding(const uint8_t *label_ch0, int N, int H, int W, int max_instances, const double *rays_host,
                         const double *gauss_host, void *workspace, size_t workspace_bytes, uint8_t *label3,
                         uint16_t *point_f16, uint8_t *direction, int32_t *inst_out, int32_t *counts_out, void *stream);
size_t cdnet_label_encoding_instances_workspace_bytes(int N, int H, int W, int max_instances);
int cdnet_label_encoding_instances(const int32_t *label_inst, int N, int H, int W, int max_instances, const double *rays_host,
                                   const double *gauss_host, void *workspace, size_t workspace_bytes, uint8_t *label3,
                                   uint16_t *point_f16, uint8_t *direction, int32_t *inst, int32_t *counts, void *stream);

typedef struct cdnet_fuse_term {
    const uint16_t *x;
    int Hs, Ws;
    const float *scale;
    const float *shift;
    int f16, pad_;
} cdnet_fuse_term;
int cdnet_fuse_sum(const cdnet_fuse_term *terms, int nterm, int N, int H, int W, int C, int relu, uint16_t *out, int out_cstride,
                   int out_coff, void *stream);

int cdnet_upsample_bilinear_backward(const uint16_t *dout, int N, int H, int W, int C, int dout_cstride, int dout_coff, int Hs, int Ws,
                                     uint16_t *din, void *stream);
int cdnet_s2d_to_nhwc(const uint16_t *in, int N, int H2, int W2, int C, uint16_t *out, void *stream);
int cdnet_fuse_sum_f32(const cdnet_fuse_term *terms, int nterm, int N, int H, int W, int C, int relu, float *out, int out_cstride,
                       int out_coff, void *stream);
int cdnet_upsample_bilinear_backward_f32(const float *dout, int N, int H, int W, int C, int dout_cstride, int dout_coff, int Hs, int Ws,
                                         float *din, void *stream);
int cdnet_s2d_to_nhwc_f32(const float *in, int N, int H2, int W2, int C, float *out, void *stream);

typedef struct cdnet_grad_term {
    const uint16_t *g;
    int cstride, coff;
} cdnet_grad_term;
int cdnet_grad_sum(const cdnet_grad_term *terms, int nterm, const uint16_t *mask, long long npix, int C, uint16_t *out, void *stream);
int cdnet_grad_sum_f32(const cdnet_grad_term *terms, int nterm, const float *mask, long long npix, int C, float *out, void *stream);

int cdnet_label_pair_histogram(const int32_t *true_lab, const int32_t *pred_lab, int N, int plane, int cap, int hash_slots,
                               int32_t *area_true, int32_t *area_pred, uint32_t *hash_keys, int32_t *hash_counts, int32_t *err_flag,
                               void *stream);
int cdnet_remap_label(const int32_t *lab, int N, int plane, int cap, int32_t *scratch, int32_t *out, int32_t *err_flag, void *stream);

#ifdef __cplusplus
}
#endif
#endif
```

Measured before the change: 1102.

## Use four-tap parity-chunk backward for fp32 convT4 and all-parity transposed forward

Adds a weight pack mode that splits the stride-2 4x4 transposed-conv input-gradient into four parity chunk groups of two-by-two taps. The fp32 conv kernel gets a chunk-parity form (4 taps instead of 9, which skips the structurally zero taps) and an all-parity form that computes all four output parities in one launch, reusing the staged input across parities. The Python runtime now selects the four-tap backward when Cin > 32 and the nine-tap path is not persistent. The all-parity form keeps four accumulator sets, which raises register and LDS pressure. The debug enum reuses the value 128 for the new flag, colliding with an existing one.

```diff
diff --git a/cdnet_amd/csrc/conv.hip b/cdnet_amd/csrc/conv.hip
--- a/cdnet_amd/csrc/conv.hip
+++ b/cdnet_amd/csrc/conv.hip
@@ -74,6 +74,9 @@
                 if (mode == 4) {
                     const int kh = 2 * (tap / 3) + a - 1, kw = 2 * (tap % 3) + b - 1;
                     if (kh >= 0 && kh < 4 && kw >= 0 && kw < 4) v = w[(((size_t)co * Ct + c) * 4 + kh) * 4 + kw];
+                } else if (mode == 8) {
+                    const int kh = 2 * ((a == 0) + (tap >> 1)) + a - 1, kw = 2 * ((b == 0) + (tap & 1)) + b - 1;
+                    v = w[(((size_t)co * Ct + c) * 4 + kh) * 4 + kw];
                 } else if (mode == 5) {
                     v = w[(((size_t)co * Ct + c) * 2 + a) * 2 + b];
                 } else {
@@ -1272,8 +1275,9 @@
     const int split = (mode & 16) ? 1 : 0;
     mode &= 15;
     CDNET_REQUIRE(w && packed, "%s: null pointer", who);
-    CDNET_REQUIRE(CK % 16 == 0 && BN % 32 == 0 && Cin % CK == 0 && mode >= 0 && mode <= 7, "%s: Cin=%d CK=%d BN=%d mode=%d", who, Cin, CK, BN, mode);
-    const int taps = mode == 2 ? 4 : (mode == 3 ? 1 : ((mode == 4 || mode == 6 || mode == 7) ? 9 : (mode == 5 ? 1 : KH * KW)));
+    CDNET_REQUIRE(CK % 16 == 0 && BN % 32 == 0 && Cin % CK == 0 && mode >= 0 && mode <= 8, "%s: Cin=%d CK=%d BN=%d mode=%d", who, Cin, CK, BN, mode);
+    CDNET_REQUIRE(mode != 8 || (Cin % 4 == 0 && (Cin / 4) % CK == 0), "%s: mode 8 needs out_channels = Cin / 4 = %d / 4 to be a multiple of CK = %d (a chunk must not straddle two parities)", who, Cin, CK);
+    const int taps = (mode == 2 || mode == 8) ? 4 : (mode == 3 ? 1 : ((mode == 4 || mode == 6 || mode == 7) ? 9 : (mode == 5 ? 1 : KH * KW)));
     const int nchunk = Cin / CK, ntile = cdiv(Cout, BN);
     const size_t per = (size_t)ntile * nchunk * taps * CK * BN * (split ? 2 : 1);
     d.split = split;
@@ -1376,9 +1380,12 @@
     const bool padded = A.nchunk == nchunk + 1 && A.taps == 9 && A.nsrc == 2 && !A.f32;
     CDNET_REQUIRE(nchunk == A.nchunk || padded, "cdnet_conv_forward: nchunk %d != %d", A.nchunk, nchunk);
     CDNET_REQUIRE((A.taps == 9 && A.npar == 1 && A.ostride == 1) || (A.taps == 1 && A.npar == 1 && A.ostride == 1) ||
-                  (A.taps == 4 && A.npar == 4 && A.ostride == 2) || (A.taps == 1 && A.npar == 4 && A.ostride == 2),
+                  (A.taps == 4 && A.npar == 4 && A.ostride == 2) || (A.taps == 1 && A.npar == 4 && A.ostride == 2) ||
+                  (A.taps == 4 && A.npar == 1 && A.ostride == 1 && A.f32 && A.par_chunks > 0),
                   "cdnet_conv_forward: taps=%d npar=%d ostride=%d", A.taps, A.npar, A.ostride);
     CDNET_REQUIRE(A.out_cstride % 8 == 0 && A.out_coff % 8 == 0, "cdnet_conv_forward: output channel slice must be 16-byte aligned");
+    CDNET_REQUIRE(A.par_chunks == 0 || (A.taps == 4 && A.npar == 1 && A.f32 && A.nchunk == 4 * A.par_chunks),
+                  "cdnet_conv_forward: par_chunks = %d belongs to fp32 launches with taps = 4, npar = 1 and nchunk = 4 * par_chunks", A.par_chunks);
     hipStream_t st = (hipStream_t)stream;
     CDNET_REQUIRE(A.taps1 == 0 || A.taps1 == A.taps || (A.taps1 == 1 && A.taps == 9 && A.nsrc == 2), "cdnet_conv_forward: taps1 = %d (0, taps, or 1 beside a nine-tap first source)", A.taps1);
     if (A.f32) return conv_forward_f32(A, st);
diff --git a/cdnet_amd/csrc/conv32.hip b/cdnet_amd/csrc/conv32.hip
--- a/cdnet_amd/csrc/conv32.hip
+++ b/cdnet_amd/csrc/conv32.hip
@@ -32,13 +32,13 @@
 constexpr int PSTR = CK * 2 + 16;
 constexpr int XF_MAX = 2048;
 
-template <int TH, int TW, int BN, int TAPS>
+template <int TH, int TW, int BN, int TAPS, int NP = 1>
 struct Lds32 {
     static constexpr int NPIX = (TH + 2) * (TW + 2);
     static constexpr int A_PLANE = NPIX * PSTR;
     static constexpr int B_PLANE = TAPS * CK * BN * 2;
-    static constexpr int STAGE = 2 * A_PLANE + 2 * B_PLANE;
-    static constexpr int STATS_BYTES = 4 * 2 * BN * 4;
+    static constexpr int STAGE = 2 * A_PLANE + NP * 2 * B_PLANE;
+    static constexpr int STATS_BYTES = NP * 4 * 2 * BN * 4;
     static constexpr int MAIN = ((STAGE > STATS_BYTES ? STAGE : STATS_BYTES) + 15) / 16 * 16;
     static int bytes(int ctot) { return MAIN + 2 * ((ctot + 7) / 8 * 8) * 4; }
 };
@@ -130,9 +130,40 @@
     }
 }
 
-template <int TH, int TW, int BN, int WM, int WN, int TAPS>
+template <int MPW, int NPW>
+__device__ __forceinline__ void store_tile_f32_up(const ConvArgs &A, const f32x16 (&acc)[MPW][NPW], int n, int y0, int x0, int mblock0, int nblock0,
+                                                  int half, int l31, int cout0, int pa_, int pb_) {
+    const size_t Wo = (size_t)A.W * 2, cs = (size_t)A.out_cstride;
+    float *out = reinterpret_cast<float *>(A.out);
+    const int yl = y0 + mblock0 * 2, xl = x0 + 4 * half;
+#pragma unroll
+    for (int ni = 0; ni < NPW; ++ni) {
+        const int co = cout0 + (nblock0 + ni) * 32 + l31;
+        const bool cok = co < A.Cout;
+        const float osc = (A.oscale && cok) ? A.oscale[co] : 1.f;
+        const float osh = fmaf((A.bias && cok) ? A.bias[co] : 0.f, osc, (A.oshift && cok) ? A.oshift[co] : 0.f);
+        float *lb = out + (((size_t)n * (A.H * 2) + (size_t)(yl * 2 + pa_)) * Wo + (size_t)(xl * 2 + pb_)) * cs + A.out_coff + co;
+#pragma unroll
+        for (int mi = 0; mi < MPW; ++mi)
+#pragma unroll
+            for (int r = 0; r < 16; ++r) {
+                const int p = (r & 3) + 8 * (r >> 2);
+                const int ty = mi * 2 + p / 16, tx = p % 16;
+                float v = fmaf(acc[mi][ni][r], osc, osh);
+                if (A.orelu) v = fmaxf(v, 0.f);
+                if (cok && yl + ty < A.H && xl + tx < A.W) lb[((size_t)(2 * ty) * Wo + (size_t)(2 * tx)) * cs] = v;
+            }
+    }
+}
+
+enum : int { FORM_GRID = 0, FORM_CHUNK = 1, FORM_ALLPAR = 2 };
+
+template <int TH, int TW, int BN, int WM, int WN, int TAPS, int FORM = FORM_GRID>
 __global__ __launch_bounds__(256, 2) void conv_f32_kernel(ConvArgs A) {
-    using L = Lds32<TH, TW, BN, TAPS>;
+    constexpr int NP = FORM == FORM_ALLPAR ? 4 : 1;
+    static_assert(FORM == FORM_GRID || TAPS == 4, "the chunk-parity and all-parity forms are four-tap launches");
+    static_assert(FORM != FORM_ALLPAR || (TH == 16 && TW == 16), "store_tile_f32_up: 16 x 16 tiles");
+    using L = Lds32<TH, TW, BN, TAPS, NP>;
     constexpr int HW_ = TW + 2, NPIX = L::NPIX;
     constexpr int MT = TH * TW / 32, NT = BN / 32;
     constexpr int MPW = MT / WM, NPW = NT / WN;
@@ -172,7 +203,8 @@
         cout_tile = seq - tile * NC;
     }
     const int z = tile / tiles_img, rt = tile - z * tiles_img;
-    const int n = z / A.npar, par = z - n * A.npar;
+    const int gpar = FORM == FORM_ALLPAR ? 1 : A.npar;
+    const int n = z / gpar, par = z - n * gpar;
     const int ty_ = rt / tiles_x;
     const int y0 = ty_ * TH, x0 = (rt - ty_ * tiles_x) * TW;
 
@@ -200,9 +232,11 @@
         if (c < n0) { si = 0; cc0 = c * CK; } else { si = 1; cc0 = (c - n0) * CK; }
     };
     const unsigned short *wbase = A.w + ((size_t)(par * gridDim.y + cout_tile) * A.nchunk) * (size_t)(L::B_PLANE);
-
+    const size_t wpar = (size_t)gridDim.y * A.nchunk * (size_t)(L::B_PLANE);
+
+    constexpr bool WFULL = NP > 1 && NBV % 256 == 0;
     f32x4 pa[NA][2];
-    u32x4 pb[NB];
+    u32x4 pb[NP * NB];
     auto issue = [&](int chunk) {
         int si, cc0;
         chunk_src(chunk, si, cc0);
@@ -216,14 +250,32 @@
             pa[i][0] = p[0];
             pa[i][1] = p[1];
         }
-        const u32x4 *wsrc = reinterpret_cast<const u32x4 *>(wbase + (size_t)chunk * L::B_PLANE);
-#pragma unroll
-        for (int i = 0; i < NB; ++i) {
-            const int v = tid + i * 256;
-            if (v < NBV) pb[i] = wsrc[v];
+#pragma unroll
+        for (int p = 0; p < NP; ++p) {
+            const u32x4 *wsrc = reinterpret_cast<const u32x4 *>(wbase + p * wpar + (size_t)chunk * L::B_PLANE);
+#pragma unroll
+            for (int i = 0; i < NB; ++i) {
+                const int v = tid + i * 256;
+                if (WFULL || v < NBV) pb[p * NB + i] = wsrc[v];
+            }
+        }
+    };
+    auto commit_w = [&]() {
+#pragma unroll
+        for (int p = 0; p < NP; ++p) {
+            u32x4 *bdst = reinterpret_cast<u32x4 *>(lds_b + p * 2 * L::B_PLANE);
+#pragma unroll
+            for (int i = 0; i < NB; ++i) {
+                const int v = tid + i * 256;
+                if (WFULL || v < NBV) bdst[v] = pb[p * NB + i];
+            }
         }
     };
     auto commit = [&](int chunk) {
+        if constexpr (NP > 1) {
+            commit_w();
+            __builtin_amdgcn_sched_barrier(0);
+        }
         int si, cc0;
         chunk_src(chunk, si, cc0);
         const ConvSrc &s = A.src[si];
@@ -273,12 +325,7 @@
             *reinterpret_cast<u32x4 *>(d) = hi;
             *reinterpret_cast<u32x4 *>(d + L::A_PLANE) = lo;
         }
-        u32x4 *bdst = reinterpret_cast<u32x4 *>(lds_b);
-#pragma unroll
-        for (int i = 0; i < NB; ++i) {
-            const int v = tid + i * 256;
-            if (v < NBV) bdst[v] = pb[i];
-        }
+        if constexpr (NP == 1) commit_w();
     };
 
     int abase[MPW];
@@ -293,6 +340,7 @@
     for (int t = 0; t < TAPS; ++t) {
         int r, c;
         if (TAPS == 9) { r = t / 3; c = t % 3; }
+        else if (TAPS == 4 && FORM == FORM_CHUNK) { r = t >> 1; c = t & 1; }
         else if (TAPS == 4) {
             const int a = par >> 1, b = par & 1, ty = t >> 1, tx = t & 1;
             r = a == 0 ? (ty == 0 ? 1 : 0) : (ty == 0 ? 2 : 1);
@@ -300,108 +348,209 @@
         } else { r = 1; c = 1; }
         toff[t] = (r * HW_ + c) * PSTR;
     }
-    f32x16 acc[MPW][NPW];
-#pragma unroll
-    for (int mi = 0; mi < MPW; ++mi)
-#pragma unroll
-        for (int ni = 0; ni < NPW; ++ni)
-#pragma unroll
-            for (int r = 0; r < 16; ++r) acc[mi][ni][r] = 0.f;
+    f32x16 acc[NP][MPW][NPW];
+#pragma unroll
+    for (int p = 0; p < NP; ++p)
+#pragma unroll
+        for (int mi = 0; mi < MPW; ++mi)
+#pragma unroll
+            for (int ni = 0; ni < NPW; ++ni)
+#pragma unroll
+                for (int r = 0; r < 16; ++r) acc[p][mi][ni][r] = 0.f;
+
+    auto products = [&](const bf16x8 (&ah)[MPW], const bf16x8 (&al)[MPW], int p, int t) {
+        bf16x8 bh[NPW], bl[NPW];
+#pragma unroll
+        for (int ni = 0; ni < NPW; ++ni) {
+            bh[ni] = *reinterpret_cast<const bf16x8 *>(lds_b + p * 2 * L::B_PLANE + bbase + t * 2 * BN * 16 + ni * 512);
+            bl[ni] = *reinterpret_cast<const bf16x8 *>(lds_b + p * 2 * L::B_PLANE + L::B_PLANE + bbase + t * 2 * BN * 16 + ni * 512);
+        }
+#pragma unroll
+        for (int mi = 0; mi < MPW; ++mi)
+#pragma unroll
+            for (int ni = 0; ni < NPW; ++ni) {
+                acc[p][mi][ni] = __builtin_amdgcn_mfma_f32_32x32x16_bf16(al[mi], bh[ni], acc[p][mi][ni], 0, 0, 0);
+                acc[p][mi][ni] = __builtin_amdgcn_mfma_f32_32x32x16_bf16(ah[mi], bl[ni], acc[p][mi][ni], 0, 0, 0);
+                acc[p][mi][ni] = __builtin_amdgcn_mfma_f32_32x32x16_bf16(ah[mi], bh[ni], acc[p][mi][ni], 0, 0, 0);
+            }
+    };
 
     issue(0);
+    int cpar = 0, cleft = A.par_chunks;
     for (int chunk = 0; chunk < A.nchunk; ++chunk) {
         __syncthreads();
         commit(chunk);
         __syncthreads();
         if (chunk + 1 < A.nchunk) issue(chunk + 1);
-#pragma unroll
-        for (int t = 0; t < TAPS; ++t) {
-            bf16x8 ah[MPW], al[MPW], bh[NPW], bl[NPW];
-#pragma unroll
-            for (int mi = 0; mi < MPW; ++mi) {
-                ah[mi] = *reinterpret_cast<const bf16x8 *>(lds_a + abase[mi] + toff[t]);
-                al[mi] = *reinterpret_cast<const bf16x8 *>(lds_a + L::A_PLANE + abase[mi] + toff[t]);
-            }
+        if constexpr (FORM == FORM_ALLPAR) {
+#pragma unroll
+            for (int q = 8; q >= 0; --q) {
+                const int r = q / 3, c = q % 3;
+                bf16x8 ah[MPW], al[MPW];
+#pragma unroll
+                for (int mi = 0; mi < MPW; ++mi) {
+                    ah[mi] = *reinterpret_cast<const bf16x8 *>(lds_a + abase[mi] + (r * HW_ + c) * PSTR);
+                    al[mi] = *reinterpret_cast<const bf16x8 *>(lds_a + L::A_PLANE + abase[mi] + (r * HW_ + c) * PSTR);
+                }
+#pragma unroll
+                for (int p = 0; p < 4; ++p) {
+                    const int ty = 1 + (p >> 1) - r, tx = 1 + (p & 1) - c;
+                    if (ty >= 0 && ty < 2 && tx >= 0 && tx < 2) products(ah, al, p, ty * 2 + tx);
+                }
+            }
+        } else {
+            int cbase = 0;
+            if constexpr (FORM == FORM_CHUNK) {
+                cbase = (((cpar >> 1) == 0 ? HW_ : 0) + ((cpar & 1) == 0 ? 1 : 0)) * PSTR;
+                if (--cleft == 0) { cleft = A.par_chunks; ++cpar; }
+            }
+#pragma unroll
+            for (int t = 0; t < TAPS; ++t) {
+                bf16x8 ah[MPW], al[MPW], bh[NPW], bl[NPW];
+#pragma unroll
+                for (int mi = 0; mi < MPW; ++mi) {
+                    ah[mi] = *reinterpret_cast<const bf16x8 *>(lds_a + abase[mi] + cbase + toff[t]);
+                    al[mi] = *reinterpret_cast<const bf16x8 *>(lds_a + L::A_PLANE + abase[mi] + cbase + toff[t]);
+                }
+#pragma unroll
+                for (int ni = 0; ni < NPW; ++ni) {
+                    bh[ni] = *reinterpret_cast<const bf16x8 *>(lds_b + bbase + t * 2 * BN * 16 + ni * 512);
+                    bl[ni] = *reinterpret_cast<const bf16x8 *>(lds_b + L::B_PLANE + bbase + t * 2 * BN * 16 + ni * 512);
+                }
+#pragma unroll
+                for (int mi = 0; mi < MPW; ++mi)
+#pragma unroll
+                    for (int ni = 0; ni < NPW; ++ni) {
+                        acc[0][mi][ni] = __builtin_amdgcn_mfma_f32_32x32x16_bf16(al[mi], bh[ni], acc[0][mi][ni], 0, 0, 0);
+                        acc[0][mi][ni] = __builtin_amdgcn_mfma_f32_32x32x16_bf16(ah[mi], bl[ni], acc[0][mi][ni], 0, 0, 0);
+                        acc[0][mi][ni] = __builtin_amdgcn_mfma_f32_32x32x16_bf16(ah[mi], bh[ni], acc[0][mi][ni], 0, 0, 0);
+                    }
+            }
+        }
+    }
+    __syncthreads();
+
+    const int cout0 = cout_tile * BN;
+    if constexpr (NP == 1) {
+        if (A.stats) {
+            float ssum[NPW], ssq[NPW];
+            const bool full_tile = y0 + TH <= A.H && x0 + TW <= A.W && !(A.debug & 16);
 #pragma unroll
             for (int ni = 0; ni < NPW; ++ni) {
-                bh[ni] = *reinterpret_cast<const bf16x8 *>(lds_b + bbase + t * 2 * BN * 16 + ni * 512);
-                bl[ni] = *reinterpret_cast<const bf16x8 *>(lds_b + L::B_PLANE + bbase + t * 2 * BN * 16 + ni * 512);
-            }
-#pragma unroll
-            for (int mi = 0; mi < MPW; ++mi)
-#pragma unroll
-                for (int ni = 0; ni < NPW; ++ni) {
-                    acc[mi][ni] = __builtin_amdgcn_mfma_f32_32x32x16_bf16(al[mi], bh[ni], acc[mi][ni], 0, 0, 0);
-                    acc[mi][ni] = __builtin_amdgcn_mfma_f32_32x32x16_bf16(ah[mi], bl[ni], acc[mi][ni], 0, 0, 0);
-                    acc[mi][ni] = __builtin_amdgcn_mfma_f32_32x32x16_bf16(ah[mi], bh[ni], acc[mi][ni], 0, 0, 0);
-                }
-        }
-    }
-    __syncthreads();
-
-    const int cout0 = cout_tile * BN;
-    if (A.stats) {
-        float ssum[NPW], ssq[NPW];
-        const bool full_tile = y0 + TH <= A.H && x0 + TW <= A.W && !(A.debug & 16);
-#pragma unroll
-        for (int ni = 0; ni < NPW; ++ni) {
-            ssum[ni] = 0.f; ssq[ni] = 0.f;
-            if (full_tile) {
+                ssum[ni] = 0.f; ssq[ni] = 0.f;
+                if (full_tile) {
+#pragma unroll
+                    for (int mi = 0; mi < MPW; ++mi)
+#pragma unroll
+                        for (int r = 0; r < 16; ++r) {
+                            const float v = acc[0][mi][ni][r];
+                            ssum[ni] += v;
+                            ssq[ni] = fmaf(v, v, ssq[ni]);
+                        }
+                } else {
 #pragma unroll
                 for (int mi = 0; mi < MPW; ++mi)
 #pragma unroll
                     for (int r = 0; r < 16; ++r) {
-                        const float v = acc[mi][ni][r];
+                        const int m = (wm * MPW + mi) * 32 + (r & 3) + 8 * (r >> 2) + 4 * half;
+                        const float v = ((y0 + m / TW) < A.H && (x0 + m % TW) < A.W) ? acc[0][mi][ni][r] : 0.f;
                         ssum[ni] += v;
                         ssq[ni] = fmaf(v, v, ssq[ni]);
                     }
-            } else {
-#pragma unroll
-            for (int mi = 0; mi < MPW; ++mi)
-#pragma unroll
-                for (int r = 0; r < 16; ++r) {
-                    const int m = (wm * MPW + mi) * 32 + (r & 3) + 8 * (r >> 2) + 4 * half;
-                    const float v = ((y0 + m / TW) < A.H && (x0 + m % TW) < A.W) ? acc[mi][ni][r] : 0.f;
-                    ssum[ni] += v;
-                    ssq[ni] = fmaf(v, v, ssq[ni]);
-                }
-            }
-            ssum[ni] += __shfl_xor(ssum[ni], 32);
-            ssq[ni] += __shfl_xor(ssq[ni], 32);
-            if (half == 0) {
-                s_stats[wave][0][(wn * NPW + ni) * 32 + l31] = ssum[ni];
-                s_stats[wave][1][(wn * NPW + ni) * 32 + l31] = ssq[ni];
-            }
-        }
-        __syncthreads();
-        if (tid < 2 * BN) {
-            const int which = tid / BN, col = tid % BN;
-            const int wn_of = col / (NPW * 32);
-            float v = 0.f;
-#pragma unroll
-            for (int k = 0; k < WM; ++k) v += s_stats[k * WN + wn_of][which][col];
-            const int co = cout0 + col;
-            if (co < A.Cout) A.stats[((size_t)tile * 2 + which) * A.Cout + co] = v;
-        }
-    }
-    store_tile_f32<MPW, NPW, TW>(A, acc, n, y0, x0, wm * MPW, wn * NPW, half, l31, cout0, par >> 1, par & 1);
-}
-
-template <int TH, int TW, int BN, int WM, int WN, int TAPS>
+                }
+                ssum[ni] += __shfl_xor(ssum[ni], 32);
+                ssq[ni] += __shfl_xor(ssq[ni], 32);
+                if (half == 0) {
+                    s_stats[wave][0][(wn * NPW + ni) * 32 + l31] = ssum[ni];
+                    s_stats[wave][1][(wn * NPW + ni) * 32 + l31] = ssq[ni];
+                }
+            }
+            __syncthreads();
+            if (tid < 2 * BN) {
+                const int which = tid / BN, col = tid % BN;
+                const int wn_of = col / (NPW * 32);
+                float v = 0.f;
+#pragma unroll
+                for (int k = 0; k < WM; ++k) v += s_stats[k * WN + wn_of][which][col];
+                const int co = cout0 + col;
+                if (co < A.Cout) A.stats[((size_t)tile * 2 + which) * A.Cout + co] = v;
+            }
+        }
+        store_tile_f32<MPW, NPW, TW>(A, acc[0], n, y0, x0, wm * MPW, wn * NPW, half, l31, cout0, par >> 1, par & 1);
+    } else {
+        const bool full_tile = y0 + TH <= A.H && x0 + TW <= A.W && !(A.debug & 16);
+#pragma unroll
+        for (int p = 0; p < NP; ++p) {
+            int yp = y0, xp = x0;
+            asm volatile("" : "+s"(yp), "+s"(xp));
+            if (A.stats) {
+#pragma unroll
+                for (int ni = 0; ni < NPW; ++ni) {
+                    float ssum = 0.f, ssq = 0.f;
+                    if (full_tile) {
+#pragma unroll
+                        for (int mi = 0; mi < MPW; ++mi)
+#pragma unroll
+                            for (int r = 0; r < 16; ++r) {
+                                const float v = acc[p][mi][ni][r];
+                                ssum += v;
+                                ssq = fmaf(v, v, ssq);
+                            }
+                    } else {
+#pragma unroll
+                        for (int mi = 0; mi < MPW; ++mi)
+#pragma unroll
+                            for (int r = 0; r < 16; ++r) {
+                                const int m = (wm * MPW + mi) * 32 + (r & 3) + 8 * (r >> 2) + 4 * half;
+                                const float v = ((yp + m / TW) < A.H && (xp + m % TW) < A.W) ? acc[p][mi][ni][r] : 0.f;
+                                ssum += v;
+                                ssq = fmaf(v, v, ssq);
+                            }
+                    }
+                    ssum += __shfl_xor(ssum, 32);
+                    ssq += __shfl_xor(ssq, 32);
+                    if (half == 0) {
+                        s_stats[p * 4 + wave][0][(wn * NPW + ni) * 32 + l31] = ssum;
+                        s_stats[p * 4 + wave][1][(wn * NPW + ni) * 32 + l31] = ssq;
+                    }
+                }
+            }
+            store_tile_f32_up<MPW, NPW>(A, acc[p], n, yp, xp, wm * MPW, wn * NPW, half, l31, cout0, p >> 1, p & 1);
+        }
+        if (A.stats) {
+            __syncthreads();
+            if (tid < 2 * BN) {
+                const int which = tid / BN, col = tid % BN;
+                const int wn_of = col / (NPW * 32);
+                const int co = cout0 + col;
+#pragma unroll
+                for (int p = 0; p < NP; ++p) {
+                    float v = 0.f;
+#pragma unroll
+                    for (int k = 0; k < WM; ++k) v += s_stats[p * 4 + k * WN + wn_of][which][col];
+                    const int row = (n * 4 + p) * tiles_img + rt;
+                    if (co < A.Cout) A.stats[((size_t)row * 2 + which) * A.Cout + co] = v;
+                }
+            }
+        }
+    }
+}
+
+template <int TH, int TW, int BN, int WM, int WN, int TAPS, int FORM = FORM_GRID>
 int launch_conv32(const ConvArgs &A, hipStream_t st) {
-    using L = Lds32<TH, TW, BN, TAPS>;
+    using L = Lds32<TH, TW, BN, TAPS, FORM == FORM_ALLPAR ? 4 : 1>;
     int ctot = 0;
     for (int i = 0; i < A.nsrc; ++i) ctot += A.src[i].C;
     const int smem = L::bytes(ctot);
-    dim3 grid(cdiv(A.W, TW) * cdiv(A.H, TH) * A.N * A.npar, cdiv(A.Cout, BN), 1);
-    return launch_lds<conv_f32_kernel<TH, TW, BN, WM, WN, TAPS>>(grid, 256, L::bytes(XF_MAX), smem, st, "hipFuncSetAttribute(conv32)", "conv_f32_kernel", A);
-}
-
-template <int TAPS>
+    dim3 grid(cdiv(A.W, TW) * cdiv(A.H, TH) * A.N * (FORM == FORM_ALLPAR ? 1 : A.npar), cdiv(A.Cout, BN), 1);
+    return launch_lds<conv_f32_kernel<TH, TW, BN, WM, WN, TAPS, FORM>>(grid, 256, L::bytes(XF_MAX), smem, st, "hipFuncSetAttribute(conv32)", "conv_f32_kernel", A);
+}
+
+template <int TAPS, int FORM = FORM_GRID>
 int dispatch_conv32(const ConvArgs &A, hipStream_t st) {
-    if (A.tile == 16 && A.BN == 64) return launch_conv32<16, 16, 64, 4, 1, TAPS>(A, st);
-    if (A.tile == 16 && A.BN == 32) return launch_conv32<16, 16, 32, 4, 1, TAPS>(A, st);
-    if (A.tile == 8 && A.BN == 64) return launch_conv32<8, 8, 64, 2, 2, TAPS>(A, st);
+    if (A.tile == 16 && A.BN == 64) return launch_conv32<16, 16, 64, 4, 1, TAPS, FORM>(A, st);
+    if (A.tile == 16 && A.BN == 32) return launch_conv32<16, 16, 32, 4, 1, TAPS, FORM>(A, st);
+    if (A.tile == 8 && A.BN == 64) return launch_conv32<8, 8, 64, 2, 2, TAPS, FORM>(A, st);
     set_error("cdnet_conv_forward(f32): unsupported configuration tile=%d CK=%d BN=%d", A.tile, A.CK, A.BN);
     return CDNET_E_ARG;
 }
@@ -664,7 +813,21 @@
     CDNET_REQUIRE(A.taps1 == 0 || A.taps1 == A.taps, "cdnet_conv_forward(f32): a one-tap second source runs on conv_ws32_kernel only (ask cdnet_conv_ws_eligible)");
     CDNET_REQUIRE(!A.pool_out, "cdnet_conv_forward(f32): the fused max-pool output rides in conv_ws32_kernel's epilogue only (ask cdnet_conv_ws_eligible)");
     if (A.taps == 9) return dispatch_conv32<9>(A, st);
-    if (A.taps == 4) return dispatch_conv32<4>(A, st);
+    if (A.taps == 4 && A.npar == 1) {
+        CDNET_REQUIRE(A.par_chunks > 0 && A.nsrc == 2 && A.src[0].C == 2 * A.par_chunks * CK && A.src[1].C == A.src[0].C && !A.stats,
+                      "cdnet_conv_forward(f32): taps = 4 with npar = 1 needs par_chunks > 0 and two sources of 2 * par_chunks chunks each (got %d; %d sources)",
+                      A.par_chunks, A.nsrc);
+        return dispatch_conv32<4, FORM_CHUNK>(A, st);
+    }
+    if (A.taps == 4) {
+        if (A.tile == 16 && A.BN == 32 && !(A.debug & CONV_DBG_PAR_GRID)) {
+            int n_cu = 0;
+            if (const int rc = cu_count(&n_cu)) return rc;
+            const long long wgs = (long long)cdiv(A.W, 16) * cdiv(A.H, 16) * A.N * cdiv(A.Cout, 32);
+            if (wgs >= n_cu || (A.debug & CONV_DBG_PERSIST_SMALL)) return launch_conv32<16, 16, 32, 4, 1, 4, FORM_ALLPAR>(A, st);
+        }
+        return dispatch_conv32<4>(A, st);
+    }
     {
         const int rc = try_conv1x1_stream(A, st);
         if (rc >= 0) return rc;
diff --git a/cdnet_amd/csrc/conv_args.h b/cdnet_amd/csrc/conv_args.h
--- a/cdnet_amd/csrc/conv_args.h
+++ b/cdnet_amd/csrc/conv_args.h
@@ -31,7 +31,7 @@
     const unsigned short *eres;
     const float *eres_scale, *eres_shift;
     int eres_f16, eres_relu;
-    int taps1, pad_;
+    int taps1, par_chunks;
     unsigned short *pool_out;
     const float *dot_w, *dot_b;
     float *dot_out;
@@ -42,6 +42,7 @@
     CONV_DBG_ONE_TILE = 32,
     CONV_DBG_PERSIST_SMALL = 64,
     CONV_DBG_OLD_WS16 = 128,
+    CONV_DBG_PAR_GRID = 128,
     CONV_DBG_NO_STREAM_1X1 = 256,
     CONV_DBG_GRID_SHIFT = 8,
 };
diff --git a/cdnet_amd/engine.py b/cdnet_amd/engine.py
--- a/cdnet_amd/engine.py
+++ b/cdnet_amd/engine.py
@@ -19,7 +19,7 @@
                 ('ostride', C.c_int), ('nchunk', C.c_int), ('tile', C.c_int), ('CK', C.c_int), ('BN', C.c_int),
                 ('out_f16', C.c_int), ('debug', C.c_int), ('ws', C.c_int), ('f32', C.c_int),
                 ('eres', C.c_void_p), ('eres_scale', C.c_void_p), ('eres_shift', C.c_void_p), ('eres_f16', C.c_int), ('eres_relu', C.c_int),
-                ('taps1', C.c_int), ('pad_', C.c_int), ('pool_out', C.c_void_p),
+                ('taps1', C.c_int), ('par_chunks', C.c_int), ('pool_out', C.c_void_p),
                 ('dot_w', C.c_void_p), ('dot_b', C.c_void_p), ('dot_out', C.c_void_p)]
 
 
@@ -115,6 +115,18 @@
     return (16, ck, bn)
 
 
+CONVT4_BWD_CFG = (8, 16, 64)
+
+
+def convT4_bwd_four_tap(ct, cin, nine_tap_persistent):
+    if ct % 16:
+        return False
+    force = os.environ.get('CDNET_CONVT4_BWD', '')
+    if force in ('4', '9'):
+        return force == '4'
+    return cin > 32 and not nine_tap_persistent
+
+
 def dominant_kernel_name(precision, tiles=16):
     if precision == 'fp32':
         return 'conv_ws32_kernel<64,0,false>'
@@ -132,7 +144,7 @@
         Cout, Cin, KH, KW = w.shape
     elif mode == 1:
         Cin, Cout, KH, KW = w.shape
-    elif mode in (4, 5, 6):
+    elif mode in (4, 5, 6, 8):
         Cout, ct, KH, KW = w.shape
         Cin = 4 * ct
     elif mode == 7:
@@ -140,7 +152,7 @@
         Cout = 4 * ct
     else:
         Cin, Cout, KH, KW = w.shape
-    taps = {2: 4, 3: 1, 4: 9, 5: 1, 6: 9, 7: 9}.get(mode, KH * KW)
+    taps = {2: 4, 3: 1, 4: 9, 5: 1, 6: 9, 7: 9, 8: 4}.get(mode, KH * KW)
     npar = 4 if mode in (2, 3) else 1
     return Cout, Cin, KH, KW, CK, BN, taps, npar
 
@@ -186,12 +198,13 @@
     return out
 
 
+CONV_DBG_PAR_GRID = 128
 CONV_DEBUG = 0
 
 
 def conv_forward(srcs, wpacked, Cout, cfg, taps=9, transposed=False, bias=None, oscale=None, oshift=None,
                  orelu=False, out=None, stats=None, H=None, W=None, out_dtype=torch.bfloat16, eres=None, query_ws=False, bns=None, taps1=0, pool_out=None, dot=None,
-                 pad_chunks=0, debug_or=0):
+                 pad_chunks=0, debug_or=0, par_chunks=0):
     tile, CK, BN = cfg[:3]
     s0 = srcs[0]
     f32 = s0.f32
@@ -231,8 +244,12 @@
     a.out_f16 = int(out is not None and out.dtype == torch.float16)
     a.ws = 0
     a.taps1 = taps1
+    assert par_chunks == 0 or (f32 and taps == 4 and not transposed and len(srcs) == 2 and nchunk == 4 * par_chunks)
+    a.par_chunks = par_chunks
     a.pool_out = _dp(pool_out)
     a.debug = CONV_DEBUG | debug_or
+    if f32 and transposed and taps == 4 and os.environ.get('CDNET_CONVT4_FWD', '') == 'grid':
+        a.debug |= CONV_DBG_PAR_GRID
     a.f32 = int(f32)
     assert out is None or (out.dtype == torch.float32) == f32
     if eres is not None:
diff --git a/cdnet_amd/runtime.py b/cdnet_amd/runtime.py
--- a/cdnet_amd/runtime.py
+++ b/cdnet_amd/runtime.py
@@ -108,23 +108,39 @@
             self.wp = engine.pack_weights(self.weight.detach(), self.cfg, self.pack_mode, Cin_pad=pad, out=self.wp, split=f32)
             self.wp_version = ver
 
-    def backward_pack(self, cin_total, H, W):
+    def backward_pack(self, cin_total, H, W, views=None):
         ver = (self.weight._version, WEIGHTS_EPOCH[0])
         f32 = self.cfg_f32
         if self.cfg_bwd is None:
             if self.transposed:
                 self.cfg_bwd = engine.choose_cfg([2 * self.Cout, 2 * self.Cout], self.Cin, H, W, taps=(9 if self.kind == 'convT4' else 1), f32=f32)
+                self.bwd_four_tap = False
+                if self.kind == 'convT4' and f32:
+                    ws = views is not None and engine.conv_forward(views, None, self.Cin, self.cfg_bwd, taps=9, H=H, W=W, query_ws=True) != 0
+                    self.bwd_four_tap = engine.convT4_bwd_four_tap(self.Cout, self.Cin, ws)
+                    if self.bwd_four_tap:
+                        self.cfg_bwd = engine.CONVT4_BWD_CFG
             else:
                 self.cfg_bwd = engine.choose_cfg([self.Cout], cin_total, H, W, taps=self.taps, f32=f32)
         if self.wpb is None or self.wpb_version != ver:
             if self.transposed:
-                mode = 4 if self.kind == 'convT4' else 5
+                mode = self.backward_pack_mode()
                 self.wpb = engine.pack_weights(self.weight.detach(), self.cfg_bwd, mode, out=self.wpb, split=f32)
             else:
                 assert cin_total == self.Cin, 'the RGB stem never needs an input gradient'
-                self.wpb = engine.pack_weights(self.weight.detach(), self.cfg_bwd, 7 if self.kind == 'conv3s2' else 1, out=self.wpb, split=f32)
+                self.wpb = engine.pack_weights(self.weight.detach(), self.cfg_bwd, self.backward_pack_mode(), out=self.wpb, split=f32)
             self.wpb_version = ver
         return self.wpb, self.cfg_bwd
+
+    def backward_pack_mode(self):
+        if self.transposed:
+            return (8 if getattr(self, 'bwd_four_tap', False) else 4) if self.kind == 'convT4' else 5
+        return 7 if self.kind == 'conv3s2' else 1
+
+    def backward_taps(self):
+        if self.kind != 'convT4':
+            return 1, 0
+        return (4, self.Cout // 16) if getattr(self, 'bwd_four_tap', False) else (9, 0)
 
     def eval_fold(self):
         bn = self.bn
diff --git a/cdnet_amd/trainer.py b/cdnet_amd/trainer.py
--- a/cdnet_amd/trainer.py
+++ b/cdnet_amd/trainer.py
@@ -585,7 +585,10 @@
         N = g.N if isinstance(g, Src) else g.shape[0]
         Cout = L.Cout
         cin_total = sum(s.C for s in srcs)
-        wpb, cfgb = L.backward_pack(cin_total, H, W)
+        views = None
+        if L.transposed:
+            views = [Src(g, view=(a * 2 * W * Cout, H, W, 2 * Cout, 4 * W * Cout)) for a in (0, 1)]
+        wpb, cfgb = L.backward_pack(cin_total, H, W, views)
         if L.kind == 'conv3s2':
             Cp = cin_total // 4
             gs2d = self.buf(('ds2d', L.name), (N, H, W, cin_total), runtime.act_dtype())
@@ -607,8 +610,8 @@
                 engine.conv_forward([g if isinstance(g, Src) else Src(g)], wpb, cin_total, cfgb, taps=L.taps, out=gin, H=H, W=W)
         else:
             gin = self.buf(('din', L.name), (N, H, W, cin_total), runtime.act_dtype())
-            views = [Src(g, view=(a * 2 * W * Cout, H, W, 2 * Cout, 4 * W * Cout)) for a in (0, 1)]
-            engine.conv_forward(views, wpb, cin_total, cfgb, taps=(9 if L.kind == 'convT4' else 1), out=gin, H=H, W=W)
+            taps, par_chunks = L.backward_taps()
+            engine.conv_forward(views, wpb, cin_total, cfgb, taps=taps, par_chunks=par_chunks, out=gin, H=H, W=W)
         coff = 0
         for s in srcs:
             if getattr(s, 'is_input', False):
@@ -688,8 +691,7 @@
                 if L.wp is not None and not L.wp_padded:
                     groups[0][0].append(engine.pack_job(w, L.cfg, L.pack_mode, L.wp, split=L.cfg_f32)); groups[0][1].append((L, 'wp_version'))
                 if L.wpb is not None:
-                    mode = (4 if L.kind == 'convT4' else 5) if L.transposed else (7 if L.kind == 'conv3s2' else 1)
-                    groups[1][0].append(engine.pack_job(w, L.cfg_bwd, mode, L.wpb, split=L.cfg_f32)); groups[1][1].append((L, 'wpb_version'))
+                    groups[1][0].append(engine.pack_job(w, L.cfg_bwd, L.backward_pack_mode(), L.wpb, split=L.cfg_f32)); groups[1][1].append((L, 'wpb_version'))
             if not groups[0][0] or not groups[1][0] or self.flat.step_count < 1:
                 return
             self._pack_jobs = []
diff --git a/include/cdnet_hip.h b/include/cdnet_hip.h
--- a/include/cdnet_hip.h
+++ b/include/cdnet_hip.h
@@ -102,7 +102,7 @@
     const float *eres_scale, *eres_shift;
     int eres_f16, eres_relu;
     int taps1;
-    int pad_;
+    int par_chunks;
     uint16_t *pool_out;
     const float *dot_w;
     const float *dot_b;
```

New measurement: 1108 (median of 6 runs). No clear change (+0.6%).
